# tub-rip/emba

Hardware: AMD Instinct MI355X
Metric: events/sec through warp+Jacobian+JtJ build, 1M events, 1024x2048 pano (higher is better)
Workload: dtype f64; 1 GPU; synthetic N=1000000 sensor=240x180 pano=1024x2048 K=21 seed=20240907; events_per_gpu=1000000, total_events=1000000, thres_valid_pixel=5, cost=quadratic, parallelism=single GPU, events_per_rank=1000000, ep_in_step=True, inliers_rank0=675197, candidates_rank0=956800, active_pixels=68600

## Files before the change

emba_amd/_lib.py:

```python
import ctypes as C
import os

_HERE = os.path.dirname(os.path.abspath(__file__))
LIB_PATH = os.environ.get("EMBA_LIB", os.path.join(_HERE, "libemba_hip.so"))

OK, ERR_INVALID_ARG, ERR_NO_DEVICE, ERR_HIP, ERR_TIME_RANGE, ERR_STATE, ERR_CAPACITY, ERR_NUMERIC = range(8)
STATUS_NAMES = ["EMBA_OK", "EMBA_ERR_INVALID_ARG", "EMBA_ERR_NO_DEVICE", "EMBA_ERR_HIP", "EMBA_ERR_TIME_RANGE",
                "EMBA_ERR_STATE", "EMBA_ERR_CAPACITY", "EMBA_ERR_NUMERIC"]

_dp = C.POINTER(C.c_double)
_i32p = C.POINTER(C.c_int32)
_u32p = C.POINTER(C.c_uint32)
_u16p = C.POINTER(C.c_uint16)
_u8p = C.POINTER(C.c_uint8)
_i64p = C.POINTER(C.c_int64)
_szp = C.POINTER(C.c_size_t)
_fp = C.POINTER(C.c_float)


class EmbaCfg(C.Structure):
    _fields_ = [("sensor_w", C.c_int32), ("sensor_h", C.c_int32), ("pano_w", C.c_int32), ("pano_h", C.c_int32),
                ("bearing_lut", _dp), ("C_th", C.c_double), ("event_batch", C.c_int32), ("outlier_px", C.c_double),
                ("device", C.c_int32), ("stream", C.c_void_p)]


class EmbaAlignSettings(C.Structure):
    _fields_ = [("max_iters", C.c_int32), ("min_pixels", C.c_int32), ("lambda0", C.c_double), ("lambda_up", C.c_double), ("lambda_down", C.c_double),
                ("lambda_min", C.c_double), ("lambda_max", C.c_double), ("tol_rot", C.c_double), ("huber_k", C.c_double)]


class EmbaTrackSettings(C.Structure):
    _fields_ = [("n_levels", C.c_int32), ("levels", C.c_int32 * 8), ("batch", C.c_int32), ("predict", C.c_int32), ("skip_zero", C.c_int32),
                ("min_weight", C.c_uint64), ("min_overlap", C.c_double), ("align", EmbaAlignSettings)]


class EmbaExposureSettings(C.Structure):
    _fields_ = [("align", EmbaAlignSettings), ("gain_min", C.c_double), ("gain_max", C.c_double)]


class EmbaTrackExposureSettings(C.Structure):
    _fields_ = [("track", EmbaTrackSettings), ("estimate", C.c_int32), ("gain_min", C.c_double), ("gain_max", C.c_double)]


class EmbaRefitSettings(C.Structure):
    _fields_ = [("track", EmbaTrackExposureSettings), ("sweeps", C.c_int32), ("alternate", C.c_int32), ("recover", C.c_int32), ("sweep_tol", C.c_double)]


class EmbaGraphSettings(C.Structure):
    _fields_ = [("max_iters", C.c_int32), ("cg_max_iters", C.c_int32), ("lambda0", C.c_double), ("lambda_up", C.c_double), ("lambda_down", C.c_double),
                ("lambda_min", C.c_double), ("lambda_max", C.c_double), ("tol", C.c_double), ("cg_tol", C.c_double)]


SIGNATURES = {
    "emba_abi_version": (C.c_int, []),
    "emba_build_info": (C.c_char_p, []),
    "emba_create": (C.c_int, [C.POINTER(EmbaCfg), C.POINTER(C.c_void_p)]),
    "emba_destroy": (None, [C.c_void_p]),
    "emba_last_error": (C.c_char_p, [C.c_void_p]),
    "emba_set_events": (C.c_int, [C.c_void_p, _u16p, _u16p, _u8p, _i64p, C.c_size_t, _u16p, _u16p, _i64p, C.c_size_t]),
    "emba_set_events_dev": (C.c_int, [C.c_void_p, C.c_void_p, C.c_void_p, C.c_void_p, C.c_void_p, C.c_size_t, C.c_void_p, C.c_void_p, C.c_void_p,
                                      C.c_size_t]),
    "emba_last_setup_ms": (C.c_int, [C.c_void_p, _dp, _dp, _i32p, _szp, _szp]),
    "emba_last_order_stats": (C.c_int, [C.c_void_p, _dp, _dp]),
    "emba_last_order_inlier_estimate": (C.c_int, [C.c_void_p, _dp]),
    "emba_last_tile_geometry": (C.c_int, [C.c_void_p, _i32p, _i32p, _i32p, _i32p, _i32p]),
    "emba_last_tile_drift": (C.c_int, [C.c_void_p, _szp, _i32p]),
    "emba_event_counts": (C.c_int, [C.c_void_p, _szp, _szp]),
    "emba_eval_data_error": (C.c_int, [C.c_void_p, _dp, C.c_int32, C.c_int64, C.c_int64, _dp, _dp, C.c_int32, _dp, _szp, _i32p]),
    "emba_form_normal_eq": (C.c_int, [C.c_void_p, _dp, C.c_int32, C.c_int32, C.c_double, C.c_double, _dp, _dp, _szp, _u32p,
                                      C.c_size_t, _dp, _dp, _dp]),
    "emba_get_A12_sparse": (C.c_int, [C.c_void_p, _i32p, _i32p, _i32p, _dp, _dp, _dp, _dp]),
    "emba_compact_ep": (C.c_int, [C.c_void_p]),
    "emba_get_ep": (C.c_int, [C.c_void_p, _dp, C.c_size_t, _szp]),
    "emba_get_inlier_pixels": (C.c_int, [C.c_void_p, _u32p]),
    "emba_get_inlier_pixel_starts": (C.c_int, [C.c_void_p, _u32p]),
    "emba_get_ep_by_pixel": (C.c_int, [C.c_void_p, _dp, C.POINTER(C.c_uint64)]),
    "emba_data_cost": (C.c_int, [C.c_void_p, C.c_int32, C.c_double, _dp]),
    "emba_reg_cost": (C.c_int, [C.c_void_p, C.c_double, _dp]),
    "emba_costs": (C.c_int, [C.c_void_p, C.c_int32, C.c_double, C.c_double, _dp, _dp]),
    "emba_costs_launch": (C.c_int, [C.c_void_p, C.c_int32, C.c_double, C.c_int32]),
    "emba_costs_finish": (C.c_int, [C.c_void_p, C.c_int32, C.c_double, C.c_double, _dp, _dp]),
    "emba_dump_state": (C.c_int, [C.c_void_p, _dp, _dp, _i32p, _i32p, _i32p, _dp, _dp, _dp]),
    "emba_upload_map": (C.c_int, [C.c_void_p, _dp, _dp]),
    "emba_bind_map_dev": (C.c_int, [C.c_void_p, C.c_void_p, C.c_void_p]),
    "emba_solve_normal_eq": (C.c_int, [C.c_void_p, C.c_double, C.c_int32, _dp, _dp]),
    "emba_solve_map_only": (C.c_int, [C.c_void_p, C.c_double, _dp]),
    "emba_solve_poses_only": (C.c_int, [C.c_void_p, C.c_double, C.c_int32, _dp]),
    "emba_last_solve_info": (C.c_int, [C.c_void_p, _i32p]),
    "emba_solve_shard_size": (C.c_int, [C.c_void_p, _szp]),
    "emba_solve_shard_count": (C.c_int, [C.c_void_p, C.c_int32, _szp]),
    "emba_solve_shard_pack": (C.c_int, [C.c_void_p, C.c_int32, C.c_void_p]),
    "emba_cg_shard_size": (C.c_int, [C.c_void_p, _szp]),
    "emba_cg_shard_begin": (C.c_int, [C.c_void_p, C.c_int32, C.c_int32, C.c_void_p, C.c_size_t, C.c_double, C.c_int32, C.c_void_p]),
    "emba_cg_shard_apply": (C.c_int, [C.c_void_p, C.c_void_p]),
    "emba_cg_shard_pt": (C.c_int, [C.c_void_p, C.c_void_p, _dp]),
    "emba_cg_shard_update": (C.c_int, [C.c_void_p, C.c_double, C.c_void_p]),
    "emba_cg_shard_direction": (C.c_int, [C.c_void_p, C.c_double]),
    "emba_cg_shard_end": (C.c_int, [C.c_void_p, _dp, C.c_void_p]),
    "emba_solve_shard_cached": (C.c_int, [C.c_void_p, C.c_int32, C.c_int32, _i32p, _szp]),
    "emba_solve_shard_partial": (C.c_int, [C.c_void_p, C.c_int32, C.c_int32, C.c_void_p, C.c_size_t, C.c_double, C.c_void_p]),
    "emba_solve_shard_finish": (C.c_int, [C.c_void_p, C.c_int32, C.c_int32, C.c_void_p, C.c_size_t, C.c_double, C.c_int32, C.c_void_p, _dp, C.c_void_p]),
    "emba_solve_normal_eq_cg": (C.c_int, [C.c_void_p, C.c_double, C.c_int32, C.c_int32, C.c_double, _dp, _dp, _i32p, _dp]),
    "emba_update_map": (C.c_int, [C.c_void_p, _dp, C.c_double]),
    "emba_update_map_dev": (C.c_int, [C.c_void_p, C.c_void_p, C.c_double]),
    "emba_map_accept": (C.c_int, [C.c_void_p]),
    "emba_map_reject": (C.c_int, [C.c_void_p]),
    "emba_trial_reject": (C.c_int, [C.c_void_p]),
    "emba_download_map": (C.c_int, [C.c_void_p, _dp, _dp]),
    "emba_get_map_active": (C.c_int, [C.c_void_p, _dp, C.c_size_t]),
    "emba_set_cost": (C.c_int, [C.c_void_p, C.c_int32, C.c_double]),
    "emba_reconstruct_intensity": (C.c_int, [C.c_void_p, _dp, _dp, _dp]),
    "emba_render_map_images": (C.c_int, [C.c_void_p, C.c_double, _u8p, _u8p, _u8p, _u8p]),
    "emba_reconstruct_intensity_bc": (C.c_int, [C.c_void_p, _dp, _dp, _dp, C.c_int32]),
    "emba_render_map_images_bc": (C.c_int, [C.c_void_p, C.c_double, _u8p, _u8p, _u8p, _u8p, C.c_int32]),
    "emba_normalize_robust": (C.c_int, [C.c_void_p, _dp, C.c_size_t, C.c_double, _u8p, _dp, _dp]),
    "emba_seq_upload": (C.c_int, [C.c_void_p, _u16p, _u16p, _u8p, _i64p, C.c_size_t, C.c_int32, _szp]),
    "emba_seq_size": (C.c_int, [C.c_void_p, _szp]),
    "emba_seq_free": (C.c_int, [C.c_void_p]),
    "emba_seq_window": (C.c_int, [C.c_void_p, C.c_int64, C.c_int64, _szp, _szp]),
    "emba_set_events_seq": (C.c_int, [C.c_void_p, C.c_size_t, C.c_size_t]),
    "emba_set_events_seq_shard": (C.c_int, [C.c_void_p, C.c_size_t, C.c_size_t, C.c_size_t]),
    "emba_seq_halo": (C.c_int, [C.c_void_p, C.c_size_t, C.c_size_t, _u16p, _u16p, _i64p, C.c_size_t, _szp]),
    "emba_seq_get": (C.c_int, [C.c_void_p, C.c_size_t, C.c_size_t, _u16p, _u16p, _u8p, _i64p]),
    "emba_seq_filter": (C.c_int, [C.c_void_p, C.c_double, C.c_int64, C.c_int64, C.c_int32, C.POINTER(C.c_uint64)]),
    "emba_seq_hot_pixels": (C.c_int, [C.c_void_p, _u8p]),
    "emba_seq_cmax": (C.c_int, [C.c_void_p, C.c_int64, C.c_double, _dp, _i64p, C.POINTER(C.c_uint64), C.POINTER(C.c_uint64), _i32p, C.c_size_t, _szp]),
    "emba_seq_cmax_objective": (C.c_int, [C.c_void_p, C.c_size_t, C.c_size_t, _dp, C.c_size_t, C.POINTER(C.c_uint64), _u32p, _i32p, _i32p, _i32p]),
    "emba_seq_event_panorama": (C.c_int, [C.c_void_p, C.c_size_t, C.c_size_t, _dp, C.c_int32, C.c_int64, C.c_int64, C.c_int32, _i32p, C.POINTER(C.c_uint64), _i64p,
                                          C.POINTER(C.c_uint64), C.POINTER(C.c_uint64), _dp]),
    "emba_seq_contrast_gradient": (C.c_int, [C.c_void_p, C.c_size_t, C.c_size_t, _dp, C.c_int32, C.c_int64, C.c_int64, C.c_int32, _dp, _dp, _dp,
                                             C.POINTER(C.c_uint64), _dp, _dp, _i32p]),
    "emba_seq_contrast_gradient_level": (C.c_int, [C.c_void_p, C.c_size_t, C.c_size_t, _dp, C.c_int32, C.c_int64, C.c_int64, C.c_int32, C.c_int32, _dp, _dp,
                                                   _dp, C.POINTER(C.c_uint64), _dp, _dp, _i32p]),
    "emba_seq_contrast_prior_add": (C.c_int, [C.c_void_p, C.c_size_t, C.c_size_t, _dp, C.c_int32, C.c_int64, C.c_int64, C.c_int32, C.c_uint32, _szp,
                                              C.POINTER(C.c_uint64)]),
    "emba_seq_contrast_prior_set": (C.c_int, [C.c_void_p, C.c_int32, _dp]),
    "emba_seq_contrast_prior_get": (C.c_int, [C.c_void_p, C.c_int32, _dp, _i32p]),
    "emba_seq_contrast_prior_clear": (C.c_int, [C.c_void_p]),
    "emba_seq_contrast_gradient_prior": (C.c_int, [C.c_void_p, C.c_size_t, C.c_size_t, _dp, C.c_int32, C.c_int64, C.c_int64, C.c_int32, C.c_int32, C.c_double,
                                                   _dp, _dp, _dp, C.POINTER(C.c_uint64), _dp, _dp, _i32p]),
    "emba_render_views": (C.c_int, [C.c_void_p, _dp, C.c_int32, _i64p, C.c_size_t, _dp, C.c_int32, C.c_int64, C.c_int64, C.c_double, C.c_double, C.c_double,
                                    _dp, _u8p, C.POINTER(C.c_uint64), _dp]),
    "emba_seq_event_frames": (C.c_int, [C.c_void_p, C.c_size_t, C.c_size_t, _i64p, C.c_size_t, C.c_int32, _i32p, C.POINTER(C.c_uint64), C.POINTER(C.c_uint64)]),
    "emba_mosaic_frames": (C.c_int, [C.c_void_p, _u8p, _i64p, C.c_size_t, _dp, C.c_int32, C.c_int64, C.c_int64, C.c_int32, C.c_int32, C.POINTER(C.c_uint64),
                                     C.POINTER(C.c_uint64), _dp]),
    "emba_mosaic_get": (C.c_int, [C.c_void_p, C.c_uint64, C.c_double, C.POINTER(C.c_uint64), C.POINTER(C.c_uint64), _dp, _u8p, C.POINTER(C.c_uint64)]),
    "emba_mosaic_map": (C.c_int, [C.c_void_p, C.c_uint64, C.c_double, C.c_double, C.c_double, C.c_int32, _dp, _dp, _dp, C.c_int32]),
    "emba_mosaic_clear": (C.c_int, [C.c_void_p]),
    "emba_simulate_events": (C.c_int, [C.c_void_p, _dp, C.c_int32, _i64p, C.c_size_t, _dp, C.c_int32, C.c_int64, C.c_int64, C.c_double, C.c_double, C.c_int32,
                                       C.c_uint64, C.POINTER(C.c_uint64)]),
    "emba_sim_size": (C.c_int, [C.c_void_p, _szp]),
    "emba_sim_get": (C.c_int, [C.c_void_p, C.c_size_t, C.c_size_t, _u16p, _u16p, _u8p, _i64p]),
    "emba_seq_from_sim": (C.c_int, [C.c_void_p, C.c_int32, _szp]),
    "emba_frames_align_eval": (C.c_int, [C.c_void_p, _u8p, C.c_size_t, _dp, _dp, _u8p, C.c_int32, C.c_uint64, C.c_double, C.c_double, C.c_double, C.c_int32,
                                         C.c_double, _dp, C.POINTER(C.c_uint64), _dp, _dp]),
    "emba_frames_align": (C.c_int, [C.c_void_p, _u8p, C.c_size_t, _dp, _dp, _u8p, C.c_int32, C.c_uint64, C.c_double, C.c_double, C.c_double, C.c_int32,
                                    C.c_void_p, _dp, _dp, C.POINTER(C.c_uint64), _i32p, _i32p, _dp, C.POINTER(C.c_uint64)]),
    "emba_frames_track": (C.c_int, [C.c_void_p, _u8p, _i64p, C.c_size_t, _dp, C.c_void_p, _dp, _i32p, _i32p, _dp, C.POINTER(C.c_uint64), _dp, C.POINTER(C.c_uint64), _dp]),
    "emba_track_eval": (C.c_int, [C.c_void_p, _u8p, C.c_size_t, _dp, C.c_int32, C.c_uint64, C.c_int32, C.c_double, _dp, C.POINTER(C.c_uint64), _dp, _dp]),
    "emba_track_level_get": (C.c_int, [C.c_void_p, C.c_int32, C.POINTER(C.c_uint64), C.POINTER(C.c_uint64)]),
    "emba_frames_exposure_eval": (C.c_int, [C.c_void_p, _u8p, C.c_size_t, _dp, _dp, _dp, _dp, _u8p, C.c_int32, C.c_uint64, C.c_double, C.c_double, C.c_double,
                                            C.c_int32, C.c_double, _dp, C.POINTER(C.c_uint64), _dp, _dp]),
    "emba_frames_exposure_align": (C.c_int, [C.c_void_p, _u8p, C.c_size_t, _dp, _dp, _dp, C.c_int32, _dp, _u8p, C.c_int32, C.c_uint64, C.c_double, C.c_double,
                                             C.c_double, C.c_int32, C.c_void_p, _dp, _dp, _dp, _dp, C.POINTER(C.c_uint64), _i32p, _i32p, _dp, C.POINTER(C.c_uint64)]),
    "emba_mosaic_frames_exposure": (C.c_int, [C.c_void_p, _u8p, _i64p, C.c_size_t, _dp, _dp, _dp, C.c_int32, C.c_int64, C.c_int64, C.c_int32, C.c_int32,
                                              C.POINTER(C.c_uint64), C.POINTER(C.c_uint64), _dp]),
    "emba_frames_track_exposure": (C.c_int, [C.c_void_p, _u8p, _i64p, C.c_size_t, _dp, C.c_void_p, _dp, _dp, _dp, _i32p, _i32p, _dp, C.POINTER(C.c_uint64), _dp,
                                             C.POINTER(C.c_uint64), _dp]),
    "emba_track_exposure_eval": (C.c_int, [C.c_void_p, _u8p, C.c_size_t, _dp, _dp, _dp, C.c_int32, C.c_uint64, C.c_int32, C.c_double, _dp, C.POINTER(C.c_uint64),
                                           _dp, _dp]),
    "emba_frames_refit": (C.c_int, [C.c_void_p, _u8p, _i64p, C.c_size_t, _dp, _dp, _dp, _i32p, C.c_void_p, _dp, _dp, _dp, _i32p, _i32p, _i32p, _dp,
                                    C.POINTER(C.c_uint64), _dp, _dp, _i32p, C.POINTER(C.c_uint64), _dp]),
    "emba_frames_pair_eval": (C.c_int, [C.c_void_p, _u8p, C.c_size_t, _i32p, C.c_size_t, _dp, _dp, _dp, C.c_double, C.c_double, C.c_double, C.c_double, _dp,
                                        C.c_int32, C.c_double, _dp, C.POINTER(C.c_uint64), _dp, _dp]),
    "emba_frames_pair_align": (C.c_int, [C.c_void_p, _u8p, C.c_size_t, _i32p, C.c_size_t, _dp, _dp, _dp, C.c_double, C.c_double, C.c_double, C.c_double, _dp,
                                         C.c_int32, C.c_void_p, _dp, _dp, C.POINTER(C.c_uint64), _i32p, _i32p, _dp, C.POINTER(C.c_uint64), _dp]),
    "emba_rotation_graph_solve": (C.c_int, [_dp, _i32p, C.c_size_t, _i32p, _dp, _dp, C.c_size_t, C.c_void_p, _dp, _dp, _i32p, _i32p, _szp]),
    "emba_median_blur3_map": (C.c_int, [C.c_void_p]),
    "emba_median_blur3": (C.c_int, [C.c_void_p, _dp, C.c_int32, C.c_int32, _dp]),
    "emba_bind_exchange_buffers": (C.c_int, [C.c_void_p, C.c_void_p, C.c_void_p, C.c_size_t]),
    "emba_count_map_ready": (C.c_int, [C.c_void_p]),
    "emba_count_compress": (C.c_int, [C.c_void_p, C.c_void_p, C.c_int32]),
    "emba_count_expand": (C.c_int, [C.c_void_p, C.c_void_p]),
    "emba_step_form_active": (C.c_int, [C.c_void_p, C.c_int32, C.c_void_p]),
    "emba_eval_launch": (C.c_int, [C.c_void_p, _dp, C.c_int32, C.c_int64, C.c_int64]),
    "emba_eval_finish": (C.c_int, [C.c_void_p, _dp, _szp, _i32p]),
    "emba_form_active": (C.c_int, [C.c_void_p, C.c_int32, _szp, _szp]),
    "emba_form_accumulate": (C.c_int, [C.c_void_p, _dp, C.c_int32, C.c_double]),
    "emba_form_finish": (C.c_int, [C.c_void_p, C.c_double, _dp, _dp, _u32p, C.c_size_t, _dp, _dp, _dp]),
    "emba_step": (C.c_int, [C.c_void_p, _dp, C.c_int32, C.c_int64, C.c_int64, C.c_int32, C.c_int32, C.c_double, C.c_double, _szp, _szp]),
    "emba_last_counts": (C.c_int, [C.c_void_p, _szp, _szp]),
    "emba_set_option": (C.c_int, [C.c_void_p, C.c_char_p, C.c_int32]),
    "emba_get_option": (C.c_int, [C.c_void_p, C.c_char_p, _i32p]),
    "emba_sync": (C.c_int, [C.c_void_p]),
    "emba_timer_start": (C.c_int, [C.c_void_p, C.c_int32]),
    "emba_timer_stop": (C.c_int, [C.c_void_p, C.c_int32]),
    "emba_timer_elapsed_ms": (C.c_int, [C.c_void_p, C.c_int32, _fp]),
    "emba_enable_kernel_timing": (C.c_int, [C.c_void_p, C.c_int32]),
    "emba_last_kernel_ms": (C.c_int, [C.c_void_p, _fp, _fp]),
    "emba_kernel_ms_slot": (C.c_int, [C.c_void_p, C.c_int32, _fp, _fp]),
    "emba_kernel_timing_all": (C.c_int, [C.c_void_p, C.c_int32]),
    "emba_kernel_ms_all": (C.c_int, [C.c_void_p, C.c_int32, _fp]),
    "emba_bracket_overhead_us": (C.c_int, [C.c_void_p, C.c_int32, _fp]),
    "emba_clock_probe": (C.c_int, [C.c_void_p, _dp, _dp, _dp, _i32p, _i32p, _i32p]),
    "emba_device_pci_bus_id": (C.c_int, [C.c_void_p, C.c_char_p, C.c_size_t]),
    "emba_group_create": (C.c_int, [C.POINTER(EmbaCfg), _i32p, C.c_int32, C.POINTER(C.c_void_p)]),
    "emba_group_create_flags": (C.c_int, [C.POINTER(EmbaCfg), _i32p, C.c_int32, C.c_uint32, C.POINTER(C.c_void_p)]),
    "emba_group_set_option": (C.c_int, [C.c_void_p, C.c_char_p, C.c_int32]),
    "emba_group_destroy": (None, [C.c_void_p]),
    "emba_group_last_error": (C.c_char_p, [C.c_void_p]),
    "emba_group_size": (C.c_int32, [C.c_void_p]),
    "emba_group_uses_rccl": (C.c_int32, [C.c_void_p]),
    "emba_group_ctx": (C.c_void_p, [C.c_void_p, C.c_int32]),
    "emba_group_set_events": (C.c_int, [C.c_void_p, _u16p, _u16p, _u8p, _i64p, C.c_size_t]),
    "emba_group_seq_upload": (C.c_int, [C.c_void_p, _u16p, _u16p, _u8p, _i64p, C.c_size_t, C.c_int32, _szp]),
    "emba_group_seq_size": (C.c_int, [C.c_void_p, _szp]),
    "emba_group_seq_free": (C.c_int, [C.c_void_p]),
    "emba_group_seq_window": (C.c_int, [C.c_void_p, C.c_int64, C.c_int64, _szp, _szp]),
    "emba_group_seq_filter": (C.c_int, [C.c_void_p, C.c_double, C.c_int64, C.c_int64, C.c_int32, C.POINTER(C.c_uint64)]),
    "emba_group_set_events_seq": (C.c_int, [C.c_void_p, C.c_size_t, C.c_size_t]),
    "emba_group_median_blur3_map": (C.c_int, [C.c_void_p]),
    "emba_group_upload_map": (C.c_int, [C.c_void_p, _dp, _dp]),
    "emba_group_step": (C.c_int, [C.c_void_p, _dp, C.c_int32, C.c_int64, C.c_int64, C.c_int32, C.c_int32, C.c_double, C.c_double, _szp, _szp]),
    "emba_group_eval": (C.c_int, [C.c_void_p, _dp, C.c_int32, C.c_int64, C.c_int64, _dp, _dp, _dp, _szp, _i32p]),
    "emba_group_get_ep": (C.c_int, [C.c_void_p, _dp, C.c_size_t, _szp]),
    "emba_group_form": (C.c_int, [C.c_void_p, C.c_int32, C.c_int32, C.c_double, C.c_double, _szp, _szp]),
    "emba_group_set_cost": (C.c_int, [C.c_void_p, C.c_int32, C.c_double]),
    "emba_group_apply_l2": (C.c_int, [C.c_void_p, C.c_double]),
    "emba_group_last_solve_exchanged": (C.c_int, [C.c_void_p, _i32p]),
    "emba_group_solve_cg": (C.c_int, [C.c_void_p, C.c_double, C.c_int32, C.c_int32, C.c_double, _dp, _dp, _i32p, _dp]),
    "emba_group_trial_reject": (C.c_int, [C.c_void_p]),
    "emba_group_download": (C.c_int, [C.c_void_p, _dp, _dp, _u32p, C.c_size_t, _dp, _dp]),
    "emba_group_costs": (C.c_int, [C.c_void_p, C.c_int32, C.c_double, C.c_double, _dp, _dp]),
    "emba_group_solve": (C.c_int, [C.c_void_p, C.c_double, C.c_int32, _dp, _dp]),
    "emba_group_solve_map_only": (C.c_int, [C.c_void_p, C.c_double, _dp]),
# ... 32 lines not shown
```

emba_amd/csrc/context.h:

```cpp
#pragma once
#include "../../include/emba_hip.h"

#include <hip/hip_runtime.h>

#include <algorithm>
#include <cmath>
#include <cstdarg>
#include <cstdio>
#include <string>
#include <vector>

#include "kernels.h"
#include "solve_kernels.h"
#include "map_rule.h"
#include "cmax_rule.h"
#include "contrast_rule.h"

struct DevBuf {
    void* p = nullptr;
    size_t bytes = 0;
    DevBuf() = default;
    DevBuf(DevBuf&& o) noexcept : p(o.p), bytes(o.bytes) { o.p = nullptr; o.bytes = 0; }
    DevBuf& operator=(DevBuf&& o) noexcept { if (this != &o) { reset(); std::swap(p, o.p); std::swap(bytes, o.bytes); } return *this; }
    ~DevBuf() { reset(); }
    template <typename T> T* as() const { return static_cast<T*>(p); }
    void reset() { if (p) (void)hipFree(p); p = nullptr; bytes = 0; }
    hipError_t ensure(size_t n, bool* fresh = nullptr, bool poison = false, hipStream_t s = nullptr)
    {
        n = std::max<size_t>(n, 8);
        if (fresh) *fresh = false;
        if (p && bytes >= n) return hipSuccess;
        reset();
        hipError_t e = hipMalloc(&p, n);
        if (e != hipSuccess) { p = nullptr; return e; }
        bytes = n;
        if (fresh) *fresh = true;
        return poison ? hipMemsetAsync(p, 0xFF, n, s) : hipSuccess;
    }
};

struct RecordSet { DevBuf rec, tag; uint32_t stamp = 0; };

struct SolveLists { uint32_t* off = nullptr; emba::RecView sorted{}; };

struct EqState {
    bool active_done = false, accum_done = false;
    bool finish_done = false;
    bool compact_valid = false;
    bool l2_fused = false;
    bool force_generic_a22 = false;
    size_t P = 0, pack_len = 0;
    int K = 0, thres = 0, irls = 0; double eta = 0;
};

struct EvalState {
    bool launched = false, done = false;
    bool ep_deferred = false;
    bool inl_pending = false, P_pending = false;
    bool seq_armed = false;
    bool inl_idx_valid = false;
    bool ep_valid = false;
    bool ep_in_gram = false;
    bool ep_after_gram = false;
    bool pix_starts_valid = false;
    uint32_t count_stamp = 0;
    int acc_irls = 0; double acc_eta = 0.0;
    int use_texel = 0;
    bool prep_in_warp = false;
    bool texels_packed = false;
    bool segpose = false;
    bool readable() const { return launched && (done || inl_pending || ep_deferred); }
};

struct PixAccState {
    bool first_use() const { return dirty_all_; }
    bool lines_clean() const { return clean_; }
    bool lines_consumed() const { return consumed_; }
    bool counts_raw() const { return raw_; }
    int32_t marker() const { return mark_; }
    void bound() { dirty_all_ = true; clean_ = false; }
    void first_use_cleared() { dirty_all_ = false; clean_ = true; }
    void marked(int32_t marker) { mark_ = marker; clean_ = false; consumed_ = false; raw_ = true; }
    void not_marked() { raw_ = false; }
    void materialised() { raw_ = false; }
    void consumed_by_gather() { clean_ = true; consumed_ = true; }
private:
    bool dirty_all_ = true, clean_ = false, consumed_ = false, raw_ = false;
    int32_t mark_ = 0;
};

struct MapPlanes {
    DevBuf own_x, own_y, trial_x, trial_y;
    const double* Gx() const { return x_; }
    const double* Gy() const { return y_; }
    const double* cur_Gx() const { return cur_x_; }
    const double* cur_Gy() const { return cur_y_; }
    const emba::MapState& state() const { return st_; }
    void uploaded() { to_own(); st_.uploaded(); }
    void bound(const double* gx, const double* gy) { x_ = cur_x_ = gx; y_ = cur_y_ = gy; st_.bound(); }
    void trial_built() { x_ = trial_x.as<double>(); y_ = trial_y.as<double>(); st_.trial_built(); }
    void accepted() { std::swap(own_x, trial_x); std::swap(own_y, trial_y); to_own(); st_.accepted(); }
    void rejected() { x_ = cur_x_; y_ = cur_y_; st_.rejected(); }
    void blurred() { to_own(); st_.blurred(); }
    void texels_packed() { st_.texels_packed(); }
private:
    void to_own() { x_ = cur_x_ = own_x.as<double>(); y_ = cur_y_ = own_y.as<double>(); }
    const double *x_ = nullptr, *y_ = nullptr, *cur_x_ = nullptr, *cur_y_ = nullptr;
    emba::MapState st_;
};

struct PostWarpState {
    bool gather_deferred = false; emba::ActiveWriteParams gather{};
    int fsup_half = 0;
    void defer(const emba::ActiveWriteParams& aw) { gather = aw; gather_deferred = true; }
};

struct EvalOpts { int irls = 0; double eta = 0.0; bool keep_alt_set = false; };
struct FormOpts {
    bool consume = false, wants_ep = false;
    const uint8_t* global_u8 = nullptr;
    double fused_alpha = 0.0;
};

struct WindowState {
    bool have_events = false;
    size_t n_in = 0, n_used = 0, n_halo = 0, n_pm = 0, n_sorted = 0, n_batch = 0, n_cand = 0;
    long nblk = 0;
    long n_fblk = 0, n_fsup = 0;
    size_t P_prev = 0;
    size_t n_outside_tile = 0; int n_rebin = 0; uint32_t last_rebin_stamp = 0;
};

struct OrderState {
    bool keys_ready = false; int64_t key_t0 = 0, key_dt = 0; int key_K = 0;
    uint32_t* d_ev_pix = nullptr; uint32_t* d_ev_batch = nullptr;
    bool tile_order = false, have_ev_pm = false;
    long n_chunks = 0;
    size_t n_lead = 0;
    bool chunks_lpt = false;
    int tile_shape = 0; bool tile_fine = false;
    double order_per_px = 0.0, order_lead_frac = 0.0;
    double order_inl_pred = 0.0;
    std::vector<uint32_t> run_start; bool runs_known = false;
    int cuts_sw = 0, cuts_base_blocks = 0, cuts_blocks = 0;
};

enum StatusWord : int {
    kStFirstBad = 0,
    kStUnsorted = 1,
    kStProbeA = 0, kStProbeB = 1,
    kStBadHalo = 2,
    kStTotal = 4,
    kStHeads = 6,
    kStCounter = 8,
    kStatusWords = 16
};

struct ListsKey {
    bool packed = false; uint32_t stamp = 0; size_t P = 0, nrec = 0; long lo = 0;
    bool operator==(const ListsKey& o) const { return packed == o.packed && stamp == o.stamp && P == o.P && nrec == o.nrec && lo == o.lo; }
};

struct SolveCache {
    bool lists_valid = false; ListsKey key;
    bool perm_valid = false;
    size_t perm_lo = 0, perm_n = 0;
    size_t x2_resident_P = (size_t)-1;
    int info = 0;
    struct CgShard { bool active = false; int rank = 0, n_ranks = 1, n = 0, skip = 0; size_t lo = 0, npix = 0, Nl = 0; double lambda = 0; } cg;
    void invalidate() { lists_valid = false; perm_valid = false; }
};

struct CmaxBuffers { DevBuf omega, t_ref, j0, j, evals, cand, cand_j, cand_iwe; };

struct SeqPoseBuffers { DevBuf batch_t, pose, knots; };

struct PanoBuffers { DevBuf image, slots, out, pm; };

struct ContrastBuffers { DevBuf image, slots, out, pm, D, cp; };

struct ContrastPriors {
    DevBuf image[emba::kContrastLevels], out;
    bool present[emba::kContrastLevels] = {};
    void drop() { for (bool& b : present) b = false; }
    void reset() { drop(); for (DevBuf& b : image) b.reset(); }
};

struct ViewBuffers { DevBuf plane, t, pose, knots, head, frames, u8, pm, outside, edge, counts, ends; };

struct MosaicBuffers {
    DevBuf sum_w, sum_v; uint64_t votes = 0;
    DevBuf t, pose, knots, head, frames, pm, counters, mean, covered, L, covered_log, gx, gy;
};

struct FrameLoopBuffers {
    DevBuf frames, pm, resid, partial, q_trial, esums, ecounts;
    DevBuf q, sums, counts, lambda, dnorm, status, iters, have_trial, cost0, n0, running;
};

struct AlignBuffers { DevBuf plane, valid; FrameLoopBuffers loop; };

struct TrackBuffers {
    DevBuf lw[8], lv[8]; uint32_t voted = 0;
    DevBuf t, q_all, status_all, iters_all, cost_all, overlap_all, counts_all, counters, pred;
    DevBuf gain_all, bias_all, gain_pred, bias_pred, gain_trial, bias_trial, gain, bias;
    DevBuf refit_all;
    FrameLoopBuffers loop;
};

struct ExposureBuffers {
    FrameLoopBuffers loop;
    DevBuf gain_trial, bias_trial, gain, bias;
    DevBuf vote_gain, vote_bias;
};

struct PairBuffers { DevBuf pairs, gain, bias; FrameLoopBuffers loop; };

struct SimState {
    DevBuf x, y, pol, t, x2, y2, pol2, t2; size_t n = 0; bool have = false; uint64_t stats[4] = {0, 0, 0, 0};
    DevBuf plane, step_t, pose, knots, head, frames, outside, cells, ref[2], armed[2], sums, total, ev_t, ev_sp;
};

struct PoissonBuffers {
    DevBuf SH;
    DevBuf lamH;
    DevBuf SW;
    DevBuf lamW;
    DevBuf thomas;
    DevBuf wrapq;
    DevBuf Sfold;
    DevBuf Gx, Gy;
    DevBuf F;
    DevBuf T;
    DevBuf EO;
};

struct emba_ctx {
    emba_cfg cfg{};
    int device = 0;
    hipStream_t stream = nullptr;
    bool own_stream = false;
    std::string err;

    int sw = 0, sh = 0, W = 0, H = 0;
    size_t S = 0, npix = 0;
    double fx = 0, fy = 0, cx = 0, cy = 0, C_th = 0, outlier_px = 10.0;
    double fov_x = M_PI, fov_y = M_PI;

    DevBuf d_lut;
    DevBuf d_texel;
    MapPlanes map;
    SolveCache solve;
    int solve_perm_mode = -1;
    double* h_cost = nullptr;
    double* h_cost_dev = nullptr; DevBuf d_cost_acc; int cost_seq = 0;
    DevBuf d_x2;
    DevBuf d_count_own; int32_t* d_count = nullptr;
    DevBuf d_pixacc;
    PixAccState pix;
    int texel_mode = 0;
    DevBuf d_rect;
    uint32_t seg_seq = 0;
    int step_prep = 0, step_prep_polls = 1024;
    emba::InlineSegParams seg_inline{}; emba::InlineKnots seg_knots{};
    DevBuf d_seg_flag;
    DevBuf d_blk_rect;
    DevBuf d_compact, d_active_bits;
    DevBuf d_active;
    DevBuf d_ablk_cnt, d_ablk_off; size_t n_ablk = 0;
    DevBuf d_pack_own;
    double* d_pack = nullptr; size_t pack_cap = 0; bool pack_bound = false;
    DevBuf d_knots;
    int* d_err = nullptr;
    DevBuf d_err2;
    uint32_t eval_seq = 0;
    DevBuf d_total;
    std::vector<uint32_t> h_pix_starts;
    void* h_stage[2] = {nullptr, nullptr}; hipEvent_t stage_ev[2]{};
    int* h_pinned = nullptr;
    int seq = 0;
    bool spun = false;
    int* h_pinned_dev = nullptr;
    double* h_knots_dev = nullptr;

    WindowState win;
    OrderState order;
    DevBuf d_pm_pix, d_pm_batch, d_pm_orig;
    DevBuf d_ev_slot;
    DevBuf d_ev_pix_own, d_ev_batch_own;
    DevBuf d_ev_pm;
    DevBuf d_cp, d_batch_u;
    DevBuf d_ev_u, d_ev_seg;
    DevBuf d_chunks;
    int segpose_mode = 0;
    int order_mode = 0;
    DevBuf d_batch_t, d_pose;
    DevBuf d_seg;
    int step_gather = 2;
    DevBuf d_seg_act;
    PostWarpState post;
    int step_one_set = 1;
    int step_fast = 1;
    int use_tags = 1;
    DevBuf d_gram_cuts; std::vector<uint32_t> h_gram_cuts; bool last_gram_paired = false;
    DevBuf d_slot_key; uint32_t rec_stamp = 0;
    RecordSet work, alt;
    bool eq_in_alt = false;
    EqState eq, eq_saved;
    EvalState ev;
    DevBuf d_e_sorted, d_flag, d_inl_idx;
    int opt_poison = 0;
    int opt_tile_reserve = 2, opt_tile_shape = -1, opt_tile_fine = -1, opt_tile_min_events = 1650000, opt_tile_chunk = 0;
    int opt_gather_waves = 0, opt_chunk_order_bin = 0, opt_solve_counts = -1, opt_syrk_dense = 0, opt_syrk_lists = 0, opt_gram_sparse = -1, opt_gram_sparse_chunk = 4, opt_gram_multikey = 0, opt_syrk_min_cols = 512, opt_syrk_item_cap = 4096, opt_solve_debug = 0, opt_poisson = 0, opt_gemm64 = 0;
    int step_ep = 1;
    DevBuf d_fblk_cnt, d_fblk_off;
    DevBuf d_fsup;
    DevBuf d_ep;
    double set_events_ms = 0, prepare_ms = 0;

    size_t n_inliers = 0;
    int cost_irls = 0; double cost_eta = 0.0;
    double* h_knots = nullptr; int h_knots_cap = 0; hipEvent_t knots_copied = nullptr; bool knots_in_flight = false;

    hipEvent_t ev_start[8]{}, ev_stop[8]{};
    bool kernel_timing = false;
    hipEvent_t kt_sets[16][5]{}; hipEvent_t* kt = kt_sets[0]; int kt_slot = 0;
    bool kt_valid[16][3]{};
    bool kt_all = false;
    hipEvent_t cal_ev[2]{};
    DevBuf d_probe;
    bool kt_warp_valid = false, kt_accum_valid = false;
    int n_cu = 256;
    int ablate = 0;
    struct {
        DevBuf scan_sums, scan_offs;
        DevBuf sort_hist;
        DevBuf status;
        DevBuf keys[2], vals[2];
        DevBuf flags;
        DevBuf pos;
        DevBuf bin, used;
        DevBuf bin_start_or_x;
        DevBuf pred_or_y;
        DevBuf heads_or_pol;
        DevBuf halo;
    } ord;
    struct Solve {
        DevBuf S_or_x, rhs_or_r, U_or_p, y_or_z, cf_or_t, x2_or_invd;
        DevBuf info_or_sc;
        DevBuf slab, mask, list, cnt, range, pair_items, items;
        DevBuf perm_cnt, perm_tick, perm;
        DevBuf shard_cnt;
    } sv;
    struct {
        DevBuf off, cursor, sorted, tmp;
    } lists;
    struct {
        DevBuf out;
        DevBuf pix_starts;
        DevBuf A22b2;
    } dl;
    PoissonBuffers poisson;
    DevBuf d_rstate, d_rhist, d_rcand;
    DevBuf d_img, d_nsrc;
    struct {
        DevBuf x, y, pol, t, raw, status, halo_last, halo_flag, halo_pos; size_t n = 0;
        DevBuf x2, y2, pol2, t2, f_start, f_hot, f_sums; bool have = false, have_hot = false;
        void reset()
        {
            for (DevBuf* b : {&x, &y, &pol, &t, &raw, &status, &halo_last, &halo_flag, &halo_pos, &x2, &y2, &pol2, &t2, &f_start, &f_hot, &f_sums}) b->reset();
            n = 0; have = have_hot = false;
        }
    } evseq;
    emba::CmaxPinhole cmax_pin;
    CmaxBuffers cmax;
    SeqPoseBuffers seq_pose;
    PanoBuffers pano;
    ContrastBuffers contrast;
    ContrastPriors priors;
    int opt_contrast_vote = -1;
    int contrast_vote_path = -1;
    ViewBuffers view;
    SimState sim;
    MosaicBuffers mosaic;
    AlignBuffers align;
    TrackBuffers track;
    ExposureBuffers exposure;
    PairBuffers pair;
    DevBuf d_blur;
};

namespace {

thread_local std::string g_create_error;

emba_status fail(emba_ctx* c, emba_status st, const char* fmt, ...)
{
    char buf[512];
    va_list ap;
    va_start(ap, fmt);
    vsnprintf(buf, sizeof buf, fmt, ap);
    va_end(ap);
    if (c) c->err = buf; else g_create_error = buf;
    return st;
}

#define HIP_TRY(c, call)                                                                         \
    do {                                                                                         \
        hipError_t e_ = (call);                                                                  \
        if (e_ != hipSuccess)                                                                    \
            return fail((c), EMBA_ERR_HIP, "%s failed: %s (%s:%d)", #call, hipGetErrorString(e_), \
                        __FILE__, __LINE__);                                                     \
    } while (0)

template <typename T>
emba_status ensure(emba_ctx* c, DevBuf& b, size_t count, bool* fresh = nullptr)
// ... 13 lines not shown
```

emba_amd/csrc/device_math.h:

```cpp
#pragma once
#include <hip/hip_runtime.h>
#include <stdint.h>

namespace emba {

#pragma clang fp contract(off)

constexpr double kSophusEps = 1e-10;
constexpr double kPi = 3.14159265358979323846;

__device__ __forceinline__ double sum3(double a, double b, double c) { return a + (b + c); }
__device__ __forceinline__ double sqn3(double a, double b, double c) { return (a + b) + c; }

__device__ __forceinline__ void mat3_mul(const double* A, const double* B, double* C)
{
    double T[9];
#pragma unroll
    for (int i = 0; i < 3; ++i)
#pragma unroll
        for (int j = 0; j < 3; ++j) {
            const double t0 = A[3 * i + 0] * B[0 + j], t1 = A[3 * i + 1] * B[3 + j], t2 = A[3 * i + 2] * B[6 + j];
            T[3 * i + j] = (i < 2) ? (t0 + t1) + t2 : t0 + (t1 + t2);
        }
#pragma unroll
    for (int i = 0; i < 9; ++i) C[i] = T[i];
}

__device__ __forceinline__ void hat3(const double* p, double* M)
{
    M[0] = 0;     M[1] = -p[2]; M[2] = p[1];
    M[3] = p[2];  M[4] = 0;     M[5] = -p[0];
    M[6] = -p[1]; M[7] = p[0];  M[8] = 0;
}

__device__ __forceinline__ void quat_normalize(double* q)
{
    const double n2 = (q[0] * q[0] + q[2] * q[2]) + (q[1] * q[1] + q[3] * q[3]);
    const double n = sqrt(n2);
    q[0] /= n; q[1] /= n; q[2] /= n; q[3] /= n;
}

__device__ __forceinline__ void so3_mul(const double* a, const double* b, double* out)
{
    const double ax = a[0], ay = a[1], az = a[2], aw = a[3];
    const double bx = b[0], by = b[1], bz = b[2], bw = b[3];
    double r[4];
    r[3] = aw * bw - ax * bx - ay * by - az * bz;
    r[0] = aw * bx + ax * bw + ay * bz - az * by;
    r[1] = aw * by + ay * bw + az * bx - ax * bz;
    r[2] = aw * bz + az * bw + ax * by - ay * bx;
    quat_normalize(r);
    out[0] = r[0]; out[1] = r[1]; out[2] = r[2]; out[3] = r[3];
}

__device__ __forceinline__ void quat_to_matrix(const double* q, double* R)
{
    const double x = q[0], y = q[1], z = q[2], w = q[3];
    const double tx = 2 * x, ty = 2 * y, tz = 2 * z;
    const double twx = tx * w, twy = ty * w, twz = tz * w;
    const double txx = tx * x, txy = ty * x, txz = tz * x;
    const double tyy = ty * y, tyz = tz * y, tzz = tz * z;
    R[0] = 1 - (tyy + tzz); R[1] = txy - twz;       R[2] = txz + twy;
    R[3] = txy + twz;       R[4] = 1 - (txx + tzz); R[5] = tyz - twx;
    R[6] = txz - twy;       R[7] = tyz + twx;       R[8] = 1 - (txx + tyy);
}

__device__ __forceinline__ void sin_cos_half(double x, double& sn, double& cs)
{
    if (fabs(x) <= 0x1.921fb54442d18p-1) {
        const double z = x * x;
        const double rs = fma(z, fma(z, fma(z, fma(z, 1.58969099521155010221e-10, -2.50507602534068634195e-08), 2.75573137070700676789e-06),
                                     -1.98412698298579493134e-04), 8.33333333332248946124e-03);
        sn = fma(z * x, fma(z, rs, -1.66666666666666324348e-01), x);
        const double rc = z * fma(z, fma(z, fma(z, fma(z, fma(z, -1.13596475577881948265e-11, 2.08757232129817482790e-09), -2.75573143513906633035e-07),
                                              2.48015872894767294178e-05), -1.38888888888741095749e-03), 4.16666666666666019037e-02);
        const double hz = 0.5 * z, w = 1.0 - hz;
        cs = w + fma(z, rc, (1.0 - w) - hz);
    } else {
        sn = sin(x); cs = cos(x);
    }
}

__device__ __forceinline__ double rcp_nr(double x)
{
    double r = __builtin_amdgcn_rcp(x);
    double e = fma(-x, r, 1.0);
    r = fma(r, e, r);
    e = fma(-x, r, 1.0);
    return fma(r, e, r);
}

__device__ __forceinline__ void so3_exp(const double* w, double* q)
{
    const double theta_sq = sqn3(w[0] * w[0], w[1] * w[1], w[2] * w[2]);
    double imag, real;
    if (theta_sq < kSophusEps * kSophusEps) {
        const double theta_po4 = theta_sq * theta_sq;
        imag = 0.5 - (1.0 / 48.0) * theta_sq + (1.0 / 3840.0) * theta_po4;
        real = 1.0 - (1.0 / 8.0) * theta_sq + (1.0 / 384.0) * theta_po4;
    } else {
        const double theta = sqrt(theta_sq);
        const double half = 0.5 * theta;
        double sn, cs;
        sin_cos_half(half, sn, cs);
        imag = sn / theta;
        real = cs;
    }
    q[0] = imag * w[0]; q[1] = imag * w[1]; q[2] = imag * w[2]; q[3] = real;
}

__device__ __forceinline__ void so3_log(const double* q, double* w)
{
    const double squared_n = sqn3(q[0] * q[0], q[1] * q[1], q[2] * q[2]);
    const double qw = q[3];
    double f;
    if (squared_n < kSophusEps * kSophusEps) {
        const double squared_w = qw * qw;
        f = 2.0 / qw - (2.0 / 3.0) * (squared_n) / (qw * squared_w);
    } else {
        const double n = sqrt(squared_n);
        if (fabs(qw) < kSophusEps) f = (qw > 0.0) ? kPi / n : -kPi / n;
        else f = 2.0 * atan(n / qw) / n;
    }
    w[0] = f * q[0]; w[1] = f * q[1]; w[2] = f * q[2];
}

__device__ __forceinline__ void left_jacobian(const double* phi, double* J)
{
    const double n2 = sqn3(phi[0] * phi[0], phi[1] * phi[1], phi[2] * phi[2]);
    double H[9], H2[9];
    hat3(phi, H);
    mat3_mul(H, H, H2);
#pragma unroll
    for (int i = 0; i < 9; ++i) J[i] = (i % 4 == 0) ? 1.0 : 0.0;
    if (n2 > kSophusEps) {
        const double n = sqrt(n2);
        const double n3 = n2 * n;
        const double c1 = 1 - cos(n), c2 = n - sin(n);
#pragma unroll
        for (int i = 0; i < 9; ++i) J[i] += H[i] * c1 / n2;
#pragma unroll
        for (int i = 0; i < 9; ++i) J[i] += H2[i] * c2 / n3;
    } else {
#pragma unroll
        for (int i = 0; i < 9; ++i) J[i] += H[i] / 2;
#pragma unroll
        for (int i = 0; i < 9; ++i) J[i] += H2[i] / 6;
    }
}

__device__ __forceinline__ void left_jacobian_inv(const double* phi, double* J)
{
    const double n2 = sqn3(phi[0] * phi[0], phi[1] * phi[1], phi[2] * phi[2]);
    double H[9], H2[9];
    hat3(phi, H);
    mat3_mul(H, H, H2);
#pragma unroll
    for (int i = 0; i < 9; ++i) J[i] = ((i % 4 == 0) ? 1.0 : 0.0) - H[i] / 2;
    if (n2 > kSophusEps) {
        const double n = sqrt(n2);
        if (n < kPi - sqrt(kSophusEps)) {
            const double c = 1 / n2 - (1 + cos(n)) / (2 * n * sin(n));
#pragma unroll
            for (int i = 0; i < 9; ++i) J[i] += H2[i] * c;
        } else {
#pragma unroll
            for (int i = 0; i < 9; ++i) J[i] += H2[i] / (kPi * kPi);
        }
    } else {
#pragma unroll
        for (int i = 0; i < 9; ++i) J[i] += H2[i] / 12;
    }
}

__device__ __forceinline__ void spline2_eval(const double* p0, const double* p1, double u, double* q_out, double* J1)
{
    double p0inv[4] = {-p0[0], -p0[1], -p0[2], p0[3]};
    quat_normalize(p0inv);
    double r01[4], delta[3], kdelta[3];
    so3_mul(p0inv, p1, r01);
    so3_log(r01, delta);
#pragma unroll
    for (int i = 0; i < 3; ++i) kdelta[i] = delta[i] * u;
    double Jli[9], Jlk[9], T[9], R0[9], R0inv[9];
    left_jacobian_inv(delta, Jli);
    left_jacobian(kdelta, Jlk);
    quat_to_matrix(p0, R0);
#pragma unroll
    for (int i = 0; i < 9; ++i) T[i] = u * R0[i];
    mat3_mul(T, Jlk, T);
    mat3_mul(T, Jli, T);
    quat_to_matrix(p0inv, R0inv);
    mat3_mul(T, R0inv, J1);
    double e[4], res[4];
    so3_exp(kdelta, e);
    so3_mul(p0, e, res);
    q_out[0] = res[0]; q_out[1] = res[1]; q_out[2] = res[2]; q_out[3] = res[3];
}

__device__ __forceinline__ void project_jacobian(const double* rb, double fx, double fy, double* J23);

__device__ __forceinline__ void segment_consts(const double* p0, const double* p1, double* seg)
{
    double p0inv[4] = {-p0[0], -p0[1], -p0[2], p0[3]};
    quat_normalize(p0inv);
    double r01[4], delta[3], R0[9];
    so3_mul(p0inv, p1, r01);
    so3_log(r01, delta);
    const double n2 = sqn3(delta[0] * delta[0], delta[1] * delta[1], delta[2] * delta[2]);
    const double th = sqrt(n2);
    double k[3] = {0, 0, 0}, r2;
    if (th > 0.0) {
        quat_to_matrix(p0, R0);
        const double a0 = delta[0] / th, a1 = delta[1] / th, a2 = delta[2] / th;
#pragma unroll
        for (int r = 0; r < 3; ++r) k[r] = R0[3 * r] * a0 + R0[3 * r + 1] * a1 + R0[3 * r + 2] * a2;
    }
    if (n2 > kSophusEps) {
        if (th < kPi - sqrt(kSophusEps)) r2 = 1.0 - th * (1.0 + cos(th)) / (2.0 * sin(th));
        else r2 = n2 / (kPi * kPi);
    } else {
        r2 = n2 / 12.0;
    }
    seg[0] = p0[0]; seg[1] = p0[1]; seg[2] = p0[2]; seg[3] = p0[3];
    seg[4] = delta[0]; seg[5] = delta[1]; seg[6] = delta[2]; seg[7] = -0.5 * th;
    seg[8] = k[0]; seg[9] = k[1]; seg[10] = k[2]; seg[11] = r2;
}

__device__ __forceinline__ void rebuild_j1(double u, double a1, double a2, const double* k, double* J1)
{
    const double kk = k[0] * k[0] + k[1] * k[1] + k[2] * k[2];
    const double d = u - a2 * kk;
    J1[0] = d + a2 * k[0] * k[0]; J1[1] = a2 * k[0] * k[1] - a1 * k[2]; J1[2] = a2 * k[0] * k[2] + a1 * k[1];
    J1[3] = a2 * k[1] * k[0] + a1 * k[2]; J1[4] = d + a2 * k[1] * k[1]; J1[5] = a2 * k[1] * k[2] - a1 * k[0];
    J1[6] = a2 * k[2] * k[0] - a1 * k[1]; J1[7] = a2 * k[2] * k[1] + a1 * k[0]; J1[8] = d + a2 * k[2] * k[2];
}

__device__ __attribute__((noinline)) double2 sin_cos_call(double x)
{
    double sn, cs;
    sin_cos_half(x, sn, cs);
    return make_double2(sn, cs);
}

template <bool CALL>
__device__ __forceinline__ void spline2_event(const double* seg, double u, double* q_out, double* J1)
{
    const double kd[3] = {seg[4] * u, seg[5] * u, seg[6] * u};
    const double theta_sq = sqn3(kd[0] * kd[0], kd[1] * kd[1], kd[2] * kd[2]);
    double imag, real, p1c, p2c;
    if (theta_sq < kSophusEps * kSophusEps) {
        const double theta_po4 = theta_sq * theta_sq;
        imag = 0.5 - (1.0 / 48.0) * theta_sq + (1.0 / 3840.0) * theta_po4;
        real = 1.0 - (1.0 / 8.0) * theta_sq + (1.0 / 384.0) * theta_po4;
        const double n = sqrt(theta_sq);
        p1c = 0.5 * n; p2c = theta_sq * (1.0 / 6.0);
    } else {
        const double theta = sqrt(theta_sq);
        const double half = 0.5 * theta;
        double sh, ch;
        if (CALL) { const double2 sc = sin_cos_call(half); sh = sc.x; ch = sc.y; }
        else sin_cos_half(half, sh, ch);
        imag = sh / theta;
        real = ch;
        if (theta_sq > kSophusEps) { const double it2 = 2.0 * rcp_nr(theta); p1c = sh * sh * it2; p2c = 1.0 - sh * ch * it2; }
        else { p1c = 0.5 * theta; p2c = theta_sq * (1.0 / 6.0); }
    }
    const double e[4] = {imag * kd[0], imag * kd[1], imag * kd[2], real};
    so3_mul(seg, e, q_out);
    const double r1 = seg[7], r2 = seg[11];
    const double alpha = p1c + r1 - p1c * r2 - p2c * r1, gamma = p2c + r2 + p1c * r1 - p2c * r2;
    rebuild_j1(u, u * alpha, u * gamma, seg + 8, J1);
}

__device__ __forceinline__ void project_jacobian(const double* rb, double fx, double fy, double* J23);

__device__ __attribute__((noinline)) double2 project_angles_call(double x, double y, double z)
{
    const double phi = atan2(x, z);
    const double r2 = x * x + y * y + z * z;
    return make_double2(phi, asin(y / sqrt(r2)));
}


template <bool CALL = false>
__device__ __forceinline__ void project_chain(const double* rb, double fx, double fy, double cx, double cy,
                                              double* pm, double* J23)
{
    if (CALL) {
        const double2 a = project_angles_call(rb[0], rb[1], rb[2]);
        pm[0] = cx + a.x * fx;
        pm[1] = cy + a.y * fy;
        project_jacobian(rb, fx, fy, J23);
        return;
    }
    const double x = rb[0], y = rb[1], z = rb[2];
    const double phi = atan2(x, z);
    const double r2 = x * x + y * y + z * z;
    const double theta = asin(y / sqrt(r2));
    pm[0] = cx + phi * fx;
    pm[1] = cy + theta * fy;
    project_jacobian(rb, fx, fy, J23);
}

#pragma clang fp contract(fast)
__device__ __forceinline__ void project_jacobian(const double* rb, double fx, double fy, double* J23)
{
    const double x = rb[0], y = rb[1], z = rb[2];
    const double d2 = x * x + z * z;
    const double rho = sqrt(d2 + y * y);
    const double inv_rho = rcp_nr(rho);
    const double Ydivrho = y * inv_rho;
    const double inv_d2 = rcp_nr(d2);
    const double inv_d = fx * inv_d2;
    const double tmp2 = -fy * rho * (sqrt(d2) * inv_d2);
    const double tmp3 = Ydivrho * inv_rho * inv_rho;
    const double Jp[6] = {z * inv_d, 0.0, -x * inv_d, tmp2 * tmp3 * x, tmp2 * (tmp3 * y - inv_rho), tmp2 * tmp3 * z};
    const double M[9] = {0, rb[2], -rb[1], -rb[2], 0, rb[0], rb[1], -rb[0], 0};
#pragma unroll
    for (int i = 0; i < 2; ++i)
#pragma unroll
        for (int j = 0; j < 3; ++j) {
            double s = 0;
#pragma unroll
            for (int k = 0; k < 3; ++k) s += Jp[3 * i + k] * M[3 * k + j];
            J23[3 * i + j] = s;
        }
}

}
```

emba_amd/csrc/kernels.h:

```cpp
#pragma once
#include <hip/hip_runtime.h>
#include <stdint.h>

#include "device_math.h"
#include "order_rule.h"
#include "step_rule.h"

#ifdef EMBA_DIAG
#define EMBA_ABL(word, bit) (((word) & (bit)) != 0)
#else
#define EMBA_ABL(word, bit) false
#endif

namespace emba {

constexpr uint32_t kNoSlot = 0xFFFFFFFFu;
constexpr uint32_t kInvalidPix = 0xFFFFFFFFu;

__device__ __forceinline__ bool record_valid(double tail_y, uint32_t stamp, uint32_t& pano_idx)
{
    pano_idx = (uint32_t)__double2loint(tail_y);
    return (uint32_t)__double2hiint(tail_y) == stamp && pano_idx != kInvalidPix;
}
__host__ __device__ __forceinline__ int32_t count_marker(uint32_t stamp) { return (int32_t)(0x80000000u | (stamp & 0x3FFFFFFFu)); }
constexpr int kPoseStride = 14;
#ifndef TEXEL_STRIDE
#define TEXEL_STRIDE 6
#endif
constexpr int kTexelStride = TEXEL_STRIDE;
constexpr int kRecStride = 16;
constexpr int kWarpBlock = 64;
constexpr int kWarpNew = 63;
constexpr int kRecLds = 18;
constexpr int kPixAccStride = 8;
#ifndef REC_NT_STORE
#define REC_NT_STORE 1
#endif
#ifndef EP_NT_STORE
#define EP_NT_STORE 1
#endif
#ifndef GRAM_NT_LOAD
#define GRAM_NT_LOAD 1
#endif
#ifndef EV_NT_LOAD
#define EV_NT_LOAD 1
#endif
#ifndef GRAM_TAG_NT
#define GRAM_TAG_NT 0
#endif
template <class T> __device__ __forceinline__ T stream_load(const T* p, bool nt) { return nt ? __builtin_nontemporal_load(p) : *p; }
#ifndef GRAM_DUMMY_LOADS
#define GRAM_DUMMY_LOADS 0
#endif
#ifndef GRAM_U_NT
#define GRAM_U_NT 3
#endif
#ifndef GRAM_U
#define GRAM_U 4
#endif
#ifndef GRAM_SPARSE_TS
#define GRAM_SPARSE_TS 2
#endif
constexpr int kGramPad = 256;
constexpr int kGramChunkMin = 64;
constexpr int kGramChunk = 1024;
#ifndef GATHER_Q
#define GATHER_Q 4
#endif
#ifndef GRAM_GATHER_WAVES
#ifndef GRAM_WAVE_TILE
#define GRAM_WAVE_TILE 1
#endif
#define GRAM_GATHER_WAVES 4
#endif
constexpr int kGramBlock = 1024;
constexpr int kGramKeys = 4;

__device__ __forceinline__ long xcd_contiguous_block(long bid, long grid)
{
    const long per = grid >> 3;
    return (bid & 7) * per + (bid >> 3);
}

__device__ __forceinline__ void pose_thread(int b, const int64_t* __restrict__ batch_t_ns, int nb, const double* __restrict__ knots,
                                            int K, int64_t t0_ns, int64_t dt_ns, double* __restrict__ pose, int* __restrict__ err)
{
    if (b >= nb) return;
    const int64_t st = batch_t_ns[b] - t0_ns;
    const int64_t s = (st >= 0) ? st / dt_ns : -1;
    if (st < 0 || s + 2 > (int64_t)K) {
        atomicOr(err, 1);
        return;
    }
    const double u = (double)(st % dt_ns) / (double)dt_ns;
    double p0[4], p1[4];
#pragma unroll
    for (int i = 0; i < 4; ++i) { p0[i] = knots[4 * s + i]; p1[i] = knots[4 * (s + 1) + i]; }
    double q[4], J1[9];
    spline2_eval(p0, p1, u, q, J1);
    double* o = pose + (size_t)kPoseStride * b;
#pragma unroll
    for (int i = 0; i < 4; ++i) o[i] = q[i];
#pragma unroll
    for (int i = 0; i < 9; ++i) o[4 + i] = J1[i];
    o[13] = (double)s;
}

constexpr int kSegStride = 12;
__device__ __forceinline__ void seg_record(int sidx, const double* __restrict__ knots, double* __restrict__ o)
{
    double p0[4], p1[4];
#pragma unroll
    for (int i = 0; i < 4; ++i) { p0[i] = knots[4 * sidx + i]; p1[i] = knots[4 * (sidx + 1) + i]; }
    segment_consts(p0, p1, o);
#pragma unroll
    for (int i = 0; i < kSegStride; ++i) __asm__ volatile("" : "+v"(o[i]));
}
__device__ __forceinline__ void seg_thread(int sidx, const double* __restrict__ knots, int K, double* __restrict__ seg)
{
    if (sidx >= K - 1) return;
    double o[kSegStride];
    seg_record(sidx, knots, o);
#pragma unroll
    for (int i = 0; i < kSegStride; ++i) seg[(size_t)kSegStride * sidx + i] = o[i];
}

__global__ __launch_bounds__(64) void emba_pose_kernel(const int64_t* __restrict__ batch_t_ns, int nb, const double* __restrict__ knots, int K,
                                                       int64_t t0_ns, int64_t dt_ns, double* __restrict__ pose, int* __restrict__ err)
{
    pose_thread(blockIdx.x * 64 + threadIdx.x, batch_t_ns, nb, knots, K, t0_ns, dt_ns, pose, err);
}

__device__ __forceinline__ int reflect101(int i, int n)
{
    if (n == 1) return 0;
    if (i < 0) i = -i;
    if (i >= n) i = 2 * (n - 1) - i;
    return i;
}

__device__ __forceinline__ void hessian_at(const double* __restrict__ Gx, const double* __restrict__ Gy, int H, int W, int x, int y,
                                           double& g_x, double& g_y, double& gxx_o, double& gxy_o, double& gyy_o)
{
    const int xl = reflect101(x - 1, W), xr = reflect101(x + 1, W);
    const int yu = reflect101(y - 1, H), yd = reflect101(y + 1, H);
    const double* gxu = Gx + (size_t)yu * W; const double* gxc = Gx + (size_t)y * W; const double* gxd = Gx + (size_t)yd * W;
    const double* gyu = Gy + (size_t)yu * W; const double* gyc = Gy + (size_t)y * W; const double* gyd = Gy + (size_t)yd * W;
    const double gxx = ((gxu[xr] - gxu[xl]) + (gxd[xr] - gxd[xl])) + 2 * (gxc[xr] - gxc[xl]);
    const double gyx = ((gyu[xr] - gyu[xl]) + (gyd[xr] - gyd[xl])) + 2 * (gyc[xr] - gyc[xl]);
    const double gxy = ((gxd[xl] + gxd[xr]) + 2 * gxd[x]) - ((gxu[xl] + gxu[xr]) + 2 * gxu[x]);
    const double gyy = ((gyd[xl] + gyd[xr]) + 2 * gyd[x]) - ((gyu[xl] + gyu[xr]) + 2 * gyu[x]);
    g_x = gxc[x]; g_y = gyc[x];
    gxx_o = 0.125 * gxx;
    gxy_o = 0.5 * (0.125 * gxy + 0.125 * gyx);
    gyy_o = 0.125 * gyy;
}

__device__ __forceinline__ void texel_rect(const int* __restrict__ acc, int W, int H, int& x0, int& y0, int& x1, int& y1)
{
    const int ax0 = acc[0], ay0 = acc[1], ax1 = acc[2], ay1 = acc[3];
    if (ax1 < ax0 || ay1 < ay0) { x0 = 0; y0 = 0; x1 = -1; y1 = -1; return; }
    x0 = max(ax0 - kRectMargin, 0); y0 = max(ay0 - kRectMargin, 0);
    x1 = min(ax1 + kRectMargin, W - 1); y1 = min(ay1 + kRectMargin, H - 1);
}

__device__ __forceinline__ void texel_rect_blocks(long blk, long nblocks, const double* __restrict__ Gx, const double* __restrict__ Gy,
                                                  int H, int W, const int* __restrict__ rect_acc, double* __restrict__ texel)
{
    int x0, y0, x1, y1;
    texel_rect(rect_acc, W, H, x0, y0, x1, y1);
    const long rw = x1 - x0 + 1, total = rw * (long)(y1 - y0 + 1);
    for (long idx = blk * 256 + threadIdx.x; idx < total; idx += nblocks * 256) {
        const int x = x0 + (int)(idx % rw), y = y0 + (int)(idx / rw);
        double gx, gy, gxx, gxy, gyy;
        hessian_at(Gx, Gy, H, W, x, y, gx, gy, gxx, gxy, gyy);
        double2* t = reinterpret_cast<double2*>(texel + (size_t)kTexelStride * ((size_t)y * W + x));
        t[0] = make_double2(gx, gy);
        t[1] = make_double2(gxx, gxy);
        t[2] = make_double2(gyy, 0.0);
    }
}

__global__ __launch_bounds__(256) void emba_texel_kernel(const double* __restrict__ Gx, const double* __restrict__ Gy,
                                                         int H, int W, double* __restrict__ texel)
{
    static_assert(kTexelStride == 6, "three 16-B pieces per texel");
    __shared__ __attribute__((aligned(16))) double s_t[4][64 * kTexelStride];
    const int x0 = blockIdx.x * blockDim.x, lane = threadIdx.x & 63, wv = threadIdx.x >> 6;
    const int x = x0 + threadIdx.x;
    const int y = blockIdx.y;
    double gx = 0, gy = 0, gxx = 0, gxy = 0, gyy = 0;
    if (x < W) hessian_at(Gx, Gy, H, W, x, y, gx, gy, gxx, gxy, gyy);
    double2* l = reinterpret_cast<double2*>(s_t[wv] + kTexelStride * lane);
    l[0] = make_double2(gx, gy); l[1] = make_double2(gxx, gxy); l[2] = make_double2(gyy, 0.0);
    __asm__ volatile("s_waitcnt lgkmcnt(0)" ::: "memory");
    const int xw = x0 + 64 * wv;
    const int n_tex = (W - xw < 64) ? (W - xw) : 64;
    if (n_tex <= 0) return;
    double2* out = reinterpret_cast<double2*>(texel + (size_t)kTexelStride * ((size_t)y * W + xw));
    const double2* in = reinterpret_cast<const double2*>(s_t[wv]);
#pragma unroll
    for (int k = 0; k < 3; ++k) {
        const int i = 64 * k + lane;
        if (i < 3 * n_tex) out[i] = in[i];
    }
}

constexpr int kNumTileShapes = 4;
constexpr TileShape kTileShapes[kNumTileShapes] = {
    {48, 24, 32, 8, 16, 4},
    {72, 16, 48, 4, 24, 4},
    {96, 12, 64, 4, 32, 2},
    {36, 32, 24, 8, 12, 8},
};
#ifndef TILE_WAVES
#define TILE_WAVES 8
#endif
#ifndef TILE_OCC
#define TILE_OCC 4
#endif
constexpr int kTileWaves = TILE_WAVES;
constexpr int kTileRecStage = 16;

struct WarpParams {
    const uint32_t* ev_pix; const uint32_t* ev_batch; const uint32_t* ev_slot; const uint32_t* ev_pm; long n_sorted; long nblk;
    const double* ev_u; const uint16_t* ev_seg;
    const double* pose; const double* seg; const double* lut; const double* texel;
    const int* rect_acc;
    const double* Gx; const double* Gy;
    int W, H; double fx, fy, cx, cy, C_th, outlier_px;
    int32_t* count; double* pixacc; double* rec; double* tag; double* e_sorted; uint8_t* flag;
    int* err;
    double* d_pm; double* d_D; double* d_dp; double* d_Gpm; double* d_temp; int32_t* d_pm_int;
    int rec_nt;
    int ablate;
    int irls; double eta;
    uint32_t stamp;
    int32_t marker;
    const ChunkDesc* chunks; long n_chunks; int chunks_linear;
};

__device__ __forceinline__ int dpp_shr1(int v) { return __builtin_amdgcn_update_dpp(0, v, 0x138, 0xf, 0xf, false); }
__device__ __forceinline__ double dpp_shr1(double v)
{
    return __hiloint2double(dpp_shr1(__double2hiint(v)), dpp_shr1(__double2loint(v)));
}
__device__ __forceinline__ int dpp_shl1(int v) { return __builtin_amdgcn_update_dpp(0, v, 0x130, 0xf, 0xf, false); }
__device__ __forceinline__ double dpp_shl1(double v)
{
    return __hiloint2double(dpp_shl1(__double2hiint(v)), dpp_shl1(__double2loint(v)));
}

constexpr int kInlineKnots = 104;
struct InlineKnots { double q[4 * kInlineKnots]; };

struct InlineSegParams {
    double* seg; unsigned seg_bytes;
    unsigned* flag; unsigned seq;
    int K, polls;
    unsigned* fallbacks;
    int* err_next; double* knots_out;
};
typedef __attribute__((address_space(1))) unsigned gu32;
typedef __attribute__((address_space(1))) unsigned long long gu64;
struct InlineSegLane { __amdgpu_buffer_rsrc_t rsrc; };

__device__ __forceinline__ void inline_seg_produce(const InlineSegParams& h, const double* __restrict__ knots, int t, bool duties)
{
    for (int sidx = t; sidx < h.K - 1; sidx += kWarpBlock) {
        double o[kSegStride];
        seg_record(sidx, knots, o);
        gu64* dst = (gu64*)(h.seg + (size_t)kSegStride * sidx);
#pragma unroll
        for (int i = 0; i < kSegStride; ++i) __hip_atomic_store(dst + i, (unsigned long long)__double_as_longlong(o[i]), __ATOMIC_RELAXED, __HIP_MEMORY_SCOPE_AGENT);
    }
    __asm__ volatile("s_waitcnt vmcnt(0)" ::: "memory");
    if (!duties) return;
    if (t == 0) __hip_atomic_store((gu32*)h.flag, h.seq, __ATOMIC_RELAXED, __HIP_MEMORY_SCOPE_AGENT);
    if (t == 63) h.err_next[0] = 0;
    if (h.knots_out) for (int i = t; i < 4 * h.K; i += kWarpBlock) h.knots_out[i] = knots[i];
}
__device__ __forceinline__ bool inline_seg_wait(const InlineSegParams& h)
{
    bool ready = false;
    for (int n = 0; n < h.polls; ++n) {
        const unsigned f = (unsigned)__builtin_amdgcn_readfirstlane((int)__hip_atomic_load((gu32*)h.flag, __ATOMIC_RELAXED, __HIP_MEMORY_SCOPE_AGENT));
        if (f == h.seq) { ready = true; break; }
        __builtin_amdgcn_s_sleep(8);
    }
    __builtin_amdgcn_fence(__ATOMIC_ACQUIRE, "wavefront");
    return ready;
}

#ifndef WARP_LATE_EP
#define WARP_LATE_EP 0
#endif
struct LaneOut {
    bool inl; uint32_t pi; int pmx, pmy; bool wr_flag;
    double jc[6], jp[6], dpx, dpy, e;
    double v0, v1, v2, v3, v4;
};

struct LaneIn { uint32_t pw, bi, slot, pm; bool valid; double u; };

template <bool COMPACT, bool SEGPOSE = false>
__device__ __forceinline__ void load_event_words(const WarpParams& p, long i, bool valid, LaneIn& in)
{
    const long last = p.n_sorted - 1;
    const long ic = i < 0 ? 0 : (i > last ? last : i);
    in.valid = valid; in.u = 0.0;
    in.pw = stream_load(p.ev_pix + ic, COMPACT && EV_NT_LOAD); in.slot = stream_load(p.ev_slot + ic, COMPACT && EV_NT_LOAD);
    if (COMPACT) { in.pm = stream_load(p.ev_pm + ic, EV_NT_LOAD); in.u = stream_load(p.ev_u + ic, EV_NT_LOAD); in.bi = stream_load(p.ev_seg + ic, EV_NT_LOAD); }
    else if (SEGPOSE) { in.pm = (uint32_t)ic; in.u = p.ev_u[ic]; in.bi = p.ev_seg[ic]; }
    else { in.pm = (uint32_t)ic; in.bi = stream_load(p.ev_batch + ic, EV_NT_LOAD); }
}

struct NoPrefetch { __device__ __forceinline__ void operator()() const {} };
template <bool DUMP, bool COMPACT = false, class PF = NoPrefetch, bool LATE_EP = false, bool SEGPOSE = false, bool INLINE_SEG = false>
__device__ __forceinline__ void warp_lane(const WarpParams& p, long i, const LaneIn& in, int t, LaneOut& o, PF prefetch = PF(), const InlineSegLane* is = nullptr)
{
    const bool valid = in.valid;
    double pm[2] = {0, 0};
    double D[12];
#pragma unroll
    for (int k = 0; k < 12; ++k) D[k] = 0;
    uint32_t pw = 0, pol = 0;

    if (valid) {
        pw = in.pw;
        const uint32_t pix = pw & 0x1FFFFFFFu;
        pol = pw >> 31;
        const uint32_t bi = in.bi;
        const double* bv = p.lut + 3 * (size_t)pix;
        double b0, b1, b2;
        if (COMPACT) { b0 = bv[0]; b1 = bv[1]; b2 = bv[2]; }
        double R[9], J1[9];
        if (COMPACT || SEGPOSE) {
            const uint32_t sg = bi; const double uu = in.u;
            double seg[kSegStride];
            if (INLINE_SEG) {
                typedef unsigned int v4u __attribute__((ext_vector_type(4)));
                typedef double v2d __attribute__((ext_vector_type(2)));
                const int off = (int)(sg * (uint32_t)(kSegStride * sizeof(double)));
#pragma unroll
                for (int k = 0; k < kSegStride / 2; ++k) {
                    const v2d v = __builtin_bit_cast(v2d, (v4u)__builtin_amdgcn_raw_buffer_load_b128(is->rsrc, off + 16 * k, 0, 16));
                    seg[2 * k] = v.x; seg[2 * k + 1] = v.y;
                }
            } else {
                const double2* S2 = reinterpret_cast<const double2*>(p.seg + (size_t)kSegStride * (EMBA_ABL(p.ablate, 16) ? (sg & 1u) : sg));
                const double2 s0 = S2[0], s1 = S2[1], s2 = S2[2], s3 = S2[3], s4 = S2[4], s5 = S2[5];
                seg[0] = s0.x; seg[1] = s0.y; seg[2] = s1.x; seg[3] = s1.y; seg[4] = s2.x; seg[5] = s2.y;
                seg[6] = s3.x; seg[7] = s3.y; seg[8] = s4.x; seg[9] = s4.y; seg[10] = s5.x; seg[11] = s5.y;
            }
            double q[4];
            spline2_event<!DUMP>(seg, uu, q, J1);
            quat_to_matrix(q, R);
        } else {
            const double2* P2 = reinterpret_cast<const double2*>(p.pose + (size_t)kPoseStride * bi);
            const double2 a0 = P2[0], a1 = P2[1], a2 = P2[2], a3 = P2[3], a4 = P2[4], a5 = P2[5], a6 = P2[6];
            const double q[4] = {a0.x, a0.y, a1.x, a1.y};
            quat_to_matrix(q, R);
            J1[0] = a2.x; J1[1] = a2.y; J1[2] = a3.x; J1[3] = a3.y; J1[4] = a4.x; J1[5] = a4.y; J1[6] = a5.x; J1[7] = a5.y; J1[8] = a6.x;
        }
        if (!COMPACT) { b0 = bv[0]; b1 = bv[1]; b2 = bv[2]; }
        double rb[3];
        {
#pragma clang fp contract(off)
#pragma unroll
            for (int r = 0; r < 3; ++r) rb[r] = sum3(R[3 * r] * b0, R[3 * r + 1] * b1, R[3 * r + 2] * b2);
        }
        double J23[6];
        project_chain<COMPACT && !DUMP>(rb, p.fx, p.fy, p.cx, p.cy, pm, J23);
#pragma unroll
        for (int r = 0; r < 2; ++r)
#pragma unroll
            for (int c = 0; c < 3; ++c) {
                double s0 = 0, s1 = 0;
#pragma unroll
                for (int k = 0; k < 3; ++k) {
                    const double j1 = J1[3 * k + c];
                    const double j0 = ((k == c) ? 1.0 : 0.0) - j1;
                    s0 += J23[3 * r + k] * j0;
                    s1 += J23[3 * r + k] * j1;
                }
                D[6 * r + c] = s0;
                D[6 * r + c + 3] = s1;
            }
        if (DUMP) {
            if (p.d_pm) { p.d_pm[2 * i] = pm[0]; p.d_pm[2 * i + 1] = pm[1]; }
            if (p.d_D) {
#pragma unroll
                for (int k = 0; k < 12; ++k) p.d_D[12 * i + k] = D[k];
            }
        }
    }

    const double pmp0 = dpp_shr1(pm[0]), pmp1 = dpp_shr1(pm[1]);

    bool inl = false;
    const bool cand = valid && (t >= 1) && (pw & 0x20000000u);
    uint32_t pi = kInvalidPix;
    int pmx = 0, pmy = 0;
    double dpx = 0, dpy = 0, e = 0, ngx = 0, ngy = 0;
#pragma unroll
    for (int j = 0; j < 6; ++j) { o.jc[j] = 0; o.jp[j] = 0; }
    if (cand) {
        dpx = pm[0] - pmp0;
        dpy = pm[1] - pmp1;
        double dp_norm;
        {
#pragma clang fp contract(off)
            dp_norm = sqrt(dpx * dpx + dpy * dpy);
        }
        const double rx = round(pm[0]), ry = round(pm[1]);
        inl = (dp_norm <= p.outlier_px) && (rx >= 0.0) && (rx < (double)p.W) && (ry >= 0.0) && (ry < (double)p.H);
        if (DUMP && p.d_dp) { p.d_dp[2 * i] = dpx; p.d_dp[2 * i + 1] = dpy; }
        if (inl) {
            pmx = (int)rx; pmy = (int)ry;
            pi = (uint32_t)pmy * (uint32_t)p.W + (uint32_t)pmx;
            double gx = 0.01, gy = 0.02, gxx = 0.001, gxy = 0.002, gyy = 0.003;
            if (!EMBA_ABL(p.ablate, 4)) {
                bool use_tex = p.texel != nullptr;
                if (use_tex && p.rect_acc) {
                    int x0, y0, x1, y1;
                    texel_rect(p.rect_acc, p.W, p.H, x0, y0, x1, y1);
                    use_tex = pmx >= x0 && pmx <= x1 && pmy >= y0 && pmy <= y1;
                }
                if (use_tex) {
                    const double2* T2 = reinterpret_cast<const double2*>(p.texel + (size_t)kTexelStride * pi);
                    const double2 g = T2[0], h0 = T2[1], h1 = T2[2];
                    gx = g.x; gy = g.y; gxx = h0.x; gxy = h0.y; gyy = h1.x;
                } else {
                    hessian_at(p.Gx, p.Gy, p.H, p.W, pmx, pmy, gx, gy, gxx, gxy, gyy);
                }
            }
            const double C_pred = gx * dpx + gy * dpy;
            const double C_meas = 2 * ((double)pol - 0.5) * p.C_th;
            e = C_meas - C_pred;
            const double t0 = gx + (dpx * gxx + dpy * gxy);
            const double t1 = gy + (dpx * gxy + dpy * gyy);
            if (DUMP) {
                if (p.d_Gpm) { p.d_Gpm[2 * i] = gx; p.d_Gpm[2 * i + 1] = gy; }
                if (p.d_temp) { p.d_temp[2 * i] = t0; p.d_temp[2 * i + 1] = t1; }
                if (p.d_pm_int) { p.d_pm_int[2 * i] = pmx; p.d_pm_int[2 * i + 1] = pmy; }
            } else {
#pragma unroll
                for (int j = 0; j < 6; ++j) o.jc[j] = t0 * D[j] + t1 * D[6 + j];
                ngx = -gx; ngy = -gy;
                if (!LATE_EP) { if (EP_NT_STORE) __builtin_nontemporal_store(e, &p.e_sorted[in.pm]); else p.e_sorted[in.pm] = e; }
            }
        }
    }
    prefetch();
    o.inl = inl; o.pi = pi; o.pmx = pmx; o.pmy = pmy; o.dpx = dpx; o.dpy = dpy; o.e = e;
    if (DUMP) return;

    {
        const double gxn = dpp_shl1(ngx), gyn = dpp_shl1(ngy);
#pragma unroll
        for (int j = 0; j < 6; ++j) o.jp[j] = dpp_shr1(gxn * D[j] + gyn * D[6 + j]);
    }
    o.wr_flag = valid && t >= 1 && !(pw & 0x40000000u);
    if (!LATE_EP && o.wr_flag) {
        if (EP_NT_STORE) __builtin_nontemporal_store((uint8_t)(inl ? 1 : 0), &p.flag[in.pm]); else p.flag[in.pm] = inl ? 1 : 0;
    }

    double v0 = dpx * dpx, v1 = dpx * dpy, v2 = dpy * dpy, v3 = dpx * e, v4 = dpy * e;
    if (p.irls) {
        double w;
        if (p.irls == 2) w = 1.0 / (1.0 + p.eta * e * e);
        else { const double a = fabs(e); w = (a < p.eta) ? 1.0 : p.eta / a; }
        const double ew = w * e;
        v0 = w * v0; v1 = w * v1; v2 = w * v2; v3 = dpx * ew; v4 = dpy * ew;
    }
    if (!inl) { v0 = 0; v1 = 0; v2 = 0; v3 = 0; v4 = 0; }
    o.v0 = v0; o.v1 = v1; o.v2 = v2; o.v3 = v3; o.v4 = v4;
}

template <int STAGE>
__device__ __forceinline__ void store_records(const WarpParams& p, int t, const LaneOut& o, uint32_t slot, unsigned long long inl_mask,
                                              double* s_tile , uint32_t* s_slot )
{
    const int c8 = t & 7;
    if (p.tag && o.inl) p.tag[slot] = __hiloint2double((int)p.stamp, (int)o.pi);
#pragma unroll
    for (int st = 0; st < 64 / STAGE; ++st) {
        const unsigned long long smask = (STAGE == 64) ? inl_mask : ((inl_mask >> (STAGE * st)) & ((1ull << (STAGE & 63)) - 1ull));
        const int n_rec = __popcll(smask);
        if ((t / STAGE) == st && o.inl) {
            const int rk = __popcll(smask & ((1ull << (t % STAGE)) - 1ull));
            double2* w2 = reinterpret_cast<double2*>(s_tile + rk * kRecLds);
            w2[0] = make_double2(o.jc[0], o.jc[1]); w2[1] = make_double2(o.jc[2], o.jc[3]); w2[2] = make_double2(o.jc[4], o.jc[5]);
            w2[3] = make_double2(o.jp[0], o.jp[1]); w2[4] = make_double2(o.jp[2], o.jp[3]); w2[5] = make_double2(o.jp[4], o.jp[5]);
            w2[6] = make_double2(o.dpx, o.dpy);
            w2[7] = make_double2(o.e, __hiloint2double((int)p.stamp, (int)o.pi));
            s_slot[rk] = slot;
        }
        __asm__ volatile("s_waitcnt lgkmcnt(0)" ::: "memory");
        for (int r0 = 0; r0 < n_rec; r0 += 8) {
            const int rr = r0 + (t >> 3);
            if (rr < n_rec && !EMBA_ABL(p.ablate, 2))
            {
                typedef double v2d __attribute__((ext_vector_type(2)));
                v2d* dst = reinterpret_cast<v2d*>(p.rec + (size_t)kRecStride * (EMBA_ABL(p.ablate, 32) ? (s_slot[rr] & 8191u) : s_slot[rr])) + c8;
                const v2d val = reinterpret_cast<const v2d*>(s_tile + rr * kRecLds)[c8];
                if (REC_NT_STORE && p.rec_nt) __builtin_nontemporal_store(val, dst);
                else *dst = val;
            }
        }
        __asm__ volatile("s_waitcnt lgkmcnt(0)" ::: "memory");
    }
}

#ifndef WARP_OCC
#define WARP_OCC
#endif
template <bool DUMP, bool COMPACT, bool SEGPOSE, bool INLINE_SEG>
__device__ __forceinline__ void warp_residual_body(const WarpParams& p, const InlineSegParams* h, const double* knots)
{
    __shared__ __attribute__((aligned(16))) double s_tile[32 * kRecLds];
    static_assert(32 * kRecLds >= 64 * 6 + 32, "the run sums and their pixels must fit the staging tile");
    double* const s_acc = s_tile;
    uint32_t* const s_q = reinterpret_cast<uint32_t*>(s_tile + 64 * 6);
    __shared__ uint32_t s_slot[32];

    const int t = threadIdx.x;
    if (INLINE_SEG && blockIdx.x == 0) inline_seg_produce(*h, knots, t, true);
    const long b = xcd_contiguous_block(blockIdx.x, gridDim.x);
    if (b >= p.nblk) return;
    const long i = b * kWarpNew + t - 1;
    const bool valid = (i >= 0) && (i < p.n_sorted);
    LaneOut o;
    LaneIn in;
    load_event_words<COMPACT, SEGPOSE>(p, i, valid, in);
    if (INLINE_SEG) {
        InlineSegLane is;
        is.rsrc = __builtin_amdgcn_make_buffer_rsrc((void*)h->seg, 0, (int)h->seg_bytes, 0x00020000);
        if (blockIdx.x != 0 && !inline_seg_wait(*h)) {
            inline_seg_produce(*h, knots, t, false);
            if (t == 0) atomicAdd(h->fallbacks, 1u);
        }
        warp_lane<DUMP, COMPACT, NoPrefetch, (WARP_LATE_EP != 0) && !DUMP, SEGPOSE, true>(p, i, in, t, o, NoPrefetch(), &is);
    } else {
        warp_lane<DUMP, COMPACT, NoPrefetch, (WARP_LATE_EP != 0) && !DUMP, SEGPOSE>(p, i, in, t, o);
    }
    if (DUMP) return;
    const bool inl = o.inl;
    const uint32_t pi = o.pi;
    const unsigned long long inl_mask = __ballot(inl);

    __builtin_amdgcn_s_waitcnt(0x0F70);
    store_records<32>(p, t, o, in.slot, inl_mask, s_tile, s_slot);

    double v0 = o.v0, v1 = o.v1, v2 = o.v2, v3 = o.v3, v4 = o.v4;
    int run_n = inl ? 1 : 0;
    const uint32_t key = inl ? pi : (kInvalidPix - (uint32_t)t);
    const bool head = (t == 0) || (key != (uint32_t)dpp_shr1((int)key));
    const bool cont = inl && !head;
    if (__ballot(cont)) {
        const bool deep = cont && (dpp_shr1(cont ? 1 : 0) != 0);
        if (__ballot(deep)) {
            int flag = head ? 1 : 0;
#pragma unroll
            for (int d = 1; d < 64; d <<= 1) {
                const int f_up = __shfl_up(flag, d), n_up = __shfl_up(run_n, d);
                const double a0 = __shfl_up(v0, d), a1 = __shfl_up(v1, d), a2 = __shfl_up(v2, d), a3 = __shfl_up(v3, d), a4 = __shfl_up(v4, d);
                if (t >= d && !flag) { v0 += a0; v1 += a1; v2 += a2; v3 += a3; v4 += a4; run_n += n_up; flag = f_up; }
            }
        } else {
            const int n_up = dpp_shr1(run_n);
            const double a0 = dpp_shr1(v0), a1 = dpp_shr1(v1), a2 = dpp_shr1(v2), a3 = dpp_shr1(v3), a4 = dpp_shr1(v4);
            if (cont) { v0 += a0; v1 += a1; v2 += a2; v3 += a3; v4 += a4; run_n += n_up; }
        }
    }
    const int head_next = dpp_shl1(head ? 1 : 0);
    const bool emit = inl && ((t == 63) || (head_next != 0));
    const unsigned long long emit_mask = __ballot(emit);
    if (emit && !EMBA_ABL(p.ablate, 1)) p.count[pi] = p.marker;
    {
        const int n_emit = __popcll(emit_mask);
        if (emit) {
            const int rk = __popcll(emit_mask & ((1ull << t) - 1ull));
            double* a = s_acc + rk * 6;
            a[0] = v0; a[1] = v1; a[2] = v2; a[3] = v3; a[4] = v4; a[5] = (double)run_n;
            s_q[rk] = pi;
        }
        __asm__ volatile("s_waitcnt lgkmcnt(0)" ::: "memory");
        const int r10 = t / 6, comp = t - 6 * r10;
        for (int g = 0; g < n_emit; g += 10) {
            const int k = g + r10;
            if (t < 60 && k < n_emit && !EMBA_ABL(p.ablate, 8))
                atomicAdd(p.pixacc + (size_t)kPixAccStride * s_q[k] + comp, s_acc[6 * k + comp]);
        }
    }
    if (WARP_LATE_EP) {
        if (inl) { if (EP_NT_STORE) __builtin_nontemporal_store(o.e, &p.e_sorted[in.pm]); else p.e_sorted[in.pm] = o.e; }
        if (o.wr_flag) { if (EP_NT_STORE) __builtin_nontemporal_store((uint8_t)(inl ? 1 : 0), &p.flag[in.pm]); else p.flag[in.pm] = inl ? 1 : 0; }
    }
}

template <bool DUMP, bool COMPACT = false, bool SEGPOSE = false>
__global__ __launch_bounds__(kWarpBlock) WARP_OCC void emba_warp_residual_kernel(WarpParams p)
{
    warp_residual_body<DUMP, COMPACT, SEGPOSE, false>(p, nullptr, nullptr);
}
#ifndef EMBA_INLINE_WARP_OCC
#define EMBA_INLINE_WARP_OCC __attribute__((amdgpu_waves_per_eu(5, 5)))
#endif
__global__ __launch_bounds__(kWarpBlock) EMBA_INLINE_WARP_OCC void emba_warp_residual_inline_kernel(WarpParams p, InlineSegParams h, InlineKnots kn)
{
    warp_residual_body<false, false, true, true>(p, &h, kn.q);
}

template <int kTileW, int kTileH>
__global__ __launch_bounds__(kTileWaves * 64) __attribute__((amdgpu_waves_per_eu(TILE_OCC, TILE_OCC))) void emba_warp_tiled_kernel(WarpParams p)
{
    constexpr int kTilePx = kTileW * kTileH;
    __shared__ double s_sum[6][kTilePx];
    __shared__ __attribute__((aligned(16))) double s_tile[kTileWaves][kTileRecStage * kRecLds];
    __shared__ uint32_t s_slot[kTileWaves][kTileRecStage];
    __shared__ uint16_t s_list[kTileWaves][64];

    const int tid = threadIdx.x, t = tid & 63;
    const int wv = __builtin_amdgcn_readfirstlane(tid >> 6);
    const long c = p.chunks_linear ? (long)blockIdx.x : xcd_contiguous_block(blockIdx.x, gridDim.x);
    if (c >= p.n_chunks) return;
    for (int k = tid; k < 6 * kTilePx; k += kTileWaves * 64) (&s_sum[0][0])[k] = 0.0;
    __syncthreads();
    {
        const ChunkDesc ch = p.chunks[c];
        {
            const long begin = ch.begin, end = ch.end;
            constexpr long kStep = (long)kWarpNew * kTileWaves;
            LaneIn cur, nxt;
            {
                const long g0 = begin + (long)kWarpNew * wv;
                const long i0 = g0 + t - 1;
                load_event_words<true>(p, i0, g0 < end && i0 >= 0 && i0 < end, cur);
                __builtin_amdgcn_s_waitcnt(0x0F70);
            }
#pragma unroll 1
            for (long g0 = begin + (long)kWarpNew * wv; g0 < end; g0 += kStep) {
                const long i = g0 + t - 1;
                auto prefetch = [&]() { const long i1 = i + kStep; load_event_words<true>(p, i1, g0 + kStep < end && i1 < end, nxt); };
                LaneOut o;
                warp_lane<false, true>(p, i, cur, t, o, prefetch);
                const unsigned long long inl_mask = __ballot(o.inl);
                bool outside = false;
                if (o.inl) {
                    const int lx = o.pmx - ch.x0, ly = o.pmy - ch.y0;
                    outside = !(lx >= 0 && lx < kTileW && ly >= 0 && ly < kTileH);
                    if (!outside) {
                        const int q = ly * kTileW + lx;
                        if (!EMBA_ABL(p.ablate, 8)) {
                            atomicAdd(&s_sum[0][q], o.v0); atomicAdd(&s_sum[1][q], o.v1); atomicAdd(&s_sum[2][q], o.v2);
                            atomicAdd(&s_sum[3][q], o.v3); atomicAdd(&s_sum[4][q], o.v4); atomicAdd(&s_sum[5][q], 1.0);
                        }
                    } else {
                        double* a = p.pixacc + (size_t)kPixAccStride * o.pi;
                        p.count[o.pi] = p.marker;
                        atomicAdd(a + 0, o.v0); atomicAdd(a + 1, o.v1); atomicAdd(a + 2, o.v2); atomicAdd(a + 3, o.v3); atomicAdd(a + 4, o.v4); atomicAdd(a + 5, 1.0);
                    }
                }
                {
                    const unsigned long long om = __ballot(outside);
                    if (om && t == 0 && p.err) atomicAdd(p.err, 2 * (int)__popcll(om));
                }
                const uint32_t slot = cur.slot;
                __builtin_amdgcn_s_waitcnt(0x0F70);
                cur = nxt;
                __builtin_amdgcn_sched_barrier(0);
                store_records<kTileRecStage>(p, t, o, slot, inl_mask, s_tile[wv], s_slot[wv]);
            }
        }
        __syncthreads();
        for (int q0 = wv * 64; q0 < kTilePx; q0 += kTileWaves * 64) {
            const int q = q0 + t;
            const bool touched = q < kTilePx && s_sum[5][q] > 0.0;
            const unsigned long long m = __ballot(touched);
            if (!m) continue;
            if (touched) s_list[wv][__popcll(m & ((1ull << t) - 1ull))] = (uint16_t)q;
            __asm__ volatile("s_waitcnt lgkmcnt(0)" ::: "memory");
            const int n_emit = __popcll(m);
            const int r10 = t / 6, comp = t - 6 * r10;
            for (int g = 0; g < n_emit; g += 10) {
                const int k = g + r10;
                if (t < 60 && k < n_emit) {
                    const int qq = s_list[wv][k];
                    const int gy = ch.y0 + qq / kTileW, gx = ch.x0 + qq % kTileW;
                    const size_t pi = (size_t)gy * p.W + gx;
                    if (comp == 0 && !EMBA_ABL(p.ablate, 1)) p.count[pi] = p.marker;
                    if (!EMBA_ABL(p.ablate, 8)) atomicAdd(p.pixacc + (size_t)kPixAccStride * pi + comp, s_sum[comp][qq]);
                }
            }
            __asm__ volatile("s_waitcnt lgkmcnt(0)" ::: "memory");
        }
    }
}

inline void launch_warp_tiled(int shape, dim3 grid, hipStream_t s, const WarpParams& p)
{
    switch (shape) {
    case 1: hipLaunchKernelGGL((emba_warp_tiled_kernel<kTileShapes[1].tw, kTileShapes[1].th>), grid, dim3(kTileWaves * 64), 0, s, p); break;
    case 2: hipLaunchKernelGGL((emba_warp_tiled_kernel<kTileShapes[2].tw, kTileShapes[2].th>), grid, dim3(kTileWaves * 64), 0, s, p); break;
    case 3: hipLaunchKernelGGL((emba_warp_tiled_kernel<kTileShapes[3].tw, kTileShapes[3].th>), grid, dim3(kTileWaves * 64), 0, s, p); break;
    default: hipLaunchKernelGGL((emba_warp_tiled_kernel<kTileShapes[0].tw, kTileShapes[0].th>), grid, dim3(kTileWaves * 64), 0, s, p); break;
    }
}

__device__ __forceinline__ void block_scan_256(const uint32_t* __restrict__ in, uint32_t* __restrict__ out, long n,
                                               uint32_t* __restrict__ total, int* __restrict__ total_host,
                                               const int* __restrict__ err_dev, int* __restrict__ err_host)
{
    __shared__ uint32_t s_wave[4];
    __shared__ uint32_t s_carry;
    const int t = threadIdx.x, lane = t & 63, wv = t >> 6;
    const bool worker = t < 256;
    if (t == 0) s_carry = 0;
    __syncthreads();
    for (long base = 0; base < n; base += 4096) {
        const long i = base + 16 * t;
        uint32_t v[16];
#pragma unroll
        for (int k = 0; k < 16; ++k) v[k] = (worker && i + k < n) ? in[i + k] : 0;
        uint32_t mine = 0;
#pragma unroll
        for (int k = 0; k < 16; ++k) mine += v[k];
        uint32_t x = mine;
#pragma unroll
        for (int o = 1; o < 64; o <<= 1) {
            const uint32_t y = __shfl_up(x, o);
            if (lane >= o) x += y;
        }
        if (worker && lane == 63) s_wave[wv] = x;
        __syncthreads();
        uint32_t woff = 0;
        for (int w = 0; w < wv && w < 4; ++w) woff += s_wave[w];
        const uint32_t carry = s_carry;
        uint32_t run = carry + woff + x - mine;
#pragma unroll
        for (int k = 0; k < 16; ++k) { if (worker && i + k < n) out[i + k] = run; run += v[k]; }
        __syncthreads();
        if (t == 255) s_carry = carry + woff + x;
        __syncthreads();
    }
    if (t == 0) {
        total[0] = s_carry;
        if (total_host) total_host[0] = (int)s_carry;
        if (err_host) err_host[0] = err_dev[0];
    }
}

__global__ __launch_bounds__(256) void emba_scan_kernel(const uint32_t* __restrict__ in, uint32_t* __restrict__ out,
                                                         long n, uint32_t* __restrict__ total, int* __restrict__ total_host,
                                                         const int* __restrict__ err_dev, int* __restrict__ err_host)
{
    block_scan_256(in, out, n, total, total_host, err_dev, err_host);
}

__device__ __forceinline__ uint32_t block_rank_256(bool f, uint32_t* s_w )
{
    const int lane = threadIdx.x & 63, wv = threadIdx.x >> 6;
    const unsigned long long m = __ballot(f);
    const uint32_t within = __popcll(m & ((1ull << lane) - 1ull));
// ... 1366 lines not shown
```

emba_amd/csrc/options_host.h:

```cpp
#pragma once
#include "context.h"

using namespace emba;

namespace {

struct OptionRef { const char* name; int emba_ctx::*field; int lo, hi; bool reorders; };
const OptionRef kOptions[] = {
    {"step_ep", &emba_ctx::step_ep, 0, 2, false},
    {"step_fast", &emba_ctx::step_fast, 0, 1, false},
    {"step_gather", &emba_ctx::step_gather, 0, 3, false},
    {"step_one_set", &emba_ctx::step_one_set, 0, 1, false},
    {"gram_tags", &emba_ctx::use_tags, 0, 1, false},
    {"segpose", &emba_ctx::segpose_mode, 0, 2, false},
    {"order", &emba_ctx::order_mode, 0, 2, true},
    {"texel", &emba_ctx::texel_mode, 0, 3, false},
    {"solve_perm", &emba_ctx::solve_perm_mode, -1, 1, false},
    {"gather_waves", &emba_ctx::opt_gather_waves, 0, 4, false},
    {"chunk_order_bin", &emba_ctx::opt_chunk_order_bin, 0, 1, true},
    {"poison", &emba_ctx::opt_poison, 0, 1, false},
    {"tile_reserve", &emba_ctx::opt_tile_reserve, 0, 5, true},
    {"tile_shape", &emba_ctx::opt_tile_shape, -1, kNumTileShapes - 1, true},
    {"tile_fine", &emba_ctx::opt_tile_fine, -1, 1, true},
    {"tile_min_events", &emba_ctx::opt_tile_min_events, 0, 2000000000, true},
    {"tile_chunk", &emba_ctx::opt_tile_chunk, 0, 1 << 20, true},
    {"solve_counts", &emba_ctx::opt_solve_counts, -1, 2, false},
    {"syrk_dense", &emba_ctx::opt_syrk_dense, 0, 1, false},
    {"syrk_lists", &emba_ctx::opt_syrk_lists, 0, 2, false},
    {"gram_sparse", &emba_ctx::opt_gram_sparse, -1, 1, false},
    {"gram_sparse_chunk", &emba_ctx::opt_gram_sparse_chunk, 1, 8, false},
    {"syrk_min_cols", &emba_ctx::opt_syrk_min_cols, 64, 4096, false},
    {"syrk_item_cap", &emba_ctx::opt_syrk_item_cap, 1, 65536, false},
    {"solve_debug", &emba_ctx::opt_solve_debug, 0, 1, false},
    {"poisson", &emba_ctx::opt_poisson, 0, 2, false},
    {"gemm64", &emba_ctx::opt_gemm64, 0, 1, false},
    {"step_prep", &emba_ctx::step_prep, 0, 1, false},
    {"step_prep_polls", &emba_ctx::step_prep_polls, 0, 1 << 16, false},
    {"contrast_vote", &emba_ctx::opt_contrast_vote, -1, 1, false},
    {"gram_multikey", &emba_ctx::opt_gram_multikey, 0, 1, false},
};

emba_status read_step_prep_fallbacks(emba_ctx* c, int32_t* value)
{
    unsigned n = 0;
    HIP_TRY(c, hipSetDevice(c->device));
    HIP_TRY(c, hipStreamSynchronize(c->stream));
    c->spun = false; c->knots_in_flight = false;
    HIP_TRY(c, hipMemcpy(&n, c->d_seg_flag.as<unsigned>() + 32, sizeof n, hipMemcpyDeviceToHost));
    *value = (int32_t)std::min<unsigned>(n, 0x7FFFFFFFu);
    return EMBA_OK;
}

struct ReadOnlyRef { const char* name; emba_status (*read)(emba_ctx*, int32_t*); };
const ReadOnlyRef kReadOnly[] = {
    {"prep_in_warp", [](emba_ctx* c, int32_t* v) { *v = c->ev.prep_in_warp ? 1 : 0; return EMBA_OK; }},
    {"texels_packed", [](emba_ctx* c, int32_t* v) { *v = c->ev.texels_packed ? 1 : 0; return EMBA_OK; }},
    {"step_prep_fallbacks", read_step_prep_fallbacks},
    {"ep_valid", [](emba_ctx* c, int32_t* v) { *v = c->ev.ep_valid ? 1 : 0; return EMBA_OK; }},
    {"contrast_vote_path", [](emba_ctx* c, int32_t* v) { *v = c->contrast_vote_path; return EMBA_OK; }},
    {"gram_paired", [](emba_ctx* c, int32_t* v) { *v = c->last_gram_paired ? 1 : 0; return EMBA_OK; }},
};

}

extern "C" {

emba_status emba_set_option(emba_ctx* c, const char* name, int32_t value)
{
    if (!c || !name) return EMBA_ERR_INVALID_ARG;
    for (const OptionRef& o : kOptions)
        if (!strcmp(o.name, name)) {
            if (value < o.lo || value > o.hi) return fail(c, EMBA_ERR_INVALID_ARG, "option %s: %d outside [%d, %d]", name, (int)value, o.lo, o.hi);
            c->*(o.field) = (int)value;
            if (o.reorders) c->order.keys_ready = false;
            return EMBA_OK;
        }
    return fail(c, EMBA_ERR_INVALID_ARG, "unknown option '%s'", name);
}

emba_status emba_get_option(emba_ctx* c, const char* name, int32_t* value)
{
    if (!c || !name || !value) return EMBA_ERR_INVALID_ARG;
    for (const ReadOnlyRef& r : kReadOnly)
        if (!strcmp(r.name, name)) return r.read(c, value);
    for (const OptionRef& o : kOptions)
        if (!strcmp(o.name, name)) { *value = c->*(o.field); return EMBA_OK; }
    return fail(c, EMBA_ERR_INVALID_ARG, "unknown option '%s'", name);
}

}
```

emba_amd/csrc/readback_host.h:

```cpp
#pragma once
#include "context.h"

using namespace emba;

extern "C" {

emba_status emba_get_A12_sparse(emba_ctx* c, int32_t* cp_c, int32_t* cp_p, int32_t* pix, double* w, double* jc, double* jp, double* dp)
{
    if (!c) return EMBA_ERR_INVALID_ARG;
    if (!c->eq.accum_done) return fail(c, EMBA_ERR_STATE, "no normal equations formed yet");
    HIP_TRY(c, hipSetDevice(c->device));
    { emba_status st0 = resolve_pending(c); if (st0) return st0; }
    const size_t M = c->win.n_cand;
    if (!M) return EMBA_OK;
    DevBuf b_c, b_p, b_x, b_w, b_jc, b_jp, b_dp;
    emba_status st;
    if ((st = ensure<int32_t>(c, b_c, M)) || (st = ensure<int32_t>(c, b_p, M)) || (st = ensure<int32_t>(c, b_x, M)) || (st = ensure<double>(c, b_w, M)) ||
        (st = ensure<double>(c, b_jc, 6 * M)) || (st = ensure<double>(c, b_jp, 6 * M)) || (st = ensure<double>(c, b_dp, 2 * M)) || (st = ensure_compact(c)))
        return st;
    int32_t *d_c = b_c.as<int32_t>(), *d_p = b_p.as<int32_t>(), *d_x = b_x.as<int32_t>();
    double *d_w = b_w.as<double>(), *d_jc = b_jc.as<double>(), *d_jp = b_jp.as<double>(), *d_dp = b_dp.as<double>();
    hipStream_t s = c->stream;
    hipLaunchKernelGGL(emba_export_a12_kernel, dim3((unsigned)((M + 255) / 256)), dim3(256), 0, s, c->work.rec.as<double>(), c->d_slot_key.as<uint32_t>(), (long)M,
                       c->d_count, c->d_compact.as<int32_t>(), c->eq.thres, c->eq.irls, c->eq.eta, d_c, d_p, d_x, d_w, d_jc, d_jp, d_dp, c->work.stamp);
// ... 22 lines not shown
emba_status emba_get_ep(emba_ctx* c, double* ep_host, size_t cap, size_t* n_inliers)
{
    if (!c || (!ep_host && cap)) return c ? fail(c, EMBA_ERR_INVALID_ARG, "ep_host NULL") : EMBA_ERR_INVALID_ARG;
    if (!c->ev.readable()) return fail(c, EMBA_ERR_STATE, "no evaluateDataError state");
    HIP_TRY(c, hipSetDevice(c->device));
    emba_status st;
    if ((st = resolve_pending(c))) return st;
    if (!c->ev.ep_valid && (st = ensure_inl_idx(c))) return st;
    if (n_inliers) *n_inliers = c->n_inliers;
    if (cap < c->n_inliers) return fail(c, EMBA_ERR_CAPACITY, "cap=%zu < inliers=%zu", cap, c->n_inliers);
    HIP_TRY(c, hipStreamSynchronize(c->stream));
    if (c->n_inliers && (st = d2h_pageable(c, ep_host, c->d_ep.as<double>(), c->n_inliers * sizeof(double)))) return st;
    return EMBA_OK;
}

emba_status emba_get_inlier_pixels(emba_ctx* c, uint32_t* pix_host)
{
    if (!c || !pix_host) return c ? fail(c, EMBA_ERR_INVALID_ARG, "pix_host NULL") : EMBA_ERR_INVALID_ARG;
    if (!c->ev.readable()) return fail(c, EMBA_ERR_STATE, "no evaluateDataError state");
    HIP_TRY(c, hipSetDevice(c->device));
    emba_status st;
    if ((st = resolve_pending(c)) || (st = ensure_inl_idx(c))) return st;
    if (!c->n_inliers) return EMBA_OK;
    if ((st = ensure<uint32_t>(c, c->dl.out, c->n_inliers))) return st;
    uint32_t* d_out = c->dl.out.as<uint32_t>();
    hipLaunchKernelGGL(emba_inlier_pix_kernel, dim3(nblocks(c->win.n_pm)), dim3(256), 0, c->stream, c->d_pm_pix.as<uint32_t>(), c->d_flag.as<uint8_t>(), c->d_inl_idx.as<int32_t>(), (long)c->win.n_pm, d_out);
    HIP_TRY(c, hipGetLastError());
    HIP_TRY(c, hipMemcpyAsync(pix_host, d_out, c->n_inliers * 4, hipMemcpyDeviceToHost, c->stream));
    HIP_TRY(c, hipStreamSynchronize(c->stream));
    return EMBA_OK;
}

emba_status emba_get_inlier_pixel_starts(emba_ctx* c, uint32_t* starts_host)
{
    if (!c || !starts_host) return c ? fail(c, EMBA_ERR_INVALID_ARG, "starts_host NULL") : EMBA_ERR_INVALID_ARG;
    if (!c->ev.readable()) return fail(c, EMBA_ERR_STATE, "no evaluateDataError state");
    HIP_TRY(c, hipSetDevice(c->device));
    emba_status st;
    if ((st = resolve_pending(c)) || (st = ensure_inl_idx(c))) return st;
    const uint32_t S = (uint32_t)((size_t)c->sw * c->sh);
    if ((st = ensure<uint32_t>(c, c->dl.out, std::max<size_t>(c->n_inliers, 1))) || (st = ensure<uint32_t>(c, c->dl.pix_starts, (size_t)S + 1))) return st;
    uint32_t *d_px = c->dl.out.as<uint32_t>(), *d_starts = c->dl.pix_starts.as<uint32_t>();
    if (c->n_inliers) hipLaunchKernelGGL(emba_inlier_pix_kernel, dim3(nblocks(c->win.n_pm)), dim3(256), 0, c->stream, c->d_pm_pix.as<uint32_t>(), c->d_flag.as<uint8_t>(), c->d_inl_idx.as<int32_t>(), (long)c->win.n_pm, d_px);
    hipLaunchKernelGGL(emba_pix_starts_kernel, dim3(nblocks(c->n_inliers + 1)), dim3(256), 0, c->stream, d_px, (long)c->n_inliers, S, d_starts);
    HIP_TRY(c, hipGetLastError());
    HIP_TRY(c, hipMemcpyAsync(starts_host, d_starts, ((size_t)S + 1) * 4, hipMemcpyDeviceToHost, c->stream));
    HIP_TRY(c, hipStreamSynchronize(c->stream));
    c->h_pix_starts.assign(starts_host, starts_host + S + 1);
    c->ev.pix_starts_valid = true;
    return EMBA_OK;
}

emba_status emba_get_ep_by_pixel(emba_ctx* c, double* ep_out, const uint64_t* dst)
{
    if (!c || !ep_out || !dst) return c ? fail(c, EMBA_ERR_INVALID_ARG, "ep_out / dst NULL") : EMBA_ERR_INVALID_ARG;
    if (!c->ev.readable()) return fail(c, EMBA_ERR_STATE, "no evaluateDataError state");
    HIP_TRY(c, hipSetDevice(c->device));
    emba_status st;
    if ((st = resolve_pending(c))) return st;
    const size_t S = (size_t)c->sw * c->sh;
    if (!c->ev.pix_starts_valid || c->h_pix_starts.size() != S + 1) {
        std::vector<uint32_t> tmp(S + 1);
        if ((st = emba_get_inlier_pixel_starts(c, tmp.data()))) return st;
    }
    if (!c->ev.ep_valid && (st = ensure_inl_idx(c))) return st;
    HIP_TRY(c, hipStreamSynchronize(c->stream));
    const uint32_t* starts = c->h_pix_starts.data();
    if ((size_t)starts[S] != c->n_inliers) return fail(c, EMBA_ERR_STATE, "the pixel starts do not belong to this evaluation (%u residuals there, %zu here)", starts[S], c->n_inliers);
    size_t p = 0;
    return d2h_chunks(c, c->d_ep.as<double>(), c->n_inliers * sizeof(double), [&](const void* chunk, size_t off, size_t len) {
        const size_t a = off / sizeof(double), b = (off + len) / sizeof(double);
        while (p < S && (size_t)starts[p + 1] <= a) ++p;
        for (size_t q = p; q < S && (size_t)starts[q] < b; ++q) {
            const size_t lo = std::max<size_t>(starts[q], a), hi = std::min<size_t>(starts[q + 1], b);
            if (hi > lo) std::memcpy(ep_out + dst[q] + (lo - starts[q]), (const double*)chunk + (lo - a), (hi - lo) * sizeof(double));
        }
    });
}

emba_status emba_dump_state(emba_ctx* c, double* pm, double* D, int32_t* cp_idx, int32_t* inlier_idx, int32_t* pm_int, double* dp,
                            double* Gpm, double* temp)
{
    if (!c) return EMBA_ERR_INVALID_ARG;
    if (!c->ev.readable()) return fail(c, EMBA_ERR_STATE, "no evaluateDataError state to dump");
    HIP_TRY(c, hipSetDevice(c->device));
    { emba_status st0 = resolve_pending(c); if (st0) return st0; }
    if (inlier_idx) { emba_status st0 = ensure_inl_idx(c); if (st0) return st0; }
    const size_t ns = c->win.n_sorted, n = c->win.n_in;
    if (!ns) return EMBA_OK;
    hipStream_t s = c->stream;
    const bool w_pm = pm, w_D = D, w_dp = dp, w_G = Gpm, w_t = temp, w_pi = pm_int, w_inl = inlier_idx, w_flag = inlier_idx || pm_int || Gpm || temp;
    DevBuf b_pm, b_D, b_dp, b_G, b_t, b_pi;
    emba_status st = EMBA_OK;
    if ((w_pm && (st = ensure<double>(c, b_pm, 2 * ns))) || (w_D && (st = ensure<double>(c, b_D, 12 * ns))) || (w_dp && (st = ensure<double>(c, b_dp, 2 * ns))) ||
        (w_G && (st = ensure<double>(c, b_G, 2 * ns))) || (w_t && (st = ensure<double>(c, b_t, 2 * ns))) || (w_pi && (st = ensure<int32_t>(c, b_pi, 2 * ns))))
        return st;
    double *d_pm = b_pm.as<double>(), *d_D = b_D.as<double>(), *d_dp = b_dp.as<double>(), *d_G = b_G.as<double>(), *d_t = b_t.as<double>();
    int32_t* d_pi = b_pi.as<int32_t>();
    if (w_dp) (void)hipMemsetAsync(d_dp, 0, 2 * ns * 8, s);
    if (w_G) (void)hipMemsetAsync(d_G, 0, 2 * ns * 8, s);
    if (w_t) (void)hipMemsetAsync(d_t, 0, 2 * ns * 8, s);
    if (w_pi) (void)hipMemsetAsync(d_pi, 0xFF, 2 * ns * 4, s);
    WarpParams p = warp_params(c);
    p.d_pm = d_pm; p.d_D = d_D; p.d_dp = d_dp; p.d_Gpm = d_G; p.d_temp = d_t; p.d_pm_int = d_pi;
    if (c->order.tile_order) hipLaunchKernelGGL((emba_warp_residual_kernel<true, true>), dim3((unsigned)grid8(c->win.nblk)), dim3(kWarpBlock), 0, s, p);
    else if (c->ev.segpose) hipLaunchKernelGGL((emba_warp_residual_kernel<true, false, true>), dim3((unsigned)grid8(c->win.nblk)), dim3(kWarpBlock), 0, s, p);
    else hipLaunchKernelGGL((emba_warp_residual_kernel<true, false>), dim3((unsigned)grid8(c->win.nblk)), dim3(kWarpBlock), 0, s, p);
    std::vector<double> h_pm(w_pm ? 2 * ns : 0), h_D(w_D ? 12 * ns : 0), h_dp(w_dp ? 2 * ns : 0), h_G(w_G ? 2 * ns : 0), h_t(w_t ? 2 * ns : 0);
    std::vector<uint16_t> h_cp(cp_idx ? c->win.n_batch : 0);
    std::vector<int32_t> h_pi(w_pi ? 2 * ns : 0), h_inl(w_inl ? c->win.n_pm : 0);
    std::vector<uint8_t> h_flag(w_flag ? c->win.n_pm : 0);
    if (w_pm) (void)hipMemcpyAsync(h_pm.data(), d_pm, 2 * ns * 8, hipMemcpyDeviceToHost, s);
    if (w_D) (void)hipMemcpyAsync(h_D.data(), d_D, 12 * ns * 8, hipMemcpyDeviceToHost, s);
    if (w_dp) (void)hipMemcpyAsync(h_dp.data(), d_dp, 2 * ns * 8, hipMemcpyDeviceToHost, s);
    if (w_G) (void)hipMemcpyAsync(h_G.data(), d_G, 2 * ns * 8, hipMemcpyDeviceToHost, s);
    if (w_t) (void)hipMemcpyAsync(h_t.data(), d_t, 2 * ns * 8, hipMemcpyDeviceToHost, s);
    if (w_pi) (void)hipMemcpyAsync(h_pi.data(), d_pi, 2 * ns * 4, hipMemcpyDeviceToHost, s);
    if (w_inl) (void)hipMemcpyAsync(h_inl.data(), c->d_inl_idx.as<int32_t>(), c->win.n_pm * 4, hipMemcpyDeviceToHost, s);
    if (w_flag) (void)hipMemcpyAsync(h_flag.data(), c->d_flag.as<uint8_t>(), c->win.n_pm, hipMemcpyDeviceToHost, s);
    if (cp_idx) (void)hipMemcpyAsync(h_cp.data(), c->d_cp.as<uint16_t>(), h_cp.size() * 2, hipMemcpyDeviceToHost, s);
    hipError_t e = hipStreamSynchronize(s);
    if (e != hipSuccess) return fail(c, EMBA_ERR_HIP, "dump_state: %s", hipGetErrorString(e));
    if (cp_idx) for (size_t k = 0; k < n; ++k) cp_idx[k] = -1;
    if (inlier_idx) for (size_t k = 0; k < n; ++k) inlier_idx[k] = -2;
    if (pm_int) for (size_t k = 0; k < 2 * n; ++k) pm_int[k] = -1;
    if (pm) memset(pm, 0, 2 * n * 8);
    if (D) memset(D, 0, 12 * n * 8);
    if (dp) memset(dp, 0, 2 * n * 8);
    if (Gpm) memset(Gpm, 0, 2 * n * 8);
    if (temp) memset(temp, 0, 2 * n * 8);
    std::vector<uint32_t> h_evpix(ns), h_evbatch(cp_idx ? ns : 0), h_evpm(c->order.have_ev_pm ? ns : 0), h_pmorig(c->win.n_pm);
    HIP_TRY(c, hipMemcpy(h_evpix.data(), c->order.d_ev_pix, ns * 4, hipMemcpyDeviceToHost));
    if (cp_idx) HIP_TRY(c, hipMemcpy(h_evbatch.data(), c->order.d_ev_batch, ns * 4, hipMemcpyDeviceToHost));
    if (c->order.have_ev_pm) HIP_TRY(c, hipMemcpy(h_evpm.data(), c->d_ev_pm.as<uint32_t>(), ns * 4, hipMemcpyDeviceToHost));
    HIP_TRY(c, hipMemcpy(h_pmorig.data(), c->d_pm_orig.as<uint32_t>(), c->win.n_pm * 4, hipMemcpyDeviceToHost));
    for (size_t i = 0; i < ns; ++i) {
        if (h_evpix[i] & kEvLead) continue;
        const size_t f = c->order.have_ev_pm ? h_evpm[i] : i;
        const uint32_t k = h_pmorig[f];
        if (k == 0xFFFFFFFFu) continue;
        const bool cand = (h_evpix[i] & kEvHasPred) != 0;
        if (pm) { pm[2 * k] = h_pm[2 * i]; pm[2 * k + 1] = h_pm[2 * i + 1]; }
        if (D) memcpy(D + 12 * (size_t)k, &h_D[12 * i], 12 * 8);
        if (cp_idx) cp_idx[k] = (int32_t)h_cp[h_evbatch[i]];
        if (inlier_idx) inlier_idx[k] = cand ? (h_flag[f] ? h_inl[f] : -1) : -2;
        if (pm_int && h_flag[f]) { pm_int[2 * k] = h_pi[2 * i]; pm_int[2 * k + 1] = h_pi[2 * i + 1]; }
        if (dp && cand) { dp[2 * k] = h_dp[2 * i]; dp[2 * k + 1] = h_dp[2 * i + 1]; }
        if (Gpm && h_flag[f]) { Gpm[2 * k] = h_G[2 * i]; Gpm[2 * k + 1] = h_G[2 * i + 1]; }
        if (temp && h_flag[f]) { temp[2 * k] = h_t[2 * i]; temp[2 * k + 1] = h_t[2 * i + 1]; }
    }
    return EMBA_OK;
}

emba_status emba_last_counts(emba_ctx* c, size_t* n_inliers, size_t* P)
{
    if (!c) return EMBA_ERR_INVALID_ARG;
    HIP_TRY(c, hipSetDevice(c->device));
    emba_status st = resolve_pending(c, true);
    if (st) return st;
    if (n_inliers) *n_inliers = c->n_inliers;
    if (P) *P = c->eq.P;
    return EMBA_OK;
}

emba_status emba_sync(emba_ctx* c)
{
    if (!c) return EMBA_ERR_INVALID_ARG;
    HIP_TRY(c, hipSetDevice(c->device));
    emba_status st = resolve_pending(c);
    if (st) return st;
    HIP_TRY(c, hipStreamSynchronize(c->stream));
    c->spun = false;
    return EMBA_OK;
}

}
```

emba_amd/csrc/step_host.h:

```cpp
#pragma once
#include "context.h"
#include "step_rule.h"

using namespace emba;

namespace {

#define STEP_TRY(call) do { if (const emba_status st_ = (call)) return st_; } while (0)

constexpr GramSizes kGramSizes{kGramBlock, kGramChunk, kGramChunkMin, kEpTailBlk};

emba_status check_irls(emba_ctx* c, int32_t irls)
{
    if (irls < 0 || irls > 2) return fail(c, EMBA_ERR_INVALID_ARG, "irls must be 0 (quadratic), 1 (huber) or 2 (cauchy)");
    return EMBA_OK;
}

bool gram_uses_tags(const emba_ctx* c, bool ep_host) { return gram_tags(c->use_tags, c->order.tile_order, ep_host); }

emba_status ensure_pack(emba_ctx* c, int K)
{
    const PackLayout pack(K);
    if (c->pack_bound) {
        if (c->pack_cap < pack.head)
// ... 92 lines not shown

emba_status resolve_pending(emba_ctx* c, bool counts_only = false)
{
    STEP_TRY(launch_ep_compaction(c));
    if (!c->ev.inl_pending && !c->ev.P_pending) {
        if (c->spun && !counts_only) { HIP_TRY(c, hipStreamSynchronize(c->stream)); c->spun = false; c->knots_in_flight = false; }
        return EMBA_OK;
    }
    STEP_TRY(wait_for_counts(c, counts_only));
    if (c->ev.inl_pending) {
        c->ev.inl_pending = false;
        if (c->h_pinned[1] & 1) return fail(c, EMBA_ERR_TIME_RANGE, "a batch midpoint lies outside the spline's knots");
        c->n_inliers = (size_t)(uint32_t)c->h_pinned[0];
        c->win.n_outside_tile = (size_t)((uint32_t)c->h_pinned[1] >> 1);
        if (tile_rebin_due(c->order.tile_order, c->n_inliers, c->win.n_outside_tile, c->rec_stamp, c->win.last_rebin_stamp)) {
            c->order.keys_ready = false; ++c->win.n_rebin; c->win.last_rebin_stamp = c->rec_stamp;
        }
        c->ev.done = true;
    }
    if (c->ev.P_pending) {
        c->ev.P_pending = false;
        c->eq.P = (size_t)(uint32_t)c->h_pinned[2];
        c->win.P_prev = c->eq.P;
        c->eq.pack_len = PackLayout(c->eq.K).len(c->eq.P);
        if (c->eq.pack_len > c->pack_cap)
            return fail(c, EMBA_ERR_CAPACITY, "pack buffer too small: need %zu doubles, have %zu", c->eq.pack_len, c->pack_cap);
        c->eq.active_done = true;
    }
    return EMBA_OK;
}

}

extern "C" emba_status emba_bind_exchange_buffers(emba_ctx* c, int32_t* count_map_dev, double* pack_dev, size_t pack_cap)
{
    if (!c) return EMBA_ERR_INVALID_ARG;
    c->d_count = count_map_dev ? count_map_dev : c->d_count_own.as<int32_t>();
    c->ev.count_stamp = 0;
    c->pix.bound();
    if (pack_dev) { c->d_pack = pack_dev; c->pack_cap = pack_cap; c->pack_bound = true; }
    else { c->pack_bound = false; c->d_pack = c->d_pack_own.as<double>(); c->pack_cap = c->d_pack_own.bytes / sizeof(double); }
    return EMBA_OK;
}

extern "C" emba_status emba_count_compress(emba_ctx* c, uint8_t* u8_dev, int32_t cap)
{
    if (!c || !u8_dev || cap < 1 || cap > 255) return c ? fail(c, EMBA_ERR_INVALID_ARG, "count_compress: bad arguments") : EMBA_ERR_INVALID_ARG;
    if (!c->ev.launched) return fail(c, EMBA_ERR_STATE, "emba_eval_launch has not been called");
    if (c->pix.counts_raw()) {
        counts_materialised(c);
        hipLaunchKernelGGL(emba_count_materialise_compress_kernel, dim3((unsigned)((c->npix + 2047) / 2048)), dim3(256), 0, c->stream, c->d_count, c->d_pixacc.as<double>(), (long)c->npix,
                           c->pix.marker(), (int)cap, u8_dev);
    } else {
        hipLaunchKernelGGL(emba_count_compress_kernel, dim3((unsigned)((c->npix + 1023) / 1024)), dim3(256), 0, c->stream, c->d_count, (long)c->npix, (int)cap, u8_dev);
    }
    HIP_TRY(c, hipGetLastError());
    return EMBA_OK;
}

extern "C" emba_status emba_count_expand(emba_ctx* c, const uint8_t* u8_dev)
{
    if (!c || !u8_dev) return c ? fail(c, EMBA_ERR_INVALID_ARG, "count_expand: NULL") : EMBA_ERR_INVALID_ARG;
    if (!c->ev.launched) return fail(c, EMBA_ERR_STATE, "emba_eval_launch has not been called");
    c->ev.count_stamp = 0;
    hipLaunchKernelGGL(emba_count_expand_kernel, dim3((unsigned)((c->npix + 1023) / 1024)), dim3(256), 0, c->stream, u8_dev, (long)c->npix, c->d_count);
    HIP_TRY(c, hipGetLastError());
    return EMBA_OK;
}

extern "C" emba_status emba_count_map_ready(emba_ctx* c)
{
    if (!c) return EMBA_ERR_INVALID_ARG;
    HIP_TRY(c, hipSetDevice(c->device));
    return ensure_counts(c);
}


namespace {

emba_status eval_checks_and_buffers(emba_ctx* c, const double* knots, int32_t K, int64_t t0_ns, int64_t dt_ns)
{
    if (!knots) return fail(c, EMBA_ERR_INVALID_ARG, "knots NULL");
    if (!c->win.have_events) return fail(c, EMBA_ERR_STATE, "emba_set_events has not been called");
    if (!c->map.state().resident()) return fail(c, EMBA_ERR_STATE, "no map: call emba_upload_map or emba_bind_map_dev");
    HIP_TRY(c, hipSetDevice(c->device));
    STEP_TRY(ensure<double>(c, c->d_knots, (size_t)4 * K));
    STEP_TRY(ensure<double>(c, c->d_seg, (size_t)kSegStride * K));
    STEP_TRY(prepare_order(c, knots, t0_ns, dt_ns, K));
    STEP_TRY(ensure_pack(c, K));
    if (c->h_knots_cap < K) {
        if (c->h_knots) (void)hipHostFree(c->h_knots);
        HIP_TRY(c, hipHostMalloc((void**)&c->h_knots, (size_t)4 * K * sizeof(double), hipHostMallocMapped));
        HIP_TRY(c, hipHostGetDevicePointer((void**)&c->h_knots_dev, c->h_knots, 0));
        c->h_knots_cap = K;
    }
    return EMBA_OK;
}

emba_status set_equations_aside(emba_ctx* c)
{
    if (c->ev.P_pending || c->ev.inl_pending) STEP_TRY(resolve_pending(c, true));
    if (!c->alt.rec.p) STEP_TRY(size_record_set(c, c->alt, c->win.n_cand));
    std::swap(c->work, c->alt);
    c->eq_saved = c->eq;
    c->eq_in_alt = true;
    return EMBA_OK;
}

emba_status clear_on_first_use(emba_ctx* c)
{
    if (!c->pix.first_use()) return EMBA_OK;
    HIP_TRY(c, hipMemsetAsync(c->d_count, 0, c->npix * sizeof(int32_t), c->stream));
    HIP_TRY(c, hipMemsetAsync(c->d_pixacc.as<double>(), 0, c->npix * kPixAccStride * sizeof(double), c->stream));
    c->pix.first_use_cleared();
    return EMBA_OK;
}

emba_status stage_knots(emba_ctx* c, const double* knots, int32_t K, PrepPoseTexelParams& q, InlineKnots& kn)
{
    hipStream_t s = c->stream;
    q.knots_dev = c->d_knots.as<double>();
    q.knots_out = c->d_knots.as<double>();
    q.inline_knots = (K <= kInlineKnots) ? 1 : 0;
    if (q.inline_knots) { memcpy(kn.q, knots, (size_t)4 * K * sizeof(double)); return EMBA_OK; }
    if (c->knots_in_flight) HIP_TRY(c, hipStreamSynchronize(s));
    memcpy(c->h_knots, knots, (size_t)4 * K * sizeof(double));
    HIP_TRY(c, hipMemcpyAsync(c->d_knots.as<double>(), c->h_knots, (size_t)4 * K * sizeof(double), hipMemcpyHostToDevice, s));
    c->knots_in_flight = true;
    return EMBA_OK;
}

emba_status launch_prep_pose_texel(emba_ctx* c, const double* knots, int32_t K, int64_t t0_ns, int64_t dt_ns)
{
    hipStream_t s = c->stream;
    const int n_prep_blk = prep_blocks(c->pix.lines_clean(), c->win.n_sorted, c->npix);
    c->ev.use_texel = hessian_source(c->texel_mode, c->win.n_sorted, c->npix);
    PrepPoseTexelParams q{};
    InlineKnots kn;
    const int nb = (int)c->win.n_batch;
    ++c->eval_seq;
    c->d_err = c->d_err2.as<int>() + (c->eval_seq & 1u);
    q.count = c->d_count; q.npix = (long)c->npix; q.pixacc = c->d_pixacc.as<double>();
    q.W = c->W; q.H = c->H;
    q.n_prep = n_prep_blk;
    q.batch_t_ns = c->d_batch_t.as<int64_t>(); q.nb = nb;
    q.K = (int)K; q.t0_ns = t0_ns; q.dt_ns = dt_ns;
    q.pose = c->d_pose.as<double>();
    q.err = c->d_err;
    q.err_next = c->d_err2.as<int>() + ((c->eval_seq + 1u) & 1u);
    c->ev.segpose = segpose_in_pixel_order(c->order.tile_order, c->segpose_mode);
    const bool seg_records = c->order.tile_order || c->ev.segpose;
    q.n_pose = ((seg_records ? (int)K - 1 : nb) + 63) / 64;
    q.seg = seg_records ? c->d_seg.as<double>() : nullptr;
    const MapState& map = c->map.state();
    const bool stale = texels_stale(map.reads_own_memory(), map.version(), map.packed_version(), ((volatile int*)c->h_pinned)[5], c->seq);
    q.n_tex = texel_blocks(c->ev.use_texel, stale);
    if (q.n_tex) c->map.texels_packed();
    c->ev.texels_packed = q.n_tex != 0;
    q.Gx = c->map.Gx(); q.Gy = c->map.Gy();
    q.rect = c->d_rect.as<int>(); q.rect_packed = c->d_rect.as<int>() + 4;
    q.texel = c->d_texel.as<double>();
    if (c->kernel_timing && c->kt_all) { HIP_TRY(c, hipEventRecord(c->kt[4], s)); c->kt_valid[c->kt_slot][2] = true; }
    c->ev.prep_in_warp = prep_inside_warp(c->step_prep, c->order.tile_order, c->ev.segpose, (int)K, kInlineKnots, c->win.n_sorted, n_prep_blk, q.n_tex, c->ev.use_texel);
    if (c->ev.prep_in_warp) {
        memcpy(c->seg_knots.q, knots, (size_t)4 * K * sizeof(double));
        InlineSegParams& h = c->seg_inline;
        h.seg = c->d_seg.as<double>(); h.seg_bytes = (unsigned)((size_t)kSegStride * (K - 1) * sizeof(double));
        if (++c->seg_seq == 0) ++c->seg_seq;
        h.flag = c->d_seg_flag.as<unsigned>(); h.seq = c->seg_seq;
        h.K = (int)K; h.polls = c->step_prep_polls;
        h.fallbacks = c->d_seg_flag.as<unsigned>() + 32;
        h.err_next = q.err_next; h.knots_out = c->d_knots.as<double>();
        return EMBA_OK;
    }
    STEP_TRY(stage_knots(c, knots, K, q, kn));
    if (q.n_pose + q.n_tex + q.n_prep == 0) q.n_prep = 1;
    hipLaunchKernelGGL(emba_prep_pose_texel_kernel, dim3((unsigned)(q.n_pose + q.n_tex + q.n_prep)), dim3(256), 0, s, q, kn);
    return EMBA_OK;
}

WarpParams warp_params(emba_ctx* c)
{
    WarpParams p{};
    p.ev_pix = c->order.d_ev_pix; p.ev_batch = c->order.d_ev_batch; p.ev_slot = c->d_ev_slot.as<uint32_t>();
    p.ev_pm = c->order.tile_order ? c->d_ev_pm.as<uint32_t>() : nullptr;
    p.n_sorted = (long)c->win.n_sorted; p.nblk = c->win.nblk;
    p.ev_u = c->d_ev_u.as<double>(); p.ev_seg = c->d_ev_seg.as<uint16_t>();
    p.pose = c->d_pose.as<double>(); p.seg = c->d_seg.as<double>(); p.lut = c->d_lut.as<double>();
    p.W = c->W; p.H = c->H;
    p.Gx = c->map.Gx(); p.Gy = c->map.Gy();
    p.fx = c->fx; p.fy = c->fy; p.cx = c->cx; p.cy = c->cy;
    p.C_th = c->C_th; p.outlier_px = c->outlier_px;
    p.count = c->d_count; p.pixacc = c->d_pixacc.as<double>();
    p.rec = c->work.rec.as<double>();
    p.e_sorted = c->d_e_sorted.as<double>(); p.flag = c->d_flag.as<uint8_t>();
    return p;
}

emba_status launch_warp(emba_ctx* c, const EvalOpts& opt)
{
    hipStream_t s = c->stream;
    const bool tile = c->order.tile_order;
    WarpParams p = warp_params(c);
    p.texel = c->ev.use_texel ? c->d_texel.as<double>() : nullptr;
    p.rect_acc = (c->ev.use_texel == 3) ? c->d_rect.as<int>() + 4 : nullptr;
    p.tag = (c->use_tags && !tile) ? c->work.tag.as<double>() : nullptr;
    p.rec_nt = records_non_temporal(tile, c->win.n_cand, kRecStride) ? 1 : 0;
    p.err = c->d_err;
    p.ablate = c->ablate;
    p.irls = opt.irls; p.eta = opt.eta;
    p.stamp = ++c->rec_stamp;
    c->work.stamp = p.stamp;
    p.marker = count_marker(p.stamp);
    c->pix.marked(p.marker);
    p.chunks = c->d_chunks.as<ChunkDesc>(); p.n_chunks = c->order.n_chunks; p.chunks_linear = c->order.chunks_lpt ? 1 : 0;
    if (c->kernel_timing) HIP_TRY(c, hipEventRecord(c->kt[0], s));
    if (tile) launch_warp_tiled(c->order.tile_shape, dim3((unsigned)grid8(c->order.n_chunks)), s, p);
    else if (c->ev.prep_in_warp) hipLaunchKernelGGL(emba_warp_residual_inline_kernel, dim3((unsigned)grid8(c->win.nblk)), dim3(kWarpBlock), 0, s, p, c->seg_inline, c->seg_knots);
    else if (c->ev.segpose) hipLaunchKernelGGL((emba_warp_residual_kernel<false, false, true>), dim3((unsigned)grid8(c->win.nblk)), dim3(kWarpBlock), 0, s, p);
    else hipLaunchKernelGGL(emba_warp_residual_kernel<false>, dim3((unsigned)grid8(c->win.nblk)), dim3(kWarpBlock), 0, s, p);
    if (c->kernel_timing) { HIP_TRY(c, hipEventRecord(c->kt[1], s)); c->kt_warp_valid = true; c->kt_valid[c->kt_slot][0] = true; }
    return EMBA_OK;
}

emba_status eval_launch(emba_ctx* c, const double* knots, int32_t K, int64_t t0_ns, int64_t dt_ns, const EvalOpts& opt)
{
    STEP_TRY(eval_checks_and_buffers(c, knots, K, t0_ns, dt_ns));
    if (c->eq.accum_done && !opt.keep_alt_set) STEP_TRY(set_equations_aside(c));
    c->eq.K = K;
    c->eq.active_done = c->eq.accum_done = false;
    begin_evaluation(c);
    STEP_TRY(clear_on_first_use(c));
    STEP_TRY(launch_prep_pose_texel(c, knots, K, t0_ns, dt_ns));
    if (c->ev.use_texel == 1)
        hipLaunchKernelGGL(emba_texel_kernel, dim3((c->W + 255) / 256, c->H), dim3(256), 0, c->stream, c->map.Gx(), c->map.Gy(), c->H, c->W, c->d_texel.as<double>());
    if (c->win.n_sorted) STEP_TRY(launch_warp(c, opt));
    else c->pix.not_marked();
    HIP_TRY(c, hipGetLastError());
    c->ev.acc_irls = opt.irls; c->ev.acc_eta = opt.eta;
    c->ev.launched = true;
    return EMBA_OK;
}

}

extern "C" emba_status emba_eval_launch(emba_ctx* c, const double* knots, int32_t K, int64_t t0_ns, int64_t dt_ns)
{
    return c ? eval_launch(c, knots, K, t0_ns, dt_ns, EvalOpts{c->cost_irls, c->cost_eta, false}) : EMBA_ERR_INVALID_ARG;
}

extern "C" emba_status emba_eval_finish(emba_ctx* c, double* ep_out, size_t* n_inliers, int32_t* num_ev_map_out)
{
    if (!c) return EMBA_ERR_INVALID_ARG;
    if (!c->ev.launched) return fail(c, EMBA_ERR_STATE, "emba_eval_launch has not been called");
    HIP_TRY(c, hipSetDevice(c->device));
    c->ev.ep_deferred = true;
    if (!ep_out && !n_inliers && !num_ev_map_out) return EMBA_OK;
    STEP_TRY(resolve_pending(c));
    if (n_inliers) *n_inliers = c->n_inliers;
    if (ep_out && c->n_inliers) { HIP_TRY(c, hipStreamSynchronize(c->stream)); STEP_TRY(d2h_pageable(c, ep_out, c->d_ep.as<double>(), c->n_inliers * sizeof(double))); }
    if (num_ev_map_out) {
        STEP_TRY(ensure_counts(c));
        HIP_TRY(c, hipStreamSynchronize(c->stream));
        STEP_TRY(d2h_pageable(c, num_ev_map_out, c->d_count, c->npix * sizeof(int32_t)));
    }
    return EMBA_OK;
}

extern "C" emba_status emba_eval_data_error(emba_ctx* c, const double* knots, int32_t K, int64_t t0_ns, int64_t dt_ns, const double* Gx,
                                            const double* Gy, int32_t eval_deriv, double* ep_out, size_t* n_inliers,
                                            int32_t* num_ev_map_out)
{
    if (!c) return EMBA_ERR_INVALID_ARG;
    if (!eval_deriv) return fail(c, EMBA_ERR_INVALID_ARG, "eval_deriv=false is never used by the reference (solver.cpp:75,251) and is not provided");
    if (Gx || Gy) STEP_TRY(emba_upload_map(c, Gx, Gy));
    STEP_TRY(emba_eval_launch(c, knots, K, t0_ns, dt_ns));
    return emba_eval_finish(c, ep_out, n_inliers, num_ev_map_out);
}


namespace {

void fill_active_write(emba_ctx* c, int32_t thres, const FormOpts& opt, ActiveWriteParams& aw)
{
    const PackLayout pack(c->eq.K);
    aw.count = c->d_count; aw.npix = (long)c->npix; aw.thres = thres;
    aw.blk_off = c->d_ablk_off.as<uint32_t>(); aw.n_ablk = (long)c->n_ablk;
    aw.compact = nullptr;
    aw.active_idx = c->d_active.as<uint32_t>(); aw.active_bits = c->d_active_bits.as<uint8_t>();
    aw.pixacc = c->d_pixacc.as<double>();
    aw.A22b2 = pack_A22b2(c); aw.alpha = opt.fused_alpha;
    aw.pack_head = c->d_pack; aw.head_len = (long)pack.head;
    aw.max_P = (long)pack.max_P(c->pack_cap);
    aw.Gx = c->map.Gx(); aw.Gy = c->map.Gy();
    aw.ablate = c->ablate;
    if (c->eq.force_generic_a22) { aw.A22b2 = nullptr; aw.alpha = 0.0; }
}

emba_status expand_global_counts(emba_ctx* c, const uint8_t* global_u8)
{
    STEP_TRY(ensure_counts(c));
    c->ev.count_stamp = 0;
    hipLaunchKernelGGL(emba_count_expand_kernel, dim3((unsigned)((c->npix + 1023) / 1024)), dim3(256), 0, c->stream, global_u8, (long)c->npix, c->d_count);
    return EMBA_OK;
}

void launch_post_warp_a(emba_ctx* c, int32_t thres, const FormOpts& opt, const uint8_t* global_u8, bool lists_ok, ActiveWriteParams& aw, bool* lists)
{
    PostWarpParams q{};
    q.count = c->d_count; q.npix = (long)c->npix; q.thres = thres;
    q.ablk_cnt = c->d_ablk_cnt.as<uint32_t>(); q.ablk_off = c->d_ablk_off.as<uint32_t>(); q.n_ablk = (long)c->n_ablk;
    q.total_P = c->d_total.as<uint32_t>() + 1; q.total_P_host = c->h_pinned_dev + 2;
    q.fblk_cnt = c->d_fblk_cnt.as<uint32_t>(); q.fblk_off = c->d_fblk_off.as<uint32_t>(); q.n_fblk = c->win.n_fblk;
    q.perm = nullptr; q.n_pm = (long)c->win.n_pm;
    q.total_inl = c->d_total.as<uint32_t>(); q.total_inl_host = c->h_pinned_dev;
    q.err_dev = c->d_err; q.err_host = c->h_pinned_dev + 1;
    q.e_sorted = c->d_e_sorted.as<double>(); q.flag = c->d_flag.as<uint8_t>(); q.ep = c->d_ep.as<double>();
    q.inl_idx = nullptr;
    q.seq = ++c->seq; q.seq_host = c->h_pinned_dev + 3;
    c->ev.seq_armed = true;
    if (c->pix.counts_raw()) {
        q.raw_count = c->d_count; q.pixacc = c->d_pixacc.as<double>(); q.marker = c->pix.marker();
        counts_materialised(c);
    }
    const bool consume = opt.consume && c->step_fast && !c->eq.force_generic_a22;
    q.global_u8 = global_u8;
    *lists = gather_uses_lists(lists_ok, q.raw_count != nullptr, q.global_u8 != nullptr);
    if (consume) { aw.clear_pixacc = c->d_pixacc.as<double>(); c->pix.consumed_by_gather(); }
    if (*lists) {
        q.seg = c->d_seg_act.as<uint16_t>(); aw.seg = c->d_seg_act.as<uint16_t>();
        if (consume) q.clear_inactive = c->d_pixacc.as<double>();
    }
    const size_t fsup_len = (size_t)c->win.n_fsup * kFlagSupStride;
    c->post.fsup_half ^= 1;
    q.fsup = c->d_fsup.as<uint32_t>() + (size_t)c->post.fsup_half * fsup_len;
    q.fsup_next = c->d_fsup.as<uint32_t>() + (size_t)(c->post.fsup_half ^ 1) * fsup_len;
    q.n_sup = c->win.n_fsup;
    q.active_bits = c->d_active_bits.as<uint8_t>(); q.pack_head = c->d_pack; q.head_len = aw.head_len;
    aw.bits_head_done = 1;
    q.blk_rect = c->d_blk_rect.as<int>(); q.W = c->W;
    aw.blk_rect = c->d_blk_rect.as<int>(); aw.rect_out = c->d_rect.as<int>();
    aw.rect_packed = c->d_rect.as<int>() + 4; aw.fresh_host = c->h_pinned_dev + 5;
    hipLaunchKernelGGL(emba_post_warp_a_kernel, dim3((unsigned)(c->n_ablk + c->win.n_fblk)), dim3(256), 0, c->stream, q);
    aw.blk_cnt = c->d_ablk_cnt.as<uint32_t>(); aw.fblk_cnt = c->d_fblk_cnt.as<uint32_t>(); aw.n_fblk = c->win.n_fblk;
    aw.total_P = q.total_P; aw.total_P_host = q.total_P_host;
    aw.total_inl = q.total_inl; aw.total_inl_host = q.total_inl_host;
    aw.err_dev = q.err_dev; aw.err_host = q.err_host;
    aw.seq = q.seq; aw.seq_host = q.seq_host;
}

void launch_or_defer_active_set(emba_ctx* c, const FormOpts& opt, bool lists, const ActiveWriteParams& aw)
{
    c->post.gather_deferred = false;
    c->ev.ep_in_gram = opt.wants_ep && c->step_ep != 2 && c->win.n_cand;
    c->ev.ep_after_gram = opt.wants_ep && !c->ev.ep_in_gram;
    if (gather_rides_in_gram(lists, c->step_gather)) c->post.defer(aw);
    else if (lists) hipLaunchKernelGGL(emba_active_gather_kernel, dim3(1024), dim3(256), 0, c->stream, aw);
    else hipLaunchKernelGGL(emba_active_write_kernel, dim3((unsigned)c->n_ablk), dim3(256), 0, c->stream, aw);
    c->ev.inl_pending = true;
}

emba_status launch_active_set_sweeping(emba_ctx* c, int32_t thres, const ActiveWriteParams& aw)
{
    hipStream_t s = c->stream;
    STEP_TRY(launch_ep_compaction(c));
    STEP_TRY(ensure_counts(c));
    hipLaunchKernelGGL(emba_active_count_kernel, dim3((unsigned)c->n_ablk), dim3(256), 0, s, c->d_count, (long)c->npix, (int)thres, c->d_ablk_cnt.as<uint32_t>());
    hipLaunchKernelGGL(emba_scan_kernel, dim3(1), dim3(256), 0, s, c->d_ablk_cnt.as<uint32_t>(), c->d_ablk_off.as<uint32_t>(), (long)c->n_ablk, c->d_total.as<uint32_t>() + 1,
                       c->h_pinned_dev + 2, (const int*)nullptr, (int*)nullptr);
    hipLaunchKernelGGL(emba_active_write_kernel, dim3((unsigned)c->n_ablk), dim3(256), 0, s, aw);
// ... 299 lines not shown
```

emba_amd/csrc/step_rule.h:

```cpp
#pragma once
#include <stddef.h>
#include <stdint.h>

#include <algorithm>
#include <vector>

#if defined(__HIPCC__)
#define EMBA_RULE_HD __host__ __device__
#else
#define EMBA_RULE_HD
#endif

namespace emba {

struct PackLayout {
    size_t b1, A22b2, head;
    explicit PackLayout(int K) : b1((size_t)9 * K * K), A22b2(b1 + (size_t)3 * K), head(A22b2) {}
    size_t len(size_t P) const { return head + 5 * P; }
    size_t need(size_t npix) const { return len(npix); }
    size_t max_P(size_t cap) const { return (cap - head) / 5; }
};

inline int hessian_source(int texel_mode, size_t n_sorted, size_t npix)
{
    return texel_mode == 1 ? 1 : texel_mode == 2 ? 0 : texel_mode == 3 ? 3 : (n_sorted > 4 * npix ? 1 : 3);
}

inline bool segpose_in_pixel_order(bool tile_order, int segpose_mode) { return !tile_order && (segpose_mode ? segpose_mode == 2 : true); }

constexpr int kRectMargin = 24;
constexpr int kRectFreshSlack = 12;
static_assert(kRectFreshSlack <= kRectMargin, "texels exist only inside the packed box grown by kRectMargin");
EMBA_RULE_HD inline bool rect_contained(int nx0, int ny0, int nx1, int ny1, int px0, int py0, int px1, int py1, int slack)
{
    if (nx1 < nx0 || ny1 < ny0) return true;
    if (px1 < px0 || py1 < py0) return false;
    return nx0 >= px0 - slack && ny0 >= py0 - slack && nx1 <= px1 + slack && ny1 <= py1 + slack;
}
inline bool texels_stale(bool map_owned, uint32_t map_version, uint32_t packed_version, int verdict_seq, int step_seq)
{
    return !map_owned || map_version != packed_version || step_seq == 0 || verdict_seq != step_seq;
}
inline int texel_blocks(int hessian_src, bool stale) { return (hessian_src == 3 && stale) ? 1024 : 0; }

inline bool prep_inside_warp(int step_prep, bool tile_order, bool segpose, int K, int inline_knots, size_t n_sorted, int n_prep_blk, int n_tex_blk, int hessian_src)
{
    return step_prep != 0 && !tile_order && segpose && K <= inline_knots && n_sorted > 0 && n_prep_blk == 0 && n_tex_blk == 0 && hessian_src != 1;
}

inline int prep_blocks(bool lines_clean, size_t n_sorted, size_t npix) { return (lines_clean && n_sorted) ? 0 : (int)((npix + 1023) / 1024); }

constexpr size_t kRecCachedBytes = (size_t)144 << 20;
inline bool records_non_temporal(bool tile_order, size_t n_cand, int rec_stride) { return tile_order || n_cand * (size_t)(rec_stride * 8) > kRecCachedBytes; }

constexpr size_t kGatherTileMaxCand = 3500000;
inline bool gather_lists_ok(bool consume, int step_gather, bool a22_from_records, long n_ablk, long gather_max_units, size_t n_cand, bool tile_order)
{
    return consume && step_gather && !a22_from_records && n_ablk <= gather_max_units && n_cand && (step_gather == 3 || !tile_order || n_cand <= kGatherTileMaxCand);
}
inline bool gather_uses_lists(bool lists_ok, bool counts_raw, bool global_bytes) { return lists_ok && (counts_raw || global_bytes); }
inline bool global_counts_need_expanding(bool lists_ok, bool ep_deferred, size_t n_sorted, bool counts_raw) { return !(lists_ok && ep_deferred && n_sorted && !counts_raw); }
inline bool gather_rides_in_gram(bool lists, int step_gather) { return lists && step_gather >= 2; }

inline bool gram_tags(int use_tags, bool tile_order, bool ep_host) { return use_tags && !tile_order && !ep_host; }

inline bool gram_sparse(bool tags, int opt_gram_sparse, size_t P_prev, size_t n_cand, int thres)
{
    return tags && (opt_gram_sparse == 1 || (opt_gram_sparse < 0 && P_prev > 0 && n_cand >= (2u << 20) && 16ull * (size_t)thres * P_prev < n_cand));
}

inline int gather_waves(int opt_gather_waves) { return (opt_gather_waves == 1 || opt_gather_waves == 2 || opt_gather_waves == 4) ? opt_gather_waves : 4; }

struct GramSizes { int block, chunk, chunk_min, ep_tail_blk; };

struct GramPlan { int chunk; long waves; int n_gram_blocks; unsigned ep_tail_blocks, grid; int gather_waves; };
inline GramPlan gram_plan(size_t n_cand, bool sparse, int opt_gram_sparse_chunk, int n_cu, bool ep_tail, size_t n_pm, int opt_gather_waves, const GramSizes& k)
{
    GramPlan g{};
    const long chunk_cap = sparse ? (long)opt_gram_sparse_chunk * k.chunk : k.chunk;
    const long per_round = (long)n_cu * (k.block / 64);
    const long rounds = std::max<long>(1, ((long)n_cand + per_round * chunk_cap - 1) / (per_round * chunk_cap));
    long chunk = ((long)n_cand + per_round * rounds - 1) / (per_round * rounds);
    chunk = (chunk + 7) & ~7L;
    chunk = std::min<long>(std::max<long>(chunk, k.chunk_min), chunk_cap);
    g.chunk = (int)chunk;
    g.waves = ((long)n_cand + chunk - 1) / chunk;
    const long wpb = k.block / 64;
    g.grid = (unsigned)((g.waves + wpb - 1) / wpb);
    g.n_gram_blocks = (int)g.grid;
    if (ep_tail) {
        g.ep_tail_blocks = (unsigned)((n_pm + k.ep_tail_blk - 1) / k.ep_tail_blk);
        g.grid += g.ep_tail_blocks;
    }
    g.gather_waves = gather_waves(opt_gather_waves);
    return g;
}

constexpr uint32_t kGramMaxRuns = 4096;
inline bool gram_paired(int opt_multikey, bool tags, bool sparse, bool tile_order, bool runs_known, bool records_nt)
{
    return !opt_multikey && tags && !sparse && !tile_order && runs_known && !records_nt;
}
struct GramPairPlan { int share; long waves; int n_gram_blocks; };
inline GramPairPlan gram_pair_cuts(const uint32_t* run_start, size_t n_runs, size_t n_cand, int n_sw, const GramPlan& base, const GramSizes& k, std::vector<uint32_t>& cuts)
{
    const long wpb = k.block / 64;
    const long slots = (long)base.n_gram_blocks * n_sw;
    const long share_max = ((wpb * k.chunk + n_sw - 1) / n_sw + 7) & ~7L;
    auto run_len = [&](size_t r) { return (long)((r + 1 < n_runs ? run_start[r + 1] : (uint32_t)n_cand) - run_start[r]); };
    auto waves_at = [&](long share) { long n = 0; for (size_t r = 0; r < n_runs; ++r) n += (run_len(r) + share - 1) / share; return n; };
    long share = (((long)n_cand + slots - 1) / std::max<long>(slots, 1) + 7) & ~7L;
    share = std::min(std::max<long>(share, k.chunk_min), share_max);
    while (share < share_max && waves_at(share) > slots) share += 8;
    GramPairPlan g{};
    g.share = (int)share;
    g.waves = waves_at(share);
    g.n_gram_blocks = (int)std::max<long>(1, (g.waves + n_sw - 1) / n_sw);
    cuts.assign((size_t)g.n_gram_blocks * wpb * 2, 0u);
    long w = 0;
    for (size_t r = 0; r < n_runs; ++r) {
        const long len = run_len(r), n = (len + share - 1) / share;
        const long each = n ? (((len + n - 1) / n + 7) & ~7L) : 0;
        for (long i = 0; i < n; ++i, ++w) {
            const size_t at = (size_t)((w / n_sw) * wpb + w % n_sw) * 2;
            cuts[at] = run_start[r] + (uint32_t)std::min(i * each, len);
            cuts[at + 1] = run_start[r] + (uint32_t)std::min((i + 1) * each, len);
        }
    }
    return g;
}

inline bool tile_rebin_due(bool tile_order, size_t n_inliers, size_t n_outside_tile, uint32_t rec_stamp, uint32_t last_rebin_stamp)
{
    return tile_order && n_inliers && n_outside_tile * 5 > n_inliers && rec_stamp - last_rebin_stamp >= 3;
}

}
```

emba_amd/legm.py:

```python
import ctypes as C
from dataclasses import dataclass

import numpy as np

from . import _lib
from ._lib import EmbaCfg, EmbaError

_dp, _i32p, _u32p = _lib._dp, _lib._i32p, _lib._u32p
_u16p, _u8p, _i64p = _lib._u16p, _lib._u8p, _lib._i64p

COST_TYPES = {"quadratic": 0, "huber": 1, "cauchy": 2}
POISSON_BOUNDARIES = {"dirichlet": 0, "wrap": 1}


def poisson_boundary(boundary):
    if boundary not in POISSON_BOUNDARIES:
        raise ValueError(f"boundary must be 'dirichlet' or 'wrap', not {boundary!r}")
    return POISSON_BOUNDARIES[boundary]


def _p(a, ty):
    return None if a is None else a.ctypes.data_as(ty)


# ... 791 lines not shown

    def solveMapOnly(self, lam, resident_x2=False):
        self.last_counts()
        x2 = None if resident_x2 else np.zeros(2 * max(self._P, 1))
        self._check(self._L.emba_solve_map_only(self._ctx, float(lam), None if resident_x2 else _p(x2, _dp)))
        return np.zeros(3 * self.K), (None if resident_x2 else x2[:2 * self._P])

    def solvePosesOnly(self, lam, fix_first_pose=False):
        x1 = np.zeros(3 * self.K)
        self._check(self._L.emba_solve_poses_only(self._ctx, float(lam), 1 if fix_first_pose else 0, _p(x1, _dp)))
        return x1, None

    def last_solve_info(self):
        v = C.c_int32(0)
        self._check(self._L.emba_last_solve_info(self._ctx, C.byref(v)))
        return v.value

    def solve_shard_size(self):
        n = C.c_size_t(0)
        self._check(self._L.emba_solve_shard_size(self._ctx, C.byref(n)))
        return n.value

    def solve_shard_count(self, n_ranks):
        counts = np.zeros(n_ranks, dtype=np.uint64)
        self._check(self._L.emba_solve_shard_count(self._ctx, int(n_ranks), counts.ctypes.data_as(_lib._szp)))
        return counts.astype(np.int64)

    def solve_shard_pack(self, n_ranks, send_ptr):
        self._check(self._L.emba_solve_shard_pack(self._ctx, int(n_ranks), C.c_void_p(send_ptr)))

    def solve_shard_cached(self, rank, n_ranks):
        f, n = C.c_int32(0), C.c_size_t(0)
        self._check(self._L.emba_solve_shard_cached(self._ctx, int(rank), int(n_ranks), C.byref(f), C.byref(n)))
        return int(n.value) if f.value else None

    def cg_shard_size(self):
        n = C.c_size_t(0)
        self._check(self._L.emba_cg_shard_size(self._ctx, C.byref(n)))
        return n.value

    def cg_shard_begin(self, rank, n_ranks, recv_ptr, n_recv, lam, fix_first_pose, red_ptr):
        self._check(self._L.emba_cg_shard_begin(self._ctx, int(rank), int(n_ranks), C.c_void_p(recv_ptr), int(n_recv), float(lam), 1 if fix_first_pose else 0, C.c_void_p(red_ptr)))

    def cg_shard_apply(self, red_ptr):
        self._check(self._L.emba_cg_shard_apply(self._ctx, C.c_void_p(red_ptr)))

    def cg_shard_pt(self, red_ptr):
        v = C.c_double(0)
        self._check(self._L.emba_cg_shard_pt(self._ctx, C.c_void_p(red_ptr), C.byref(v)))
        return v.value

    def cg_shard_update(self, alpha, red_ptr):
        self._check(self._L.emba_cg_shard_update(self._ctx, float(alpha), C.c_void_p(red_ptr)))

    def cg_shard_direction(self, beta):
        self._check(self._L.emba_cg_shard_direction(self._ctx, float(beta)))

    def cg_shard_end(self, x2_full_ptr):
        x1 = np.zeros(3 * self.K)
        self._check(self._L.emba_cg_shard_end(self._ctx, _p(x1, _dp), C.c_void_p(x2_full_ptr)))
        return x1

    def solve_shard_partial(self, rank, n_ranks, recv_ptr, n_recv, lam, S_ptr):
        self._check(self._L.emba_solve_shard_partial(self._ctx, int(rank), int(n_ranks), C.c_void_p(recv_ptr), int(n_recv), float(lam), C.c_void_p(S_ptr)))

    def solve_shard_finish(self, rank, n_ranks, recv_ptr, n_recv, lam, fix_first_pose, S_ptr, x2_ptr):
        x1 = np.zeros(3 * self.K)
        self._check(self._L.emba_solve_shard_finish(self._ctx, int(rank), int(n_ranks), C.c_void_p(recv_ptr), int(n_recv), float(lam),
                                                    1 if fix_first_pose else 0, C.c_void_p(S_ptr), _p(x1, _dp), C.c_void_p(x2_ptr)))
        return x1

    def solveNormalEqCG(self, lam, fix_first_pose=False, max_iter=100, tol=1e-6, resident_x2=False):
        self.last_counts()
        x1 = np.zeros(3 * self.K)
        x2 = None if resident_x2 else np.zeros(2 * max(self._P, 1))
        it = C.c_int32(0); err = C.c_double(0)
        self._check(self._L.emba_solve_normal_eq_cg(self._ctx, float(lam), 1 if fix_first_pose else 0, int(max_iter), float(tol), _p(x1, _dp),
                                                    None if resident_x2 else _p(x2, _dp), C.byref(it), C.byref(err)))
        return x1, (None if resident_x2 else x2[:2 * self._P]), it.value, err.value

    def updateMap(self, x2, damping_factor):
        if x2 is None:
            self._check(self._L.emba_update_map(self._ctx, None, float(damping_factor)))
        elif isinstance(x2, int):
            self._check(self._L.emba_update_map_dev(self._ctx, C.c_void_p(x2), float(damping_factor)))
        else:
            x2 = np.ascontiguousarray(x2, dtype=np.float64)
            self._check(self._L.emba_update_map(self._ctx, _p(x2, _dp), float(damping_factor)))

    def acceptMap(self):
        self._check(self._L.emba_map_accept(self._ctx))

    def rejectMap(self):
        self._check(self._L.emba_map_reject(self._ctx))

    def rejectTrial(self):
        self._check(self._L.emba_trial_reject(self._ctx))

    def downloadMap(self):
        Gx = np.empty((self.H, self.W)); Gy = np.empty((self.H, self.W))
        self._check(self._L.emba_download_map(self._ctx, _p(Gx, _dp), _p(Gy, _dp)))
        return Gx, Gy

    def set_cost(self, cost_type="quadratic", a=0.0):
        self._check(self._L.emba_set_cost(self._ctx, COST_TYPES[cost_type], float(a)))

    def reconstructIntensity(self, Gx=None, Gy=None, download=True, boundary="dirichlet"):
        bc = poisson_boundary(boundary)
        if (Gx is None) != (Gy is None):
            raise ValueError("pass both Gx and Gy, or neither")
        if Gx is not None:
            Gx = np.ascontiguousarray(Gx, dtype=np.float64); Gy = np.ascontiguousarray(Gy, dtype=np.float64)
            if Gx.shape != (self.H, self.W) or Gy.shape != (self.H, self.W):
                raise ValueError("Gx/Gy must be pano_height x pano_width float64")
        M = np.empty((self.H, self.W)) if download else None
        self._check(self._L.emba_reconstruct_intensity_bc(self._ctx, _p(Gx, _dp), _p(Gy, _dp), _p(M, _dp), bc))
        return M

    def renderMapImages(self, pct=0.1, poisson=True, boundary="dirichlet"):
        bc = poisson_boundary(boundary)
        H, W = self.H, self.W
        gx, gy = np.empty((H, W), np.uint8), np.empty((H, W), np.uint8)
        rgb = np.empty((H, W, 3), np.uint8)
        mp = np.empty((H, W), np.uint8) if poisson else None
        self._check(self._L.emba_render_map_images_bc(self._ctx, float(pct), _p(gx, _u8p), _p(gy, _u8p), _p(rgb, _u8p), _p(mp, _u8p), bc))
        return {"Gx": gx, "Gy": gy, "G_hsv": rgb, "map_poisson": mp}

    def normalizeRobust(self, img, pct=0.1, with_range=False):
        a = np.ascontiguousarray(img, dtype=np.float64)
        out = np.empty(a.shape, np.uint8)
        rmin, rmax = C.c_double(), C.c_double()
        self._check(self._L.emba_normalize_robust(self._ctx, _p(a, _dp), a.size, float(pct), _p(out, _u8p), C.byref(rmin), C.byref(rmax)))
        return (out, (rmin.value, rmax.value)) if with_range else out

    def A12_sparse(self):
        _, M = self.event_counts()
        out = dict(cp_c=np.zeros(M, np.int32), cp_p=np.zeros(M, np.int32), pix=np.zeros(M, np.int32), w=np.zeros(M),
                   jc=np.zeros((M, 6)), jp=np.zeros((M, 6)), dp=np.zeros((M, 2)))
        self._check(self._L.emba_get_A12_sparse(self._ctx, _p(out["cp_c"], _i32p), _p(out["cp_p"], _i32p), _p(out["pix"], _i32p),
                                                _p(out["w"], _dp), _p(out["jc"], _dp), _p(out["jp"], _dp), _p(out["dp"], _dp)))
        return out

    def dump_state(self, fields=None):
        n = self.n_events
        shapes = dict(pm=((n, 2), np.float64), D=((n, 2, 6), np.float64), cp_idx=((n,), np.int32), inlier_idx=((n,), np.int32),
                      pm_int=((n, 2), np.int32), dp=((n, 2), np.float64), Gpm=((n, 2), np.float64), temp=((n, 2), np.float64))
        want = list(shapes) if fields is None else list(fields)
        d = {k: np.zeros(shapes[k][0], shapes[k][1]) for k in want}
        g = lambda k, ty: _p(d[k], ty) if k in d else None
        self._check(self._L.emba_dump_state(self._ctx, g("pm", _dp), g("D", _dp), g("cp_idx", _i32p), g("inlier_idx", _i32p),
                                            g("pm_int", _i32p), g("dp", _dp), g("Gpm", _dp), g("temp", _dp)))
        return d

    def upload_map(self, Gx, Gy):
        Gx = np.ascontiguousarray(Gx, dtype=np.float64); Gy = np.ascontiguousarray(Gy, dtype=np.float64)
        self._check(self._L.emba_upload_map(self._ctx, _p(Gx, _dp), _p(Gy, _dp)))
        self._check(self._L.emba_sync(self._ctx))

    def bind_map_dev(self, gx_ptr, gy_ptr):
        self._check(self._L.emba_bind_map_dev(self._ctx, C.c_void_p(gx_ptr), C.c_void_p(gy_ptr)))

    def bind_exchange_buffers(self, count_ptr, pack_ptr, pack_cap):
        self._check(self._L.emba_bind_exchange_buffers(self._ctx, C.c_void_p(count_ptr) if count_ptr else None,
                                                       C.c_void_p(pack_ptr) if pack_ptr else None, int(pack_cap)))

    def count_map_ready(self):
        self._check(self._L.emba_count_map_ready(self._ctx))

    def count_compress(self, u8_ptr, cap):
        self._check(self._L.emba_count_compress(self._ctx, C.c_void_p(u8_ptr), int(cap)))

    def count_expand(self, u8_ptr):
        self._check(self._L.emba_count_expand(self._ctx, C.c_void_p(u8_ptr)))

    def eval_launch(self, traj):
        knots = np.ascontiguousarray(traj.knots_xyzw, dtype=np.float64).reshape(-1, 4)
        self.K = knots.shape[0]
        self._keep = [knots]
        self._check(self._L.emba_eval_launch(self._ctx, _p(knots, _dp), self.K, int(traj.t0_ns), int(traj.dt_ns)))

    def eval_finish(self, want_ep=False, want_map=False, sync=True):
        if not sync and not want_ep and not want_map:
            self._check(self._L.emba_eval_finish(self._ctx, None, None, None))
            return None, None, None
        n_inl = C.c_size_t(0)
        ep = np.empty(max(self.n_events, 1)) if want_ep else None
        nem = np.empty((self.H, self.W), dtype=np.int32) if want_map else None
        self._check(self._L.emba_eval_finish(self._ctx, _p(ep, _dp), C.byref(n_inl), _p(nem, _i32p)))
        return n_inl.value, (ep[:n_inl.value] if want_ep else None), nem

    def form_active(self, thres, sync=True):
        if not sync:
            self._check(self._L.emba_form_active(self._ctx, int(thres), None, None))
            return None, None
        P, pl = C.c_size_t(0), C.c_size_t(0)
        self._check(self._L.emba_form_active(self._ctx, int(thres), C.byref(P), C.byref(pl)))
        self._P = P.value
        return P.value, pl.value

    def step_form_active(self, thres, global_u8_ptr=None):
        self._check(self._L.emba_step_form_active(self._ctx, int(thres), C.c_void_p(global_u8_ptr) if global_u8_ptr else None))

    def form_accumulate(self, cost_type="quadratic", a=0.0):
        self._check(self._L.emba_form_accumulate(self._ctx, None, COST_TYPES[cost_type], float(a)))

    def form_finish(self, alpha, download=False, dense_A12=False):
        if download:
            self.last_counts()
            return self._finish(alpha, dense_A12)
        self._check(self._L.emba_form_finish(self._ctx, float(alpha), None, None, None, 0, None, None, None))
        return None

    def last_counts(self):
        a, b = C.c_size_t(0), C.c_size_t(0)
        self._check(self._L.emba_last_counts(self._ctx, C.byref(a), C.byref(b)))
        self._P = b.value
        return a.value, b.value

    def step(self, traj, thres_valid_pixel, alpha, cost_type="quadratic", a=0.0):
        if getattr(self, "_step_traj", None) is not traj:
            self._step_knots = np.ascontiguousarray(traj.knots_xyzw, dtype=np.float64).reshape(-1, 4)
            self._step_traj = traj
        knots = self._step_knots
        self.K = knots.shape[0]
        a_, b_ = C.c_size_t(0), C.c_size_t(0)
        self._check(self._L.emba_step(self._ctx, _p(knots, _dp), self.K, int(traj.t0_ns), int(traj.dt_ns), int(thres_valid_pixel),
                                      COST_TYPES[cost_type], float(a), float(alpha), C.byref(a_), C.byref(b_)))
        self._P = b_.value
        return a_.value, b_.value

    def get_ep(self):
        n = C.c_size_t(0)
        ep = np.empty(max(int(self.n_events), 1), dtype=np.float64)
        self._check(self._L.emba_get_ep(self._ctx, _p(ep, _dp), ep.size, C.byref(n)))
        return ep[: n.value].copy()

    def set_option(self, name, value):
        self._check(self._L.emba_set_option(self._ctx, name.encode(), int(value)))

    def get_option(self, name):
        v = C.c_int32(0)
        self._check(self._L.emba_get_option(self._ctx, name.encode(), C.byref(v)))
        return v.value

    def compact_ep(self):
        self._check(self._L.emba_compact_ep(self._ctx))

    def sync(self):
        self._check(self._L.emba_sync(self._ctx))

    def timer_start(self, slot=0):
        self._check(self._L.emba_timer_start(self._ctx, slot))

    def timer_stop(self, slot=0):
        self._check(self._L.emba_timer_stop(self._ctx, slot))

    def timer_ms(self, slot=0):
        ms = C.c_float(0)
        self._check(self._L.emba_timer_elapsed_ms(self._ctx, slot, C.byref(ms)))
        return ms.value

    def enable_kernel_timing(self, on=True, slot=0):
        self._check(self._L.emba_enable_kernel_timing(self._ctx, (1 + int(slot)) if on else 0))

    def kernel_ms_slot(self, slot):
        a, b = C.c_float(0), C.c_float(0)
        self._check(self._L.emba_kernel_ms_slot(self._ctx, int(slot), C.byref(a), C.byref(b)))
        return a.value, b.value

    def last_kernel_ms(self):
        a, b = C.c_float(0), C.c_float(0)
        self._check(self._L.emba_last_kernel_ms(self._ctx, C.byref(a), C.byref(b)))
        return a.value, b.value

    def kernel_timing_all(self, on=True):
        self._check(self._L.emba_kernel_timing_all(self._ctx, 1 if on else 0))

    def kernel_ms_all(self, slot):
        v = (C.c_float * 4)()
        self._check(self._L.emba_kernel_ms_all(self._ctx, int(slot), v))
        return [float(x) for x in v]

    def bracket_overhead_us(self, reps=50):
        us = C.c_float(0)
        self._check(self._L.emba_bracket_overhead_us(self._ctx, int(reps), C.byref(us)))
        return us.value

    def clock_probe(self):
        sclk, us, ratio = C.c_double(0), C.c_double(0), C.c_double(0)
        cr, mr, wr = C.c_int32(0), C.c_int32(0), C.c_int32(0)
        self._check(self._L.emba_clock_probe(self._ctx, C.byref(sclk), C.byref(us), C.byref(ratio), C.byref(cr), C.byref(mr), C.byref(wr)))
        return {"sclk_mhz_measured": sclk.value, "probe_us": us.value, "cycles_per_dependent_add": ratio.value,
                "attr_clock_rate_khz": cr.value, "attr_mem_clock_rate_khz": mr.value, "attr_wall_clock_rate_khz": wr.value}

    def pci_bus_id(self):
        buf = C.create_string_buffer(32)
        self._check(self._L.emba_device_pci_bus_id(self._ctx, buf, 32))
        return buf.value.decode()
```

include/emba_hip.h:

```cpp
#ifndef EMBA_HIP_H
#define EMBA_HIP_H

#include <stddef.h>
#include <stdint.h>

#ifdef __cplusplus
extern "C" {
#endif

#define EMBA_ABI_VERSION 2

typedef enum {
    EMBA_OK = 0,
    EMBA_ERR_INVALID_ARG = 1,
    EMBA_ERR_NO_DEVICE = 2,
    EMBA_ERR_HIP = 3,
    EMBA_ERR_TIME_RANGE = 4,
    EMBA_ERR_STATE = 5,
    EMBA_ERR_CAPACITY = 6,
    EMBA_ERR_NUMERIC = 7
} emba_status;

typedef struct emba_ctx emba_ctx;

typedef struct {
    int32_t sensor_w, sensor_h;
    int32_t pano_w, pano_h;
    const double* bearing_lut;
    double C_th;
    int32_t event_batch;
    double outlier_px;
    int32_t device;
    void* stream;
} emba_cfg;

int emba_abi_version(void);
const char* emba_build_info(void);

emba_status emba_create(const emba_cfg* cfg, emba_ctx** out);
void emba_destroy(emba_ctx* ctx);
const char* emba_last_error(const emba_ctx* ctx);

emba_status emba_set_events(emba_ctx* ctx, const uint16_t* x, const uint16_t* y, const uint8_t* pol,
                            const int64_t* t_ns, size_t n,
                            const uint16_t* halo_x, const uint16_t* halo_y,
                            const int64_t* halo_batch_t_ns, size_t n_halo);

emba_status emba_set_events_dev(emba_ctx* ctx, const uint16_t* x_dev, const uint16_t* y_dev, const uint8_t* pol_dev,
                                const int64_t* t_ns_dev, size_t n,
                                const uint16_t* halo_x_dev, const uint16_t* halo_y_dev,
                                const int64_t* halo_batch_t_ns_dev, size_t n_halo);

emba_status emba_last_setup_ms(const emba_ctx* ctx, double* set_events_ms, double* prepare_ms, int32_t* tile_order,
                               size_t* n_entries, size_t* n_chunks);

emba_status emba_last_order_stats(const emba_ctx* ctx, double* events_per_pano_px, double* lead_in_frac);
emba_status emba_last_order_inlier_estimate(const emba_ctx* ctx, double* inlier_frac);
emba_status emba_last_tile_geometry(const emba_ctx* ctx, int32_t* tile_w, int32_t* tile_h, int32_t* pitch_x, int32_t* pitch_y, int32_t* reserve);

emba_status emba_last_tile_drift(const emba_ctx* ctx, size_t* n_outside, int32_t* n_rebin);

emba_status emba_event_counts(const emba_ctx* ctx, size_t* n_used, size_t* n_candidates);


emba_status emba_eval_data_error(emba_ctx* ctx, const double* knots_xyzw, int32_t K, int64_t t0_ns,
                                 int64_t dt_ns, const double* Gx, const double* Gy, int32_t eval_deriv,
                                 double* ep_out, size_t* n_inliers, int32_t* num_ev_map_out);

emba_status emba_form_normal_eq(emba_ctx* ctx, const double* ep, int32_t thres_valid_pixel,
                                int32_t irls, double eta, double alpha, double* A11, double* b1,
                                size_t* P, uint32_t* active_idx, size_t cap_P, double* A22, double* b2,
                                double* A12_dense);

emba_status emba_get_A12_sparse(emba_ctx* ctx, int32_t* cp_c, int32_t* cp_p, int32_t* pix, double* w,
                                double* jc , double* jp , double* dp );

emba_status emba_compact_ep(emba_ctx* ctx);
emba_status emba_get_ep(emba_ctx* ctx, double* ep_host, size_t cap, size_t* n_inliers);

emba_status emba_get_inlier_pixels(emba_ctx* ctx, uint32_t* pix_host);
emba_status emba_get_inlier_pixel_starts(emba_ctx* ctx, uint32_t* starts_host);
emba_status emba_get_ep_by_pixel(emba_ctx* ctx, double* ep_out, const uint64_t* dst);

emba_status emba_data_cost(emba_ctx* ctx, int32_t irls, double eta, double* cost);
emba_status emba_reg_cost(emba_ctx* ctx, double alpha, double* cost);
emba_status emba_costs(emba_ctx* ctx, int32_t irls, double eta, double alpha, double* data_cost, double* reg_cost);
emba_status emba_costs_launch(emba_ctx* ctx, int32_t irls, double eta, int32_t with_reg);
emba_status emba_costs_finish(emba_ctx* ctx, int32_t irls, double eta, double alpha, double* data_cost, double* reg_cost);

emba_status emba_dump_state(emba_ctx* ctx, double* pm, double* D, int32_t* cp_idx, int32_t* inlier_idx,
                            int32_t* pm_int, double* dp, double* Gpm, double* temp);


emba_status emba_upload_map(emba_ctx* ctx, const double* Gx_host, const double* Gy_host);
emba_status emba_bind_map_dev(emba_ctx* ctx, const double* Gx_dev, const double* Gy_dev);

emba_status emba_update_map(emba_ctx* ctx, const double* x2_host, double damping);
emba_status emba_update_map_dev(emba_ctx* ctx, const double* x2_dev, double damping);
emba_status emba_map_accept(emba_ctx* ctx);
emba_status emba_map_reject(emba_ctx* ctx);
emba_status emba_trial_reject(emba_ctx* ctx);
emba_status emba_download_map(emba_ctx* ctx, double* Gx_host, double* Gy_host);
emba_status emba_get_map_active(emba_ctx* ctx, double* gxy_host, size_t cap_P);

emba_status emba_reconstruct_intensity(emba_ctx* ctx, const double* Gx_host, const double* Gy_host, double* M_host);
#define EMBA_POISSON_DIRICHLET 0
#define EMBA_POISSON_WRAP_X 1
emba_status emba_reconstruct_intensity_bc(emba_ctx* ctx, const double* Gx_host, const double* Gy_host, double* M_host, int boundary);

emba_status emba_render_map_images(emba_ctx* ctx, double pct_discard, uint8_t* gx_u8, uint8_t* gy_u8, uint8_t* rgb_u8, uint8_t* poisson_u8);
emba_status emba_render_map_images_bc(emba_ctx* ctx, double pct_discard, uint8_t* gx_u8, uint8_t* gy_u8, uint8_t* rgb_u8, uint8_t* poisson_u8, int boundary);
emba_status emba_normalize_robust(emba_ctx* ctx, const double* src_host, size_t n, double pct_discard, uint8_t* dst_host, double* rmin, double* rmax);

emba_status emba_seq_upload(emba_ctx* ctx, const uint16_t* x, const uint16_t* y, const uint8_t* pol, const int64_t* t_ns, size_t n,
                            int32_t sampling_rate, size_t* n_kept);
emba_status emba_seq_size(const emba_ctx* ctx, size_t* n);
emba_status emba_seq_free(emba_ctx* ctx);
emba_status emba_seq_window(emba_ctx* ctx, int64_t t_beg_ns, int64_t t_end_ns, size_t* beg, size_t* end);
emba_status emba_set_events_seq(emba_ctx* ctx, size_t beg, size_t end);
emba_status emba_set_events_seq_shard(emba_ctx* ctx, size_t win_beg, size_t lo, size_t hi);
emba_status emba_seq_halo(emba_ctx* ctx, size_t win_beg, size_t lo, uint16_t* hx, uint16_t* hy, int64_t* hbt, size_t cap, size_t* n_halo);
emba_status emba_seq_get(emba_ctx* ctx, size_t beg, size_t end, uint16_t* x, uint16_t* y, uint8_t* pol, int64_t* t_ns);

emba_status emba_seq_filter(emba_ctx* ctx, double hot_sigma, int64_t refractory_ns, int64_t support_ns, int32_t sampling_rate, uint64_t* stats);
emba_status emba_seq_hot_pixels(emba_ctx* ctx, uint8_t* mask_host);

emba_status emba_seq_cmax(emba_ctx* ctx, int64_t slice_events, double omega_max, double* omega_out, int64_t* t_ref_ns_out, uint64_t* j0_out, uint64_t* j_out,
                          int32_t* evals_out, size_t cap_slices, size_t* n_slices);
emba_status emba_seq_cmax_objective(emba_ctx* ctx, size_t beg, size_t end, const double* omega, size_t M, uint64_t* j_out, uint32_t* iwe_out, int32_t* grid_w,
                                    int32_t* grid_h, int32_t* shift);

emba_status emba_seq_event_panorama(emba_ctx* ctx, size_t beg, size_t end, const double* knots_xyzw, int32_t K, int64_t t0_ns, int64_t dt_ns,
                                    int32_t signed_polarity, int32_t* image_out, uint64_t* j_out, int64_t* sum_out, uint64_t* nonzero_out,
                                    uint64_t* dropped_out, double* pm_out);

emba_status emba_seq_contrast_gradient(emba_ctx* ctx, size_t beg, size_t end, const double* knots_xyzw, int32_t K, int64_t t0_ns, int64_t dt_ns,
                                       int32_t signed_polarity, double* j_out, double* grad_out , double* image_out ,
                                       uint64_t* dropped_out, double* pm_out , double* d_out ,
                                       int32_t* cp_out );

emba_status emba_seq_contrast_gradient_level(emba_ctx* ctx, size_t beg, size_t end, const double* knots_xyzw, int32_t K, int64_t t0_ns, int64_t dt_ns,
                                             int32_t signed_polarity, int32_t level, double* j_out, double* grad_out ,
                                             double* image_out , uint64_t* dropped_out, double* pm_out ,
                                             double* d_out , int32_t* cp_out );

emba_status emba_seq_contrast_prior_add(emba_ctx* ctx, size_t beg, size_t end, const double* knots_xyzw, int32_t K, int64_t t0_ns, int64_t dt_ns,
                                        int32_t signed_polarity, uint32_t level_mask, size_t* n_added, uint64_t* dropped_out );
emba_status emba_seq_contrast_prior_set(emba_ctx* ctx, int32_t level, const double* image_host );
emba_status emba_seq_contrast_prior_get(emba_ctx* ctx, int32_t level, double* image_host , int32_t* present);
emba_status emba_seq_contrast_prior_clear(emba_ctx* ctx);
emba_status emba_seq_contrast_gradient_prior(emba_ctx* ctx, size_t beg, size_t end, const double* knots_xyzw, int32_t K, int64_t t0_ns, int64_t dt_ns,
                                             int32_t signed_polarity, int32_t level, double prior_weight, double* j_out, double* grad_out ,
                                             double* image_out , uint64_t* dropped_out, double* pm_out ,
                                             double* d_out , int32_t* cp_out );

emba_status emba_render_views(emba_ctx* ctx, const double* plane_host , int boundary, const int64_t* frame_t_ns, size_t F,
                              const double* knots_xyzw, int32_t K, int64_t t0_ns, int64_t dt_ns, double fill, double lo, double hi,
                              double* views_out , uint8_t* views_u8 , uint64_t* outside_out ,
                              double* pm_out );
emba_status emba_seq_event_frames(emba_ctx* ctx, size_t beg, size_t end, const int64_t* edge_t_ns , size_t F,
                                  int32_t signed_polarity, int32_t* frames_out , uint64_t* before_out, uint64_t* after_out);

emba_status emba_mosaic_frames(emba_ctx* ctx, const uint8_t* frames , const int64_t* frame_t_ns, size_t F,
                               const double* knots_xyzw, int32_t K, int64_t t0_ns, int64_t dt_ns, int32_t skip_zero, int32_t accumulate,
                               uint64_t* dropped_out, uint64_t* skipped_out, double* pm_out );
emba_status emba_mosaic_get(emba_ctx* ctx, uint64_t min_weight, double fill, uint64_t* sum_w_out, uint64_t* sum_v_out, double* mean_out,
                            uint8_t* covered_out, uint64_t* n_covered_out);
emba_status emba_mosaic_map(emba_ctx* ctx, uint64_t min_weight, double lo, double hi, double eps, int32_t take_log,
                            double* L_out, double* Gx_out, double* Gy_out , int32_t make_resident);
emba_status emba_mosaic_clear(emba_ctx* ctx);

emba_status emba_simulate_events(emba_ctx* ctx, const double* plane_host , int boundary, const int64_t* step_t_ns , size_t F,
                                 const double* knots_xyzw, int32_t K, int64_t t0_ns, int64_t dt_ns, double c_on, double c_off, int32_t max_per_step,
                                 uint64_t max_events, uint64_t* stats );
emba_status emba_sim_size(const emba_ctx* ctx, size_t* n);
emba_status emba_sim_get(emba_ctx* ctx, size_t beg, size_t end, uint16_t* x, uint16_t* y, uint8_t* pol, int64_t* t_ns);
emba_status emba_seq_from_sim(emba_ctx* ctx, int32_t sampling_rate, size_t* n_kept);

#define EMBA_ALIGN_RUNNING 0
#define EMBA_ALIGN_CONVERGED 1
#define EMBA_ALIGN_STALLED 2
#define EMBA_ALIGN_ITERATIONS 3
#define EMBA_ALIGN_DEGENERATE 4
typedef struct {
    int32_t max_iters, min_pixels;
    double lambda0, lambda_up, lambda_down, lambda_min, lambda_max, tol_rot, huber_k;
} emba_align_settings;
emba_status emba_frames_align_eval(emba_ctx* ctx, const uint8_t* frames , size_t F, const double* q_xyzw ,
                                   const double* plane_host , const uint8_t* valid_host , int32_t use_mosaic,
                                   uint64_t min_weight, double fill, double lo, double hi, int32_t skip_zero, double huber_k,
                                   double* sums_out , uint64_t* counts_out , double* pm_out ,
                                   double* resid_out );
emba_status emba_frames_align(emba_ctx* ctx, const uint8_t* frames , size_t F, const double* q_xyzw ,
                              const double* plane_host , const uint8_t* valid_host , int32_t use_mosaic,
                              uint64_t min_weight, double fill, double lo, double hi, int32_t skip_zero, const emba_align_settings* settings,
                              double* q_out , double* sums_out , uint64_t* counts_out , int32_t* status_out ,
                              int32_t* iters_out , double* cost0_out , uint64_t* n0_out );

#define EMBA_TRACK_ANCHOR 1
#define EMBA_TRACK_TRACKED 2
#define EMBA_TRACK_LOST 3
typedef struct {
    int32_t n_levels, levels[8], batch, predict, skip_zero;
    uint64_t min_weight;
    double min_overlap;
    emba_align_settings align;
} emba_track_settings;
emba_status emba_frames_track(emba_ctx* ctx, const uint8_t* frames , const int64_t* frame_t_ns , size_t F, const double* q0_xyzw ,
                              const emba_track_settings* settings, double* q_out , int32_t* status_out , int32_t* iters_out ,
                              double* cost_out , uint64_t* counts_out , double* overlap_out , uint64_t* stats_out ,
                              double* pm_out );
emba_status emba_track_eval(emba_ctx* ctx, const uint8_t* frames , size_t F, const double* q_xyzw , int32_t level, uint64_t min_weight,
                            int32_t skip_zero, double huber_k, double* sums_out , uint64_t* counts_out , double* pm_out ,
                            double* resid_out );
emba_status emba_track_level_get(emba_ctx* ctx, int32_t level, uint64_t* sum_w_out , uint64_t* sum_v_out );

#define EMBA_EXPOSURE_GAIN 1
#define EMBA_EXPOSURE_BIAS 2
typedef struct {
    emba_align_settings align;
    double gain_min, gain_max;
} emba_exposure_settings;
emba_status emba_frames_exposure_eval(emba_ctx* ctx, const uint8_t* frames , size_t F, const double* q_xyzw ,
                                      const double* gain , const double* bias , const double* plane_host ,
                                      const uint8_t* valid_host , int32_t use_mosaic, uint64_t min_weight, double fill, double lo, double hi,
                                      int32_t skip_zero, double huber_k, double* sums_out , uint64_t* counts_out ,
                                      double* pm_out , double* resid_out );
emba_status emba_frames_exposure_align(emba_ctx* ctx, const uint8_t* frames , size_t F, const double* q_xyzw ,
                                       const double* gain_in , const double* bias_in , int32_t estimate, const double* plane_host ,
                                       const uint8_t* valid_host , int32_t use_mosaic, uint64_t min_weight, double fill, double lo, double hi,
                                       int32_t skip_zero, const emba_exposure_settings* settings, double* q_out , double* gain_out ,
                                       double* bias_out , double* sums_out , uint64_t* counts_out , int32_t* status_out ,
                                       int32_t* iters_out , double* cost0_out , uint64_t* n0_out );
emba_status emba_mosaic_frames_exposure(emba_ctx* ctx, const uint8_t* frames , const int64_t* frame_t_ns, size_t F, const double* gain ,
                                        const double* bias , const double* knots_xyzw, int32_t K, int64_t t0_ns, int64_t dt_ns, int32_t skip_zero,
                                        int32_t accumulate, uint64_t* dropped_out, uint64_t* skipped_out, double* pm_out );

typedef struct {
    emba_track_settings track;
    int32_t estimate;
    double gain_min, gain_max;
} emba_track_exposure_settings;
emba_status emba_frames_track_exposure(emba_ctx* ctx, const uint8_t* frames , const int64_t* frame_t_ns , size_t F,
                                       const double* q0_xyzw , const emba_track_exposure_settings* settings, double* q_out ,
// ... 167 lines not shown
```

Before: 11.46 billion events/s.

## Compute spline segment records on host and pass them by value as kernel arguments

Adds a step_prep=2 mode, now the default, in which the per-segment pose constants for K-1 spline segments are computed on the CPU. They are passed to a new warp kernel inside the kernel-argument segment, and each block copies them into shared memory. Block 0 writes them back to device memory for later stages. This replaces the in-warp producer/consumer handshake, where block 0 built the segments and the other blocks polled for them, and removes a separate prep pass. The cost is a larger kernarg payload on every launch and a little host arithmetic on pose knots, which are parameters rather than activations. A segment-dump API is added for verification.

Result: faster. 11.70 billion events/s, median of 6 (+2.1%).

```diff
diff --git a/emba_amd/_lib.py b/emba_amd/_lib.py
--- a/emba_amd/_lib.py
+++ b/emba_amd/_lib.py
@@ -81,6 +81,7 @@
     "emba_costs_launch": (C.c_int, [C.c_void_p, C.c_int32, C.c_double, C.c_int32]),
     "emba_costs_finish": (C.c_int, [C.c_void_p, C.c_int32, C.c_double, C.c_double, _dp, _dp]),
     "emba_dump_state": (C.c_int, [C.c_void_p, _dp, _dp, _i32p, _i32p, _i32p, _dp, _dp, _dp]),
+    "emba_dump_segments": (C.c_int, [C.c_void_p, _dp, C.c_size_t, _szp]),
     "emba_upload_map": (C.c_int, [C.c_void_p, _dp, _dp]),
     "emba_bind_map_dev": (C.c_int, [C.c_void_p, C.c_void_p, C.c_void_p]),
     "emba_solve_normal_eq": (C.c_int, [C.c_void_p, C.c_double, C.c_int32, _dp, _dp]),
diff --git a/emba_amd/csrc/context.h b/emba_amd/csrc/context.h
--- a/emba_amd/csrc/context.h
+++ b/emba_amd/csrc/context.h
@@ -66,8 +66,10 @@
     uint32_t count_stamp = 0;
     int acc_irls = 0; double acc_eta = 0.0;
     int use_texel = 0;
+    bool prep_on_host = false;
     bool prep_in_warp = false;
     bool texels_packed = false;
+    int n_seg = 0;
     bool segpose = false;
     bool readable() const { return launched && (done || inl_pending || ep_deferred); }
 };
@@ -261,7 +263,8 @@
     int texel_mode = 0;
     DevBuf d_rect;
     uint32_t seg_seq = 0;
-    int step_prep = 0, step_prep_polls = 1024;
+    int step_prep = 2, step_prep_polls = 1024;
+    emba::SegHostDuties seg_duties{}; emba::SegRecordsByValue seg_host{};
     emba::InlineSegParams seg_inline{}; emba::InlineKnots seg_knots{};
     DevBuf d_seg_flag;
     DevBuf d_blk_rect;
diff --git a/emba_amd/csrc/device_math.h b/emba_amd/csrc/device_math.h
--- a/emba_amd/csrc/device_math.h
+++ b/emba_amd/csrc/device_math.h
@@ -2,15 +2,13 @@
 #include <hip/hip_runtime.h>
 #include <stdint.h>
 
+#include "seg_record_rule.h"
+
 namespace emba {
 
 #pragma clang fp contract(off)
 
-constexpr double kSophusEps = 1e-10;
-constexpr double kPi = 3.14159265358979323846;
-
 __device__ __forceinline__ double sum3(double a, double b, double c) { return a + (b + c); }
-__device__ __forceinline__ double sqn3(double a, double b, double c) { return (a + b) + c; }
 
 __device__ __forceinline__ void mat3_mul(const double* A, const double* B, double* C)
 {
@@ -31,38 +29,6 @@
     M[0] = 0;     M[1] = -p[2]; M[2] = p[1];
     M[3] = p[2];  M[4] = 0;     M[5] = -p[0];
     M[6] = -p[1]; M[7] = p[0];  M[8] = 0;
-}
-
-__device__ __forceinline__ void quat_normalize(double* q)
-{
-    const double n2 = (q[0] * q[0] + q[2] * q[2]) + (q[1] * q[1] + q[3] * q[3]);
-    const double n = sqrt(n2);
-    q[0] /= n; q[1] /= n; q[2] /= n; q[3] /= n;
-}
-
-__device__ __forceinline__ void so3_mul(const double* a, const double* b, double* out)
-{
-    const double ax = a[0], ay = a[1], az = a[2], aw = a[3];
-    const double bx = b[0], by = b[1], bz = b[2], bw = b[3];
-    double r[4];
-    r[3] = aw * bw - ax * bx - ay * by - az * bz;
-    r[0] = aw * bx + ax * bw + ay * bz - az * by;
-    r[1] = aw * by + ay * bw + az * bx - ax * bz;
-    r[2] = aw * bz + az * bw + ax * by - ay * bx;
-    quat_normalize(r);
-    out[0] = r[0]; out[1] = r[1]; out[2] = r[2]; out[3] = r[3];
-}
-
-__device__ __forceinline__ void quat_to_matrix(const double* q, double* R)
-{
-    const double x = q[0], y = q[1], z = q[2], w = q[3];
-    const double tx = 2 * x, ty = 2 * y, tz = 2 * z;
-    const double twx = tx * w, twy = ty * w, twz = tz * w;
-    const double txx = tx * x, txy = ty * x, txz = tz * x;
-    const double tyy = ty * y, tyz = tz * y, tzz = tz * z;
-    R[0] = 1 - (tyy + tzz); R[1] = txy - twz;       R[2] = txz + twy;
-    R[3] = txy + twz;       R[4] = 1 - (txx + tzz); R[5] = tyz - twx;
-    R[6] = txz - twy;       R[7] = tyz + twx;       R[8] = 1 - (txx + tyy);
 }
 
 __device__ __forceinline__ void sin_cos_half(double x, double& sn, double& cs)
@@ -109,22 +75,6 @@
     q[0] = imag * w[0]; q[1] = imag * w[1]; q[2] = imag * w[2]; q[3] = real;
 }
 
-__device__ __forceinline__ void so3_log(const double* q, double* w)
-{
-    const double squared_n = sqn3(q[0] * q[0], q[1] * q[1], q[2] * q[2]);
-    const double qw = q[3];
-    double f;
-    if (squared_n < kSophusEps * kSophusEps) {
-        const double squared_w = qw * qw;
-        f = 2.0 / qw - (2.0 / 3.0) * (squared_n) / (qw * squared_w);
-    } else {
-        const double n = sqrt(squared_n);
-        if (fabs(qw) < kSophusEps) f = (qw > 0.0) ? kPi / n : -kPi / n;
-        else f = 2.0 * atan(n / qw) / n;
-    }
-    w[0] = f * q[0]; w[1] = f * q[1]; w[2] = f * q[2];
-}
-
 __device__ __forceinline__ void left_jacobian(const double* phi, double* J)
 {
     const double n2 = sqn3(phi[0] * phi[0], phi[1] * phi[1], phi[2] * phi[2]);
@@ -199,33 +149,6 @@
 }
 
 __device__ __forceinline__ void project_jacobian(const double* rb, double fx, double fy, double* J23);
-
-__device__ __forceinline__ void segment_consts(const double* p0, const double* p1, double* seg)
-{
-    double p0inv[4] = {-p0[0], -p0[1], -p0[2], p0[3]};
-    quat_normalize(p0inv);
-    double r01[4], delta[3], R0[9];
-    so3_mul(p0inv, p1, r01);
-    so3_log(r01, delta);
-    const double n2 = sqn3(delta[0] * delta[0], delta[1] * delta[1], delta[2] * delta[2]);
-    const double th = sqrt(n2);
-    double k[3] = {0, 0, 0}, r2;
-    if (th > 0.0) {
-        quat_to_matrix(p0, R0);
-        const double a0 = delta[0] / th, a1 = delta[1] / th, a2 = delta[2] / th;
-#pragma unroll
-        for (int r = 0; r < 3; ++r) k[r] = R0[3 * r] * a0 + R0[3 * r + 1] * a1 + R0[3 * r + 2] * a2;
-    }
-    if (n2 > kSophusEps) {
-        if (th < kPi - sqrt(kSophusEps)) r2 = 1.0 - th * (1.0 + cos(th)) / (2.0 * sin(th));
-        else r2 = n2 / (kPi * kPi);
-    } else {
-        r2 = n2 / 12.0;
-    }
-    seg[0] = p0[0]; seg[1] = p0[1]; seg[2] = p0[2]; seg[3] = p0[3];
-    seg[4] = delta[0]; seg[5] = delta[1]; seg[6] = delta[2]; seg[7] = -0.5 * th;
-    seg[8] = k[0]; seg[9] = k[1]; seg[10] = k[2]; seg[11] = r2;
-}
 
 __device__ __forceinline__ void rebuild_j1(double u, double a1, double a2, const double* k, double* J1)
 {
diff --git a/emba_amd/csrc/kernels.h b/emba_amd/csrc/kernels.h
--- a/emba_amd/csrc/kernels.h
+++ b/emba_amd/csrc/kernels.h
@@ -106,7 +106,8 @@
     o[13] = (double)s;
 }
 
-constexpr int kSegStride = 12;
+constexpr int kSegStride = kSegRecordDoubles;
+static_assert(kSegStride == 12, "a record is {p0[4], delta[3], r1, k[3], r2}");
 __device__ __forceinline__ void seg_record(int sidx, const double* __restrict__ knots, double* __restrict__ o)
 {
     double p0[4], p1[4];
@@ -292,6 +293,31 @@
     return ready;
 }
 
+constexpr int kKernargBytes = 4096, kKernargHiddenBytes = 256;
+struct SegHostDuties {
+    double* seg_out; double* knots_out; int* err_next;
+    int K;
+    double last_knot[4];
+};
+constexpr int kSegByValue = (int)((kKernargBytes - kKernargHiddenBytes - sizeof(WarpParams) - sizeof(SegHostDuties)) / (kSegStride * sizeof(double)));
+struct alignas(16) SegRecordsByValue { double r[kSegStride * kSegByValue]; };
+static_assert(sizeof(WarpParams) + sizeof(SegHostDuties) + sizeof(SegRecordsByValue) + kKernargHiddenBytes <= kKernargBytes, "the records must fit the argument segment beside the kernel's other arguments");
+static_assert(kSegByValue >= 20, "the benchmark's K = 21 must travel by value");
+static_assert(kSegStride * kSegByValue <= 32 * kRecLds, "the records share the bytes of the record staging tile");
+static_assert(kSegStride % 2 == 0 && sizeof(WarpParams) % 16 == 0 && sizeof(SegHostDuties) % 16 == 0, "16-B copies of the records");
+
+__device__ __forceinline__ void host_seg_duties(const SegHostDuties& d, const SegRecordsByValue& sr, int t)
+{
+    typedef double v2d __attribute__((ext_vector_type(2)));
+    const int n2 = (d.K - 1) * (kSegStride / 2);
+    for (int k = t; k < n2; k += kWarpBlock) reinterpret_cast<v2d*>(d.seg_out)[k] = reinterpret_cast<const v2d*>(sr.r)[k];
+    if (t == 63) d.err_next[0] = 0;
+    if (d.knots_out) {
+        for (int i = t; i < 4 * (d.K - 1); i += kWarpBlock) d.knots_out[i] = sr.r[kSegStride * (i >> 2) + (i & 3)];
+        if (t < 4) d.knots_out[4 * (d.K - 1) + t] = d.last_knot[t];
+    }
+}
+
 #ifndef WARP_LATE_EP
 #define WARP_LATE_EP 0
 #endif
@@ -316,8 +342,8 @@
 }
 
 struct NoPrefetch { __device__ __forceinline__ void operator()() const {} };
-template <bool DUMP, bool COMPACT = false, class PF = NoPrefetch, bool LATE_EP = false, bool SEGPOSE = false, bool INLINE_SEG = false>
-__device__ __forceinline__ void warp_lane(const WarpParams& p, long i, const LaneIn& in, int t, LaneOut& o, PF prefetch = PF(), const InlineSegLane* is = nullptr)
+template <bool DUMP, bool COMPACT = false, class PF = NoPrefetch, bool LATE_EP = false, bool SEGPOSE = false, int SEG_SRC = 0>
+__device__ __forceinline__ void warp_lane(const WarpParams& p, long i, const LaneIn& in, int t, LaneOut& o, PF prefetch = PF(), const InlineSegLane* is = nullptr, const double* s_seg = nullptr)
 {
     const bool valid = in.valid;
     double pm[2] = {0, 0};
@@ -338,7 +364,7 @@
         if (COMPACT || SEGPOSE) {
             const uint32_t sg = bi; const double uu = in.u;
             double seg[kSegStride];
-            if (INLINE_SEG) {
+            if (SEG_SRC == 1) {
                 typedef unsigned int v4u __attribute__((ext_vector_type(4)));
                 typedef double v2d __attribute__((ext_vector_type(2)));
                 const int off = (int)(sg * (uint32_t)(kSegStride * sizeof(double)));
@@ -348,7 +374,8 @@
                     seg[2 * k] = v.x; seg[2 * k + 1] = v.y;
                 }
             } else {
-                const double2* S2 = reinterpret_cast<const double2*>(p.seg + (size_t)kSegStride * (EMBA_ABL(p.ablate, 16) ? (sg & 1u) : sg));
+                const double2* S2 = (SEG_SRC == 2) ? reinterpret_cast<const double2*>(s_seg + kSegStride * sg)
+                                                   : reinterpret_cast<const double2*>(p.seg + (size_t)kSegStride * (EMBA_ABL(p.ablate, 16) ? (sg & 1u) : sg));
                 const double2 s0 = S2[0], s1 = S2[1], s2 = S2[2], s3 = S2[3], s4 = S2[4], s5 = S2[5];
                 seg[0] = s0.x; seg[1] = s0.y; seg[2] = s1.x; seg[3] = s1.y; seg[4] = s2.x; seg[5] = s2.y;
                 seg[6] = s3.x; seg[7] = s3.y; seg[8] = s4.x; seg[9] = s4.y; seg[10] = s5.x; seg[11] = s5.y;
@@ -516,8 +543,8 @@
 #ifndef WARP_OCC
 #define WARP_OCC
 #endif
-template <bool DUMP, bool COMPACT, bool SEGPOSE, bool INLINE_SEG>
-__device__ __forceinline__ void warp_residual_body(const WarpParams& p, const InlineSegParams* h, const double* knots)
+template <bool DUMP, bool COMPACT, bool SEGPOSE, int SEG_SRC>
+__device__ __forceinline__ void warp_residual_body(const WarpParams& p, const InlineSegParams* h, const double* knots, const SegHostDuties* hd = nullptr, const SegRecordsByValue* sr = nullptr)
 {
     __shared__ __attribute__((aligned(16))) double s_tile[32 * kRecLds];
     static_assert(32 * kRecLds >= 64 * 6 + 32, "the run sums and their pixels must fit the staging tile");
@@ -526,7 +553,8 @@
     __shared__ uint32_t s_slot[32];
 
     const int t = threadIdx.x;
-    if (INLINE_SEG && blockIdx.x == 0) inline_seg_produce(*h, knots, t, true);
+    if (SEG_SRC == 1 && blockIdx.x == 0) inline_seg_produce(*h, knots, t, true);
+    if (SEG_SRC == 2 && blockIdx.x == 0) host_seg_duties(*hd, *sr, t);
     const long b = xcd_contiguous_block(blockIdx.x, gridDim.x);
     if (b >= p.nblk) return;
     const long i = b * kWarpNew + t - 1;
@@ -534,14 +562,20 @@
     LaneOut o;
     LaneIn in;
     load_event_words<COMPACT, SEGPOSE>(p, i, valid, in);
-    if (INLINE_SEG) {
+    if (SEG_SRC == 2) {
+        typedef double v2d __attribute__((ext_vector_type(2)));
+        const int n2 = (hd->K - 1) * (kSegStride / 2);
+        for (int k = t; k < n2; k += kWarpBlock) reinterpret_cast<v2d*>(s_tile)[k] = reinterpret_cast<const v2d*>(sr->r)[k];
+        warp_lane<DUMP, COMPACT, NoPrefetch, (WARP_LATE_EP != 0) && !DUMP, SEGPOSE, 2>(p, i, in, t, o, NoPrefetch(), nullptr, s_tile);
+        __asm__ volatile("s_waitcnt lgkmcnt(0)" ::: "memory");
+    } else if (SEG_SRC == 1) {
         InlineSegLane is;
         is.rsrc = __builtin_amdgcn_make_buffer_rsrc((void*)h->seg, 0, (int)h->seg_bytes, 0x00020000);
         if (blockIdx.x != 0 && !inline_seg_wait(*h)) {
             inline_seg_produce(*h, knots, t, false);
             if (t == 0) atomicAdd(h->fallbacks, 1u);
         }
-        warp_lane<DUMP, COMPACT, NoPrefetch, (WARP_LATE_EP != 0) && !DUMP, SEGPOSE, true>(p, i, in, t, o, NoPrefetch(), &is);
+        warp_lane<DUMP, COMPACT, NoPrefetch, (WARP_LATE_EP != 0) && !DUMP, SEGPOSE, 1>(p, i, in, t, o, NoPrefetch(), &is);
     } else {
         warp_lane<DUMP, COMPACT, NoPrefetch, (WARP_LATE_EP != 0) && !DUMP, SEGPOSE>(p, i, in, t, o);
     }
@@ -603,14 +637,18 @@
 template <bool DUMP, bool COMPACT = false, bool SEGPOSE = false>
 __global__ __launch_bounds__(kWarpBlock) WARP_OCC void emba_warp_residual_kernel(WarpParams p)
 {
-    warp_residual_body<DUMP, COMPACT, SEGPOSE, false>(p, nullptr, nullptr);
+    warp_residual_body<DUMP, COMPACT, SEGPOSE, 0>(p, nullptr, nullptr);
 }
 #ifndef EMBA_INLINE_WARP_OCC
 #define EMBA_INLINE_WARP_OCC __attribute__((amdgpu_waves_per_eu(5, 5)))
 #endif
 __global__ __launch_bounds__(kWarpBlock) EMBA_INLINE_WARP_OCC void emba_warp_residual_inline_kernel(WarpParams p, InlineSegParams h, InlineKnots kn)
 {
-    warp_residual_body<false, false, true, true>(p, &h, kn.q);
+    warp_residual_body<false, false, true, 1>(p, &h, kn.q);
+}
+__global__ __launch_bounds__(kWarpBlock) WARP_OCC void emba_warp_residual_hostseg_kernel(WarpParams p, SegHostDuties d, SegRecordsByValue sr)
+{
+    warp_residual_body<false, false, true, 2>(p, nullptr, nullptr, &d, &sr);
 }
 
 template <int kTileW, int kTileH>
diff --git a/emba_amd/csrc/options_host.h b/emba_amd/csrc/options_host.h
--- a/emba_amd/csrc/options_host.h
+++ b/emba_amd/csrc/options_host.h
@@ -34,7 +34,7 @@
     {"solve_debug", &emba_ctx::opt_solve_debug, 0, 1, false},
     {"poisson", &emba_ctx::opt_poisson, 0, 2, false},
     {"gemm64", &emba_ctx::opt_gemm64, 0, 1, false},
-    {"step_prep", &emba_ctx::step_prep, 0, 1, false},
+    {"step_prep", &emba_ctx::step_prep, 0, 2, false},
     {"step_prep_polls", &emba_ctx::step_prep_polls, 0, 1 << 16, false},
     {"contrast_vote", &emba_ctx::opt_contrast_vote, -1, 1, false},
     {"gram_multikey", &emba_ctx::opt_gram_multikey, 0, 1, false},
@@ -53,6 +53,8 @@
 
 struct ReadOnlyRef { const char* name; emba_status (*read)(emba_ctx*, int32_t*); };
 const ReadOnlyRef kReadOnly[] = {
+    {"prep_on_host", [](emba_ctx* c, int32_t* v) { *v = c->ev.prep_on_host ? 1 : 0; return EMBA_OK; }},
+    {"seg_by_value", [](emba_ctx*, int32_t* v) { *v = kSegByValue; return EMBA_OK; }},
     {"prep_in_warp", [](emba_ctx* c, int32_t* v) { *v = c->ev.prep_in_warp ? 1 : 0; return EMBA_OK; }},
     {"texels_packed", [](emba_ctx* c, int32_t* v) { *v = c->ev.texels_packed ? 1 : 0; return EMBA_OK; }},
     {"step_prep_fallbacks", read_step_prep_fallbacks},
diff --git a/emba_amd/csrc/readback_host.h b/emba_amd/csrc/readback_host.h
--- a/emba_amd/csrc/readback_host.h
+++ b/emba_amd/csrc/readback_host.h
@@ -198,6 +198,21 @@
     return EMBA_OK;
 }
 
+emba_status emba_dump_segments(emba_ctx* c, double* seg, size_t cap, size_t* n_seg)
+{
+    if (!c) return EMBA_ERR_INVALID_ARG;
+    if (!c->ev.readable()) return fail(c, EMBA_ERR_STATE, "no evaluateDataError state to dump");
+    HIP_TRY(c, hipSetDevice(c->device));
+    { emba_status st0 = resolve_pending(c); if (st0) return st0; }
+    const size_t n = (size_t)c->ev.n_seg;
+    if (n_seg) *n_seg = n;
+    if (!seg || !n) return EMBA_OK;
+    if (cap < n) return fail(c, EMBA_ERR_CAPACITY, "dump_segments: room for %zu records, the evaluation left %zu", cap, n);
+    HIP_TRY(c, hipMemcpyAsync(seg, c->d_seg.as<double>(), n * kSegStride * sizeof(double), hipMemcpyDeviceToHost, c->stream));
+    HIP_TRY(c, hipStreamSynchronize(c->stream));
+    return EMBA_OK;
+}
+
 emba_status emba_last_counts(emba_ctx* c, size_t* n_inliers, size_t* P)
 {
     if (!c) return EMBA_ERR_INVALID_ARG;
diff --git a/emba_amd/csrc/seg_record_rule.h b/emba_amd/csrc/seg_record_rule.h
--- /dev/null
+++ b/emba_amd/csrc/seg_record_rule.h
@@ -0,0 +1,114 @@
+#pragma once
+#include <math.h>
+#include <stddef.h>
+
+#if defined(__HIPCC__)
+#define EMBA_SEG_HD __host__ __device__ __forceinline__
+#else
+#define EMBA_SEG_HD inline
+#endif
+#if defined(__clang__)
+#define EMBA_NO_CONTRACT _Pragma("clang fp contract(off)")
+#else
+#if defined(__FP_FAST_FMA) && !defined(EMBA_FP_CONTRACT_OFF)
+#error "seg_record_rule.h: compile with -ffp-contract=off -DEMBA_FP_CONTRACT_OFF (the target has a fused multiply-add and this compiler may contract)"
+#endif
+#define EMBA_NO_CONTRACT
+#endif
+
+namespace emba {
+
+constexpr double kSophusEps = 1e-10;
+constexpr double kPi = 3.14159265358979323846;
+
+EMBA_SEG_HD double sqn3(double a, double b, double c) { EMBA_NO_CONTRACT return (a + b) + c; }
+
+EMBA_SEG_HD void quat_normalize(double* q)
+{
+    EMBA_NO_CONTRACT
+    const double n2 = (q[0] * q[0] + q[2] * q[2]) + (q[1] * q[1] + q[3] * q[3]);
+    const double n = sqrt(n2);
+    q[0] /= n; q[1] /= n; q[2] /= n; q[3] /= n;
+}
+
+EMBA_SEG_HD void so3_mul(const double* a, const double* b, double* out)
+{
+    EMBA_NO_CONTRACT
+    const double ax = a[0], ay = a[1], az = a[2], aw = a[3];
+    const double bx = b[0], by = b[1], bz = b[2], bw = b[3];
+    double r[4];
+    r[3] = aw * bw - ax * bx - ay * by - az * bz;
+    r[0] = aw * bx + ax * bw + ay * bz - az * by;
+    r[1] = aw * by + ay * bw + az * bx - ax * bz;
+    r[2] = aw * bz + az * bw + ax * by - ay * bx;
+    quat_normalize(r);
+    out[0] = r[0]; out[1] = r[1]; out[2] = r[2]; out[3] = r[3];
+}
+
+EMBA_SEG_HD void quat_to_matrix(const double* q, double* R)
+{
+    EMBA_NO_CONTRACT
+    const double x = q[0], y = q[1], z = q[2], w = q[3];
+    const double tx = 2 * x, ty = 2 * y, tz = 2 * z;
+    const double twx = tx * w, twy = ty * w, twz = tz * w;
+    const double txx = tx * x, txy = ty * x, txz = tz * x;
+    const double tyy = ty * y, tyz = tz * y, tzz = tz * z;
+    R[0] = 1 - (tyy + tzz); R[1] = txy - twz;       R[2] = txz + twy;
+    R[3] = txy + twz;       R[4] = 1 - (txx + tzz); R[5] = tyz - twx;
+    R[6] = txz - twy;       R[7] = tyz + twx;       R[8] = 1 - (txx + tyy);
+}
+
+EMBA_SEG_HD void so3_log(const double* q, double* w)
+{
+    EMBA_NO_CONTRACT
+    const double squared_n = sqn3(q[0] * q[0], q[1] * q[1], q[2] * q[2]);
+    const double qw = q[3];
+    double f;
+    if (squared_n < kSophusEps * kSophusEps) {
+        const double squared_w = qw * qw;
+        f = 2.0 / qw - (2.0 / 3.0) * (squared_n) / (qw * squared_w);
+    } else {
+        const double n = sqrt(squared_n);
+        if (fabs(qw) < kSophusEps) f = (qw > 0.0) ? kPi / n : -kPi / n;
+        else f = 2.0 * atan(n / qw) / n;
+    }
+    w[0] = f * q[0]; w[1] = f * q[1]; w[2] = f * q[2];
+}
+
+constexpr int kSegRecordDoubles = 12;
+EMBA_SEG_HD void segment_consts(const double* p0, const double* p1, double* seg)
+{
+    EMBA_NO_CONTRACT
+    double p0inv[4] = {-p0[0], -p0[1], -p0[2], p0[3]};
+    quat_normalize(p0inv);
+    double r01[4], delta[3], R0[9];
+    so3_mul(p0inv, p1, r01);
+    so3_log(r01, delta);
+    const double n2 = sqn3(delta[0] * delta[0], delta[1] * delta[1], delta[2] * delta[2]);
+    const double th = sqrt(n2);
+    double k[3] = {0, 0, 0}, r2;
+    if (th > 0.0) {
+        quat_to_matrix(p0, R0);
+        const double a0 = delta[0] / th, a1 = delta[1] / th, a2 = delta[2] / th;
+#if defined(__clang__)
+#pragma unroll
+#endif
+        for (int r = 0; r < 3; ++r) k[r] = R0[3 * r] * a0 + R0[3 * r + 1] * a1 + R0[3 * r + 2] * a2;
+    }
+    if (n2 > kSophusEps) {
+        if (th < kPi - sqrt(kSophusEps)) r2 = 1.0 - th * (1.0 + cos(th)) / (2.0 * sin(th));
+        else r2 = n2 / (kPi * kPi);
+    } else {
+        r2 = n2 / 12.0;
+    }
+    seg[0] = p0[0]; seg[1] = p0[1]; seg[2] = p0[2]; seg[3] = p0[3];
+    seg[4] = delta[0]; seg[5] = delta[1]; seg[6] = delta[2]; seg[7] = -0.5 * th;
+    seg[8] = k[0]; seg[9] = k[1]; seg[10] = k[2]; seg[11] = r2;
+}
+
+inline void segment_records(const double* knots, int K, double* seg)
+{
+    for (int s = 0; s + 1 < K; ++s) segment_consts(knots + 4 * s, knots + 4 * (s + 1), seg + (size_t)kSegRecordDoubles * s);
+}
+
+}
diff --git a/emba_amd/csrc/step_host.h b/emba_amd/csrc/step_host.h
--- a/emba_amd/csrc/step_host.h
+++ b/emba_amd/csrc/step_host.h
@@ -268,6 +268,7 @@
     const bool seg_records = c->order.tile_order || c->ev.segpose;
     q.n_pose = ((seg_records ? (int)K - 1 : nb) + 63) / 64;
     q.seg = seg_records ? c->d_seg.as<double>() : nullptr;
+    c->ev.n_seg = seg_records ? (int)K - 1 : 0;
     const MapState& map = c->map.state();
     const bool stale = texels_stale(map.reads_own_memory(), map.version(), map.packed_version(), ((volatile int*)c->h_pinned)[5], c->seq);
     q.n_tex = texel_blocks(c->ev.use_texel, stale);
@@ -277,6 +278,15 @@
     q.rect = c->d_rect.as<int>(); q.rect_packed = c->d_rect.as<int>() + 4;
     q.texel = c->d_texel.as<double>();
     if (c->kernel_timing && c->kt_all) { HIP_TRY(c, hipEventRecord(c->kt[4], s)); c->kt_valid[c->kt_slot][2] = true; }
+    c->ev.prep_on_host = prep_on_host(c->step_prep, c->order.tile_order, c->ev.segpose, (int)K, kSegByValue, c->win.n_sorted, n_prep_blk, q.n_tex, c->ev.use_texel);
+    if (c->ev.prep_on_host) {
+        c->ev.prep_in_warp = false;
+        segment_records(knots, (int)K, c->seg_host.r);
+        SegHostDuties& d = c->seg_duties;
+        d.seg_out = c->d_seg.as<double>(); d.knots_out = c->d_knots.as<double>(); d.err_next = q.err_next; d.K = (int)K;
+        memcpy(d.last_knot, knots + (size_t)4 * (K - 1), 4 * sizeof(double));
+        return EMBA_OK;
+    }
     c->ev.prep_in_warp = prep_inside_warp(c->step_prep, c->order.tile_order, c->ev.segpose, (int)K, kInlineKnots, c->win.n_sorted, n_prep_blk, q.n_tex, c->ev.use_texel);
     if (c->ev.prep_in_warp) {
         memcpy(c->seg_knots.q, knots, (size_t)4 * K * sizeof(double));
@@ -332,6 +342,7 @@
     p.chunks = c->d_chunks.as<ChunkDesc>(); p.n_chunks = c->order.n_chunks; p.chunks_linear = c->order.chunks_lpt ? 1 : 0;
     if (c->kernel_timing) HIP_TRY(c, hipEventRecord(c->kt[0], s));
     if (tile) launch_warp_tiled(c->order.tile_shape, dim3((unsigned)grid8(c->order.n_chunks)), s, p);
+    else if (c->ev.prep_on_host) hipLaunchKernelGGL(emba_warp_residual_hostseg_kernel, dim3((unsigned)grid8(c->win.nblk)), dim3(kWarpBlock), 0, s, p, c->seg_duties, c->seg_host);
     else if (c->ev.prep_in_warp) hipLaunchKernelGGL(emba_warp_residual_inline_kernel, dim3((unsigned)grid8(c->win.nblk)), dim3(kWarpBlock), 0, s, p, c->seg_inline, c->seg_knots);
     else if (c->ev.segpose) hipLaunchKernelGGL((emba_warp_residual_kernel<false, false, true>), dim3((unsigned)grid8(c->win.nblk)), dim3(kWarpBlock), 0, s, p);
     else hipLaunchKernelGGL(emba_warp_residual_kernel<false>, dim3((unsigned)grid8(c->win.nblk)), dim3(kWarpBlock), 0, s, p);
diff --git a/emba_amd/csrc/step_rule.h b/emba_amd/csrc/step_rule.h
--- a/emba_amd/csrc/step_rule.h
+++ b/emba_amd/csrc/step_rule.h
@@ -45,7 +45,12 @@
 
 inline bool prep_inside_warp(int step_prep, bool tile_order, bool segpose, int K, int inline_knots, size_t n_sorted, int n_prep_blk, int n_tex_blk, int hessian_src)
 {
-    return step_prep != 0 && !tile_order && segpose && K <= inline_knots && n_sorted > 0 && n_prep_blk == 0 && n_tex_blk == 0 && hessian_src != 1;
+    return step_prep == 1 && !tile_order && segpose && K <= inline_knots && n_sorted > 0 && n_prep_blk == 0 && n_tex_blk == 0 && hessian_src != 1;
+}
+
+inline bool prep_on_host(int step_prep, bool tile_order, bool segpose, int K, int seg_by_value, size_t n_sorted, int n_prep_blk, int n_tex_blk, int hessian_src)
+{
+    return step_prep == 2 && !tile_order && segpose && K >= 2 && K - 1 <= seg_by_value && n_sorted > 0 && n_prep_blk == 0 && n_tex_blk == 0 && hessian_src != 1;
 }
 
 inline int prep_blocks(bool lines_clean, size_t n_sorted, size_t npix) { return (lines_clean && n_sorted) ? 0 : (int)((npix + 1023) / 1024); }
diff --git a/emba_amd/legm.py b/emba_amd/legm.py
--- a/emba_amd/legm.py
+++ b/emba_amd/legm.py
@@ -967,6 +967,14 @@
                                             g("pm_int", _i32p), g("dp", _dp), g("Gpm", _dp), g("temp", _dp)))
         return d
 
+    def dump_segments(self):
+        n = C.c_size_t()
+        self._check(self._L.emba_dump_segments(self._ctx, None, 0, C.byref(n)))
+        seg = np.zeros((n.value, 12))
+        if n.value:
+            self._check(self._L.emba_dump_segments(self._ctx, _p(seg, _dp), n.value, None))
+        return seg
+
     def upload_map(self, Gx, Gy):
         Gx = np.ascontiguousarray(Gx, dtype=np.float64); Gy = np.ascontiguousarray(Gy, dtype=np.float64)
         self._check(self._L.emba_upload_map(self._ctx, _p(Gx, _dp), _p(Gy, _dp)))
diff --git a/include/emba_hip.h b/include/emba_hip.h
--- a/include/emba_hip.h
+++ b/include/emba_hip.h
@@ -90,6 +90,7 @@
 
 emba_status emba_dump_state(emba_ctx* ctx, double* pm, double* D, int32_t* cp_idx, int32_t* inlier_idx,
                             int32_t* pm_int, double* dp, double* Gpm, double* temp);
+emba_status emba_dump_segments(emba_ctx* ctx, double* seg, size_t cap, size_t* n_seg);
 
 
 emba_status emba_upload_map(emba_ctx* ctx, const double* Gx_host, const double* Gy_host);
```
